# PetropoulakisPanagiotis/ICP-Variants

Hardware: AMD Instinct MI355X
Metric: ICP iterations/s (k-NN + point-to-plane linear, 370k-point ETH-Apartment-like pair) (higher is better)
Workload: dtype f32

## Files before the change

### icp-variants_amd/csrc/dev_fused.hpp

```cpp
struct RowSlotGen {
    const RowTerms& R;
    static constexpr int N = 27;
    template <int A> __device__ __forceinline__ double get() const { return row_slot<A>(R); }
};
struct P2pGen {
    float s[3], d[3]; double wd;
    static constexpr int N = 22;
    template <int A> __device__ __forceinline__ double get() const {
        double v;
        if constexpr (A < 3) v = (double)s[A];
        else if constexpr (A < 6) v = (double)d[A - 3];
        else if constexpr (A == 6) v = wd;
        else if constexpr (A < 10) v = wd * s[A - 7];
        else if constexpr (A < 13) v = wd * d[A - 10];
        else v = (double)d[(A - 13) / 3] * (wd * s[(A - 13) % 3]);
        return v;
    }
};
#ifndef ICP_FUSED_WAVES
#define ICP_FUSED_WAVES 6
#endif
#ifndef ICP_WAVE_STRIDE
#define ICP_WAVE_STRIDE (ICP_BVH_THREADS > 64 ? 128 : 0)
#endif
#ifndef ICP_DEBUG_WALK_ENDS
#define ICP_DEBUG_WALK_ENDS 0
#endif
#ifndef ICP_DEBUG_TIMES
#define ICP_DEBUG_TIMES 0
#endif
#if ICP_DEBUG_TIMES
#define ICP_STAMP(j) do { if (kp.dbg_steps && lane == 0) kp.dbg_steps[8 * (wave_slot) + (j)] = (int)(unsigned int)wall_clock64(); } while (0)
#define ICP_BUDGET_ROW(slot) ((kp.dbg_steps && 16 * kp.dbg_waves + 8 * 4096 <= kp.n) ? kp.dbg_steps + 8 * kp.dbg_waves + 8 * 4096 + 8 * (slot) : nullptr)
#else
#define ICP_STAMP(j)
#define ICP_BUDGET_ROW(slot) nullptr
#endif

template <int DIM> struct QueryIn {
    float r0, r1, r2;
    float c3, c4, c5;
    float rn0, rn1, rn2;
    int q0;
    float4 st;
    float4 ra, rb;
    float tq[DIM]; int j0;
};
template <int DIM>
__device__ __forceinline__ void fused_front_clear(QueryIn<DIM>& in) {
    in.r0 = 0.f; in.r1 = 0.f; in.r2 = 0.f; in.c3 = 0.f; in.c4 = 0.f; in.c5 = 0.f; in.rn0 = 0.f; in.rn1 = 0.f; in.rn2 = 0.f; in.q0 = -1; in.j0 = -1;
    in.st.x = 0.f; in.st.y = 0.f; in.st.z = 0.f; in.st.w = 0.f; in.ra = in.st; in.rb = in.st;
#pragma unroll
    for (int q = 0; q < DIM; q++) in.tq[q] = 0.f;
}
template <int DIM>
__device__ __forceinline__ void fused_front_loads(const KnnParams& kp, const PostParams& pp, const BvhViewT<DIM>& bv, int k, bool seeded, bool inc, QueryIn<DIM>& in) {
    fused_front_clear<DIM>(in);
    if (k >= 0) {
        const int i = kp.sel ? kp.sel[k] : k;
        in.r0 = kp.sx[i]; in.r1 = kp.sy[i]; in.r2 = kp.sz[i];
        if (DIM == 6) { in.c3 = kp.scr[i]; in.c4 = kp.scg[i]; in.c5 = kp.scb[i]; }
        in.rn0 = pp.snx[i]; in.rn1 = pp.sny[i]; in.rn2 = pp.snz[i];
        in.q0 = seeded ? kp.nn_raw[k] : -1;
        if (inc) in.st = kp.qstate[k];
        if (in.q0 >= 0) {
            if (DIM == 3) { in.ra = *(const float4*)(bv.recs + in.q0); in.rb = *((const float4*)(bv.recs + in.q0) + 1); in.tq[0] = in.ra.x; in.tq[1] = in.ra.y; in.tq[2] = in.ra.z; in.j0 = __float_as_int(in.ra.w); }
            else {
                const BvhLeafT<DIM>* lf = bv.leaves + (in.q0 >> 3);
#pragma unroll
                for (int q = 0; q < DIM; q++) in.tq[q] = lf->c[q][in.q0 & 7];
                in.j0 = lf->idx[in.q0 & 7];
            }
        }
    }
}

__host__ __device__ __forceinline__ int fused_wave_slot(int lb, int w, int mgrid) {
    constexpr int NW = BVH_THREADS / WAVE, S = ICP_WAVE_STRIDE;
    if (S == 0 || NW == 1) return lb * NW + w;
    if (S == 1) return w * mgrid + lb;
    const int g = lb / S, j = lb - g * S;
    return (g + 1) * S <= mgrid ? (g * NW + w) * S + j : lb * NW + w;
}

struct PairOut { bool valid; float s0, s1, s2, d0, d1, d2, n0, n1, n2, wt; };

template <int DIM, bool WIDE, bool XW = false>
__device__ __forceinline__ void fused_search_post(const KnnParams& kp, const BvhViewT<DIM>& bv, const PostParams& pp, int k, bool seeded, bool inc, const float* Pm, const float* Nm,
                                                  QueryIn<DIM>& in, uint2* __restrict__ bvh_lbq, int tid, int wave_slot, PairOut& o) {
    const int lane = tid & 63; (void)lane; (void)wave_slot; (void)seeded;
    o.valid = false; o.s0 = 0.f; o.s1 = 0.f; o.s2 = 0.f; o.d0 = 0.f; o.d1 = 0.f; o.d2 = 0.f; o.n0 = 0.f; o.n1 = 0.f; o.n2 = 0.f; o.wt = 0.f;
    float p[DIM];
#pragma unroll
    for (int q = 0; q < DIM; q++) p[q] = 0.f;
    if (DIM == 6) { p[3 % DIM] = in.c3; p[4 % DIM] = in.c4; p[5 % DIM] = in.c5; }
    float rn0 = in.rn0, rn1 = in.rn1, rn2 = in.rn2;
    float best = FLT_MAX, lb_others = 0.f; int bi = -1, bpos = -1, q0 = in.q0;
    float4 ra = in.ra, rb = in.rb;
#if ICP_DEBUG_TIMES
    float dbg_lbo = 0.f, dbg_lb3 = 0.f, dbg_delta = 0.f; int dbg_l2old = -1; const int dbg_q0old = in.q0;
#endif
    bool need_walk = false, verified = false, two_leaf = false;
    float lb3 = 0.f; int l2 = -1;
    if (k >= 0) {
        float2 st2; st2.x = 0.f; st2.y = __int_as_float(-1);
        xform_point(Pm, in.r0, in.r1, in.r2, p[0], p[1], p[2]);
        if (finite3(p[0], p[1], p[2]) && bv.n_valid > 0) {
            need_walk = true;
            if (q0 >= 0) {
                float d = 0.f;
#pragma unroll
                for (int q = 0; q < DIM; q++) { const float e = p[q] - in.tq[q]; d = (q == 0) ? e * e : d + e * e; }
                if (d < best) { best = d; bi = in.j0; bpos = q0; }
                if (inc && bi >= 0) {
                    const float ex = p[0] - in.st.x, ey = p[1] - in.st.y, ez = p[2] - in.st.z;
                    const float delta = sqrt_up((ex * ex + ey * ey) + ez * ez), sbest = sqrt_up(best);
                    const float lbn = (in.st.w - delta) * 0.999999f;
#if ICP_DEBUG_TIMES
                    dbg_lbo = in.st.w; dbg_lb3 = st2.x; dbg_delta = delta;
#endif
                    if (sbest < lbn) { lb_others = lbn; need_walk = false; verified = true; }
                    else {
                        if (kp.qstate2) st2 = kp.qstate2[k];
#if ICP_DEBUG_TIMES
                        dbg_l2old = __float_as_int(st2.y);
#endif
                        const float lb2 = (st2.x - delta) * 0.999999f;
                        l2 = __float_as_int(st2.y);
                        if (sbest < lb2) { two_leaf = true; lb3 = lb2; }
                    }
                }
            }
        }
    }
    ICP_STAMP(1);
#if ICP_DEBUG_TIMES
    if (kp.dbg_steps && k >= 0 && (need_walk || two_leaf) && seeded) {
        int* r = kp.dbg_steps + 8 * kp.dbg_waves + 8 * (k & 4095);
        r[0] = k; r[1] = __float_as_int(best); r[2] = __float_as_int(dbg_lbo); r[3] = __float_as_int(dbg_lb3); r[4] = __float_as_int(dbg_delta); r[5] = two_leaf ? l2 : -2; r[6] = q0; r[7] = (int)(unsigned int)wall_clock64();
    }
    if (kp.dbg_steps) { const int nw_ = __popcll(__ballot(need_walk && !two_leaf)), nl_ = __popcll(__ballot(two_leaf)); if (lane == 0) { kp.dbg_steps[8 * wave_slot + 6] = nw_ | (nl_ << 8);
            kp.dbg_steps[8 * wave_slot + 7] = (int)((__builtin_amdgcn_s_getreg((31 << 11) | 4) & 0xFFFFu) | (__builtin_amdgcn_s_getreg((31 << 11) | 20) << 16)); } }
#endif
    if (two_leaf) {
        f2 p2[DIM];
#pragma unroll
        for (int q = 0; q < DIM; q++) { p2[q].x = p[q]; p2[q].y = p[q]; }
        float b2 = FLT_MAX, b3 = FLT_MAX; int nl2 = -1;
        const int lf = q0 >> 3;
        if constexpr (DIM == 3) {
#pragma unroll 1
            for (int r = 0; r < 2; r++) {
                const int lx = r ? l2 : lf;
                if (r == 0 || (l2 >= 0 && l2 != lf)) leaf_eval<DIM>(bv.leaves + lx, lx, p2, best, bi, bpos, b2, nl2, b3);
            }
        } else {
            leaf_eval<DIM>(bv.leaves + lf, lf, p2, best, bi, bpos, b2, nl2, b3);
            if (l2 >= 0 && l2 != lf) leaf_eval<DIM>(bv.leaves + l2, l2, p2, best, bi, bpos, b2, nl2, b3);
        }
        lb_others = fminf(sqrt_dn(b2), lb3);
        lb3 = fminf(sqrt_dn(b3), lb3);
        l2 = nl2;
        need_walk = false;
    }
#if ICP_DEBUG_STEPS && !ICP_DEBUG_TIMES
    if (k >= 0 && kp.dbg_steps) kp.dbg_steps[k] = need_walk ? -1 : two_leaf ? -2 : 0;
#endif
#if ICP_DEBUG_TIMES
    if (int* row = ICP_BUDGET_ROW(wave_slot)) { if (lane < 8) row[lane] = 0; }
#endif
    bool walked = false;
    if (__any(need_walk)) {
        walked = true;
        float rn[3] = {rn0, rn1, rn2};
        knn_walk_shared<DIM, BVH_THREADS, typename std::conditional<WIDE, unsigned long long, unsigned int>::type, XW ? 1 : 0>(bv, p, rn, need_walk, best, bi, bpos, lb_others, lb3, l2, bvh_lbq, tid, kp.fault, ICP_BUDGET_ROW(wave_slot));
        rn0 = rn[0]; rn1 = rn[1]; rn2 = rn[2];
        q0 = -2;
        fused_front_clear<DIM>(in);
    }
    ICP_STAMP(2);
#if ICP_DEBUG_TIMES && ICP_DEBUG_WALK_ENDS
    if (k >= 0 && need_walk && seeded) {
        DEV_COUNT(8, 1);
        if (dbg_q0old >= 0 && (bpos >> 3) == (dbg_q0old >> 3)) DEV_COUNT(9, 1);
        if (dbg_l2old >= 0 && (bpos >> 3) == dbg_l2old) DEV_COUNT(10, 1);
    }
#endif
    asm volatile("" : "+v"(k));
    if (k >= 0) {
        if (!verified) knn_store_state<DIM>(kp, k, p, best, bpos, lb_others, lb3, l2);
        else if (kp.d2_out) kp.d2_out[k] = best;
        icp_match_t m;
        if (best <= kp.max_dist) { m.idx = bi; m.weight = 1.f; } else { m.idx = -1; m.weight = 0.f; }
        if (m.idx < 0) { if (pp.matches) pp.matches[k] = m; }
        else {
            if (walked || DIM != 3 || bpos != q0) { ra = *(const float4*)(bv.recs + bpos); rb = *((const float4*)(bv.recs + bpos) + 1); }
            o.d0 = ra.x; o.d1 = ra.y; o.d2 = ra.z; o.n0 = rb.x; o.n1 = rb.y; o.n2 = rb.z;
            o.s0 = p[0]; o.s1 = p[1]; o.s2 = p[2];
            o.valid = post_eval<true>(pp, k, m, o.d0, o.d1, o.d2, o.n0, o.n1, o.n2, __float_as_uint(rb.w), o.s0, o.s1, o.s2, o.wt, rn0, rn1, rn2, Nm);
        }
    }
    ICP_STAMP(3);
}

template <class StoreFn>
__device__ __forceinline__ void fused_block_epilogue(const KnnParams& kp, const PostParams& pp, PairOut& o, uint2* __restrict__ bvh_lbq, int tid, int wave_slot, const StoreFn& store) {
    constexpr int NW = BVH_THREADS / WAVE;
    const int lane = tid & 63, w = tid >> 6; (void)wave_slot; (void)kp;
    __syncthreads();
    double* lds = (double*)bvh_lbq;
    double tot;
    if (!o.valid) { o.s0 = 0.f; o.s1 = 0.f; o.s2 = 0.f; o.d0 = 0.f; o.d1 = 0.f; o.d2 = 0.f; o.n0 = 0.f; o.n1 = 0.f; o.n2 = 0.f; o.wt = 0.f; }
    if (pp.metric == ICP_METRIC_POINT_TO_PLANE) {
        RowTerms R;
        build_rows(0, o.s0, o.s1, o.s2, o.d0, o.d1, o.d2, o.n0, o.n1, o.n2, o.wt, R);
        const RowSlotGen g{R};
        tot = wave_transpose_reduce_gen<6, 0>(g, lane);
    } else {
        const P2pGen g{{o.s0, o.s1, o.s2}, {o.d0, o.d1, o.d2}, (double)o.wt};
        tot = wave_transpose_reduce_gen<6, 0>(g, lane);
    }
    ICP_STAMP(4);
    {
        const unsigned long long vm = __ballot(o.valid);
        const int v = wave_value_of_lane(lane);
        if (v < 32) lds[w * 32 + v] = tot;
        if (lane == 0) lds[NW * 32 + w] = (double)__popcll(vm);
    }
    __syncthreads();
    if (tid < NSUM_USED) {
        double out = 0.0;
        if (tid == SUM_N) { for (int ww = 0; ww < NW; ww++) out += lds[NW * 32 + ww]; }
        else {
            const int v = pp.metric == ICP_METRIC_POINT_TO_PLANE ? tid - SUM_M : tid - 1;
            const int nv = pp.metric == ICP_METRIC_POINT_TO_PLANE ? 27 : 22;
            if (v >= 0 && v < nv) { for (int ww = 0; ww < NW; ww++) out += lds[ww * 32 + v]; }
        }
        store(tid, out);
    }
    ICP_STAMP(5);
}

template <int DIM, bool WIDE, bool MERGED>
__device__ __forceinline__ void fused_matcher_body(const KnnParams& kp, const BvhViewT<DIM>& bv, const int* __restrict__ qorder, const PostParams& pp, const RingParams& rp) {
    extern __shared__ uint2 bvh_lbq[];
    constexpr int NW = BVH_THREADS / WAVE;
    if constexpr (MERGED) { if ((int)blockIdx.x < rp.n_red) { if (BVH_THREADS == RING_THREADS || threadIdx.x < RING_THREADS) ring_reduce_solve(rp); return; } }
    const int n_red = MERGED ? rp.n_red : 0;
    const int mblock = (int)blockIdx.x - n_red, mgrid = (int)gridDim.x - n_red;
    typedef const __attribute__((address_space(4))) float* cfloat_p;
    float Pm[16], Nm[9];
    if constexpr (!MERGED) {
        const cfloat_p pc = (cfloat_p)(const void*)kp.ps->pose; const cfloat_p nc = (cfloat_p)(const void*)kp.ps->nmat;
#pragma unroll
        for (int q = 0; q < 16; q++) Pm[q] = pc[q];
#pragma unroll
        for (int q = 0; q < 9; q++) Nm[q] = nc[q];
    }
    const int tid = threadIdx.x, lane = tid & 63, w = tid >> 6;
    const int lb = xcd_contiguous_block(mblock, mgrid);
    const int wave_slot = fused_wave_slot(lb, w, mgrid);
    const int t = wave_slot * BVH_QPW + lane;
    ICP_STAMP(0);
    const int k = ((BVH_QPW == WAVE || lane < BVH_QPW) && t < kp.n) ? (qorder ? qorder[t] : t) : -1;
    const bool seeded = kp.use_prev != 0, inc = kp.incremental && seeded;
    QueryIn<DIM> in;
    fused_front_loads<DIM>(kp, pp, bv, k, seeded, inc, in);
    constexpr bool XW = xw_enabled<DIM, BVH_THREADS>();
    if constexpr (XW) {
        xw_init<BVH_THREADS>(bvh_lbq, tid);
        asm volatile("s_waitcnt lgkmcnt(0)\n\ts_barrier" ::: "memory");
    }
    if constexpr (MERGED) { if (!ring_wait_pose(loop_slot((PoseState*)kp.ps, 0, (int)((blockIdx.x * 2u + (unsigned int)w) % (unsigned int)POSE_REPLICAS)), lane, rp.run_fault, Pm, Nm)) return; }
    PairOut o;
    fused_search_post<DIM, WIDE, XW>(kp, bv, pp, k, seeded, inc, Pm, Nm, in, bvh_lbq, tid, wave_slot, o);
    if constexpr (XW) {
        if (xw_block_is_searching<BVH_THREADS>(bvh_lbq)) {
            constexpr int NT = BVH_THREADS;
            bvh_lbq[3 * NT + tid] = make_uint2(__float_as_uint(o.s0), __float_as_uint(o.s1)); bvh_lbq[4 * NT + tid] = make_uint2(__float_as_uint(o.s2), __float_as_uint(o.d0));
            bvh_lbq[5 * NT + tid] = make_uint2(__float_as_uint(o.d1), __float_as_uint(o.d2)); bvh_lbq[7 * NT + tid] = make_uint2(__float_as_uint(o.n0), __float_as_uint(o.n1));
            bvh_lbq[8 * NT + tid] = make_uint2(__float_as_uint(o.n2), __float_as_uint(o.wt)); bvh_lbq[9 * NT + tid] = make_uint2(o.valid ? 1u : 0u, 0u);
            xw_help<DIM, NT, typename std::conditional<WIDE, unsigned long long, unsigned int>::type>(bv, bvh_lbq, tid, kp.fault, ICP_BUDGET_ROW(wave_slot));
            const uint2 a = bvh_lbq[3 * NT + tid], b = bvh_lbq[4 * NT + tid], c = bvh_lbq[5 * NT + tid], d = bvh_lbq[7 * NT + tid], e = bvh_lbq[8 * NT + tid], f = bvh_lbq[9 * NT + tid];
            o.s0 = __uint_as_float(a.x); o.s1 = __uint_as_float(a.y); o.s2 = __uint_as_float(b.x); o.d0 = __uint_as_float(b.y); o.d1 = __uint_as_float(c.x); o.d2 = __uint_as_float(c.y);
            o.n0 = __uint_as_float(d.x); o.n1 = __uint_as_float(d.y); o.n2 = __uint_as_float(e.x); o.wt = __uint_as_float(e.y); o.valid = f.x != 0u;
        }
    }
    double* partials = pp.partials;
    fused_block_epilogue(kp, pp, o, bvh_lbq, tid, wave_slot, [=](int a, double v) { partials[(size_t)a * mgrid + lb] = v; });
}
template <int DIM, bool WIDE>
__global__ __launch_bounds__(BVH_THREADS, DIM == 3 ? ICP_FUSED_WAVES : 4) void k_knn_bvh_post(const KnnParams kp, const BvhViewT<DIM> bv, const int* __restrict__ qorder, const PostParams pp) {
    const RingParams none{};
    fused_matcher_body<DIM, WIDE, false>(kp, bv, qorder, pp, none);
}
template <int DIM, bool WIDE>
__global__ __launch_bounds__(BVH_THREADS, DIM == 3 ? ICP_FUSED_WAVES : 4) void k_knn_bvh_post_ring(const KnnParams kp, const BvhViewT<DIM> bv, const int* __restrict__ qorder, const PostParams pp, const RingParams rp) {
    static_assert(BVH_THREADS >= RING_THREADS, "the reducer blocks are the first RING_THREADS threads of a matcher-sized block");
    fused_matcher_body<DIM, WIDE, true>(kp, bv, qorder, pp, rp);
}
```

### icp-variants_amd/csrc/dev_solve.hpp

```cpp
template <int n, int COPY>
__device__ inline void jacobi_eig_sym(double* A , double* V, double* ev) {
#pragma unroll
    for (int i = 0; i < n; i++) {
#pragma unroll
        for (int j = 0; j < n; j++) V[i * n + j] = (i == j) ? 1.0 : 0.0;
    }
    for (int sweep = 0; sweep < 50; sweep++) {
        double off = 0.0, dg = 0.0;
#pragma unroll
        for (int i = 0; i < n; i++) {
#pragma unroll
            for (int j = 0; j < n; j++) { if (i != j) off += A[i * n + j] * A[i * n + j]; else dg += A[i * n + j] * A[i * n + j]; }
        }
        if (off <= 1e-300 || off <= 1e-34 * dg) break;
#pragma unroll
        for (int p = 0; p < n - 1; p++) {
#pragma unroll
            for (int q = p + 1; q < n; q++) {
                const double apq = A[p * n + q];
                if (apq != 0.0) {
                    const double theta = (A[q * n + q] - A[p * n + p]) / (2.0 * apq);
                    const double t = (theta >= 0 ? 1.0 : -1.0) / (fabs(theta) + sqrt(theta * theta + 1.0));
                    const double c = 1.0 / sqrt(t * t + 1.0), s = t * c;
#pragma unroll
                    for (int k = 0; k < n; k++) { const double akp = A[k * n + p], akq = A[k * n + q]; A[k * n + p] = c * akp - s * akq; A[k * n + q] = s * akp + c * akq; }
#pragma unroll
                    for (int k = 0; k < n; k++) { const double apk = A[p * n + k], aqk = A[q * n + k]; A[p * n + k] = c * apk - s * aqk; A[q * n + k] = s * apk + c * aqk; }
#pragma unroll
                    for (int k = 0; k < n; k++) { const double vkp = V[k * n + p], vkq = V[k * n + q]; V[k * n + p] = c * vkp - s * vkq; V[k * n + q] = s * vkp + c * vkq; }
                    A[p * n + q] = 0.0; A[q * n + p] = 0.0;
                }
            }
        }
    }
#pragma unroll
    for (int i = 0; i < n; i++) ev[i] = A[i * n + i];
}

constexpr double RANK_CUT6 = 6.0 * 1.1920928955078125e-07;
constexpr double RANK_CUT3 = 3.0 * 1.1920928955078125e-07;
template <int COPY = 0>
__device__ inline void solve_normal_svd(const double* sums , double* x) {
    __shared__ double A[36], V[36], ev[6];
    int q = 0;
    for (int a = 0; a < 6; a++) for (int c = a; c < 6; c++) { A[a * 6 + c] = sums[q]; A[c * 6 + a] = sums[q]; q++; }
    const double* g = sums + 21;
    jacobi_eig_sym<6, COPY>(A, V, ev);
    double emax = 0.0;
    for (int i = 0; i < 6; i++) emax = fmax(emax, ev[i]);
    const double thr = RANK_CUT6;
    for (int i = 0; i < 6; i++) x[i] = 0.0;
    for (int j = 0; j < 6; j++) {
        if (!(ev[j] > thr * thr * emax)) continue;
        double vg = 0.0;
        for (int i = 0; i < 6; i++) vg += V[i * 6 + j] * g[i];
        const double coef = vg / ev[j];
        for (int i = 0; i < 6; i++) x[i] += V[i * 6 + j] * coef;
    }
}

template <int COPY = 0>
__device__ inline void solve_fullpiv_lu6(double* M, double* rhs, double* x, int* colp, double* y) {
    const int n = 6;
    for (int i = 0; i < n; i++) colp[i] = i;
    double maxpiv = 0.0; int rank = n;
    for (int k = 0; k < n; k++) {
        int pr = k, pc = k; double best = -1.0;
        for (int i = k; i < n; i++) for (int j = k; j < n; j++) { const double v = fabs(M[i * n + j]); if (v > best) { best = v; pr = i; pc = j; } }
        if (best > maxpiv) maxpiv = best;
        if (best == 0.0) { rank = k; break; }
        if (pr != k) { for (int j = 0; j < n; j++) { const double t = M[k * n + j]; M[k * n + j] = M[pr * n + j]; M[pr * n + j] = t; } const double t = rhs[k]; rhs[k] = rhs[pr]; rhs[pr] = t; }
        if (pc != k) { for (int i = 0; i < n; i++) { const double t = M[i * n + k]; M[i * n + k] = M[i * n + pc]; M[i * n + pc] = t; } const int t = colp[k]; colp[k] = colp[pc]; colp[pc] = t; }
        for (int i = k + 1; i < n; i++) {
            const double f = M[i * n + k] / M[k * n + k];
            for (int j = k + 1; j < n; j++) M[i * n + j] -= f * M[k * n + j];
            rhs[i] -= f * rhs[k];
        }
    }
    const double thr = 1.1920928955078125e-07 * 6.0;
    int r = 0;
    for (int k = 0; k < rank; k++) { if (fabs(M[k * n + k]) > maxpiv * thr) r++; else break; }
    for (int k = 0; k < n; k++) y[k] = 0.0;
    for (int k = r - 1; k >= 0; k--) { double s = rhs[k]; for (int j = k + 1; j < r; j++) s -= M[k * n + j] * y[j]; y[k] = s / M[k * n + k]; }
    for (int k = 0; k < n; k++) x[colp[k]] = (k < r) ? y[k] : 0.0;
}

template <int COPY = 0>
__device__ inline void procrustes_rotation(const double* A , double noise_floor, double* R) {
    __shared__ double B[9], V[9], ev[3], Vs[9], U[9];
    for (int i = 0; i < 3; i++) for (int j = 0; j < 3; j++) { double s = 0; for (int k = 0; k < 3; k++) s += A[k * 3 + i] * A[k * 3 + j]; B[i * 3 + j] = s; }
    jacobi_eig_sym<3, COPY>(B, V, ev);
    int o[3] = {0, 1, 2};
    for (int a = 0; a < 2; a++) for (int b = a + 1; b < 3; b++) if (ev[o[b]] > ev[o[a]]) { const int t = o[a]; o[a] = o[b]; o[b] = t; }
    for (int c = 0; c < 3; c++) for (int r = 0; r < 3; r++) Vs[r * 3 + c] = V[r * 3 + o[c]];
    double s0 = 0.0;
    for (int c = 0; c < 2; c++) {
        double u[3];
        for (int r = 0; r < 3; r++) { u[r] = 0; for (int k = 0; k < 3; k++) u[r] += A[r * 3 + k] * Vs[k * 3 + c]; }
        if (c == 1) {
            const double dp = u[0] * U[0] + u[1] * U[3] + u[2] * U[6];
            u[0] -= dp * U[0]; u[1] -= dp * U[3]; u[2] -= dp * U[6];
        }
        const double nr = sqrt(u[0] * u[0] + u[1] * u[1] + u[2] * u[2]);
        if (c == 0) {
            s0 = nr;
            if (!(nr > noise_floor)) { for (int i = 0; i < 9; i++) R[i] = (i % 4 == 0) ? 1.0 : 0.0; return; }
        } else if (!(nr > fmax(RANK_CUT3 * s0, noise_floor))) {
            const double v0 = Vs[0], v1 = Vs[3], v2 = Vs[6], u0 = U[0], u1 = U[3], u2 = U[6];
            const double cs = v0 * u0 + v1 * u1 + v2 * u2;
            if (1.0 + cs < 1e-8) {
                const int kmin = fabs(v0) < fabs(v1) ? (fabs(v0) < fabs(v2) ? 0 : 2) : (fabs(v1) < fabs(v2) ? 1 : 2);
                const double dp = (kmin == 0 ? v0 : (kmin == 1 ? v1 : v2));
                double a[3] = {(kmin == 0 ? 1.0 : 0.0) - dp * v0, (kmin == 1 ? 1.0 : 0.0) - dp * v1, (kmin == 2 ? 1.0 : 0.0) - dp * v2};
                const double an = sqrt(a[0] * a[0] + a[1] * a[1] + a[2] * a[2]);
                for (int i = 0; i < 3; i++) a[i] /= an;
                for (int r = 0; r < 3; r++) for (int q = 0; q < 3; q++) R[r * 3 + q] = 2.0 * a[r] * a[q] - (r == q ? 1.0 : 0.0);
            } else {
                const double k0 = v1 * u2 - v2 * u1, k1 = v2 * u0 - v0 * u2, k2 = v0 * u1 - v1 * u0, f = 1.0 / (1.0 + cs);
                const double kk = k0 * k0 + k1 * k1 + k2 * k2;
                R[0] = 1.0 + f * (k0 * k0 - kk); R[1] = -k2 + f * (k0 * k1);      R[2] = k1 + f * (k0 * k2);
                R[3] = k2 + f * (k1 * k0);       R[4] = 1.0 + f * (k1 * k1 - kk); R[5] = -k0 + f * (k1 * k2);
                R[6] = -k1 + f * (k2 * k0);      R[7] = k0 + f * (k2 * k1);       R[8] = 1.0 + f * (k2 * k2 - kk);
            }
            return;
        }
        for (int r = 0; r < 3; r++) U[r * 3 + c] = u[r] / nr;
    }
    U[2] = U[3] * U[7] - U[6] * U[4]; U[5] = U[6] * U[1] - U[0] * U[7]; U[8] = U[0] * U[4] - U[3] * U[1];
    const double detV = Vs[0] * (Vs[4] * Vs[8] - Vs[5] * Vs[7]) - Vs[1] * (Vs[3] * Vs[8] - Vs[5] * Vs[6]) + Vs[2] * (Vs[3] * Vs[7] - Vs[4] * Vs[6]);
    for (int r = 0; r < 3; r++) for (int c = 0; c < 3; c++)
        R[r * 3 + c] = (U[r * 3] * Vs[c * 3] + U[r * 3 + 1] * Vs[c * 3 + 1]) + detV * U[r * 3 + 2] * Vs[c * 3 + 2];
}

__device__ inline void mat4_mul_f32(const float* A, const float* B, float* C) {
    float T[16];
    for (int c = 0; c < 4; c++) for (int r = 0; r < 4; r++) {
        float acc = A[0 * 4 + r] * B[c * 4 + 0];
        acc = acc + A[1 * 4 + r] * B[c * 4 + 1];
        acc = acc + A[2 * 4 + r] * B[c * 4 + 2];
        acc = acc + A[3 * 4 + r] * B[c * 4 + 3];
        T[c * 4 + r] = acc;
    }
    for (int i = 0; i < 16; i++) C[i] = T[i];
}
__device__ inline void mat3_mul_f32(const float* A, const float* B, float* C) {
    float T[9];
    for (int r = 0; r < 3; r++) for (int c = 0; c < 3; c++) T[r * 3 + c] = A[r * 3] * B[c] + (A[r * 3 + 1] * B[3 + c] + A[r * 3 + 2] * B[6 + c]);
    for (int i = 0; i < 9; i++) C[i] = T[i];
}
__device__ inline void set_pose_f32(float* pose, const float* R, const float* t) {
    for (int i = 0; i < 16; i++) pose[i] = (i % 5 == 0) ? 1.f : 0.f;
    for (int r = 0; r < 3; r++) { for (int c = 0; c < 3; c++) pose[c * 4 + r] = R[r * 3 + c]; pose[12 + r] = t[r]; }
}
__device__ __host__ inline void normal_matrix_from_pose(const float* pose, float* N) {
    const double a = pose[0], b = pose[4], c = pose[8];
    const double d = pose[1], e = pose[5], f = pose[9];
    const double g = pose[2], h = pose[6], i = pose[10];
    const double c00 = e * i - f * h, c01 = f * g - d * i, c02 = d * h - e * g;
    const double c10 = c * h - b * i, c11 = a * i - c * g, c12 = b * g - a * h;
    const double c20 = b * f - c * e, c21 = c * d - a * f, c22 = a * e - b * d;
    const double det = (a * c00 + b * c01) + c * c02;
    N[0] = (float)(c00 / det); N[1] = (float)(c01 / det); N[2] = (float)(c02 / det);
    N[3] = (float)(c10 / det); N[4] = (float)(c11 / det); N[5] = (float)(c12 / det);
    N[6] = (float)(c20 / det); N[7] = (float)(c21 / det); N[8] = (float)(c22 / det);
}

__device__ inline float normal_matrix_entry(const float* pose, int e) {
    const double a = pose[0], b = pose[4], c = pose[8];
    const double d = pose[1], e_ = pose[5], f = pose[9];
    const double g = pose[2], h = pose[6], i = pose[10];
    const double c00 = e_ * i - f * h, c01 = f * g - d * i, c02 = d * h - e_ * g;
    const double det = (a * c00 + b * c01) + c * c02;
    double cof;
    switch (e) {
        case 0: cof = c00; break;  case 1: cof = c01; break;  case 2: cof = c02; break;
        case 3: cof = c * h - b * i; break;  case 4: cof = a * i - c * g; break;  case 5: cof = b * g - a * h; break;
        case 6: cof = b * f - c * e_; break;  case 7: cof = c * d - a * f; break;  default: cof = a * e_ - b * d; break;
    }
    return (float)(cof / det);
}

struct SolveParams {
    const double* partials; int nblocks;
    double* totals; unsigned* ticket;
    PoseState* ps;
    int metric; int phase;
    icp_iter_stats* stats;
    int n_src;
    double* sums_out;
    int update_pose;
    const double* rmse_partials; int rmse_blocks;
    int spin;
};

__device__ __forceinline__ void wave_sync() { __builtin_amdgcn_fence(__ATOMIC_ACQ_REL, "wavefront"); __builtin_amdgcn_wave_barrier(); }
constexpr int SDF_COPY = 4;
constexpr int SDF_COLOR_COPY = 5;
template <int COPY = 0>
__device__ __forceinline__ const float* p2plane_lanes_core(const double* m , const float* pose_in, double* x_out = nullptr) {
    __shared__ double A[6][7], Lm[6][6], od[6], zs[6], rd[6], hinv[6];
    __shared__ float npose[16];
    __shared__ int okflag, guardflag;
    const int tid = threadIdx.x;
    if (tid < WAVE) {
        const int i = tid / 7, j = tid % 7;
        if (tid < 42) A[i][j] = (j == 6) ? m[21 + i] : (j >= i ? m[i * 6 - i * (i - 1) / 2 + (j - i)] : 0.0);
        if (tid < 6) od[tid] = m[tid * 6 - tid * (tid - 1) / 2];
        wave_sync();
        bool ok_all = true;
        for (int k = 0; k < 6; k++) {
            const double d = A[k][k];
            const bool ok = (d > 1e-9 * od[k]) && (k > 0 || od[0] > 0);
            if (!ok) { ok_all = false; break; }
            if (tid < 42 && i > k && j >= i) {
                const double lik = A[k][i] / d;
                if (j == i) Lm[i][k] = lik;
                A[i][j] = A[i][j] - lik * A[k][j];
            }
            wave_sync();
        }
        if (tid == 0) okflag = ok_all ? 1 : 0;
    }
    __syncthreads();
    const bool factored = okflag != 0;
    if (factored && tid >= WAVE && tid < 2 * WAVE) {
        const int l = tid - WAVE;
        if (l < 6) rd[l] = 1.0 / A[l][l];
        wave_sync();
        const int kk = l < 6 ? l : 0;
        double z[6], h = 0.0;
#pragma unroll
        for (int r = 0; r < 6; r++) {
            double v = (r == kk) ? 1.0 : 0.0;
#pragma unroll
            for (int c = 0; c < r; c++) v = v - Lm[r][c] * z[c];
            z[r] = v;
            h = h + (v * v) * rd[r];
        }
        if (l < 6) hinv[l] = h;
        wave_sync();
        if (l == 0) {
            const double tr = ((((od[0] + od[1]) + od[2]) + od[3]) + od[4]) + od[5], tri = ((((hinv[0] + hinv[1]) + hinv[2]) + hinv[3]) + hinv[4]) + hinv[5];
            guardflag = (RANK_CUT6 * RANK_CUT6) * tr * tri < 1.0 ? 1 : 0;
        }
    }
    if (tid < WAVE) {
        if (factored) {
            if (tid < 6) zs[tid] = A[tid][6] / A[tid][tid];
            wave_sync();
            double x[6];
#pragma unroll
            for (int r = 5; r >= 0; r--) {
                double v = zs[r];
#pragma unroll
                for (int c = r + 1; c < 6; c++) v = v - Lm[c][r] * x[c];
                x[r] = v;
            }
            if constexpr (COPY == SDF_COPY || COPY == SDF_COLOR_COPY) {
                if (tid < 6) x_out[tid] = tid == 0 ? x[0] : tid == 1 ? x[1] : tid == 2 ? x[2] : tid == 3 ? x[3] : tid == 4 ? x[4] : x[5];
            }
            const float ang = (float)(tid == 0 ? x[0] : tid == 1 ? x[1] : x[2]);
            double sd, cd;
            sincos((double)ang, &sd, &cd);
            const float sf = (float)sd, cf = (float)cd;
            const float ca = __int_as_float(__builtin_amdgcn_readlane(__float_as_int(cf), 0)), sa = __int_as_float(__builtin_amdgcn_readlane(__float_as_int(sf), 0));
            const float cb = __int_as_float(__builtin_amdgcn_readlane(__float_as_int(cf), 1)), sb = __int_as_float(__builtin_amdgcn_readlane(__float_as_int(sf), 1));
            const float cg = __int_as_float(__builtin_amdgcn_readlane(__float_as_int(cf), 2)), sg = __int_as_float(__builtin_amdgcn_readlane(__float_as_int(sf), 2));
            if (tid < 16) {
                const int c = tid >> 2, r = tid & 3;
                const float one = 1.f, zero = 0.f;
                const float rx0 = r == 0 ? one : zero, rx1 = r == 1 ? ca : r == 2 ? sa : zero, rx2 = r == 1 ? -sa : r == 2 ? ca : zero;
                const float ry[9] = {cb, zero, sb, zero, one, zero, -sb, zero, cb}, rz[9] = {cg, -sg, zero, sg, cg, zero, zero, zero, one};
                float q[3], rr[3];
#pragma unroll
                for (int e = 0; e < 3; e++) q[e] = rx0 * ry[e] + (rx1 * ry[3 + e] + rx2 * ry[6 + e]);
#pragma unroll
                for (int e = 0; e < 3; e++) rr[e] = q[0] * rz[e] + (q[1] * rz[3 + e] + q[2] * rz[6 + e]);
                const float tr = (float)(r == 0 ? x[3] : r == 1 ? x[4] : x[5]);
                const float d0 = r < 3 ? rr[0] : zero, d1 = r < 3 ? rr[1] : zero, d2 = r < 3 ? rr[2] : zero, d3 = r < 3 ? tr : one;
                float acc = d0 * pose_in[c * 4 + 0];
                acc = acc + d1 * pose_in[c * 4 + 1];
                acc = acc + d2 * pose_in[c * 4 + 2];
                acc = acc + d3 * pose_in[c * 4 + 3];
                npose[tid] = acc;
            }
        }
    }
    __syncthreads();
    if (!factored || !guardflag) return nullptr;
    return npose;
}
template <int COPY = 0>
__device__ __forceinline__ bool solve_p2plane_lanes(const SolveParams& sp, const double* tot ) {
    if (!(sp.update_pose && sp.metric == ICP_METRIC_POINT_TO_PLANE && sp.phase == 0 && tot[SUM_N] > 0)) return false;
    PoseState* ps = sp.ps;
    const float* npose = p2plane_lanes_core<COPY>(tot + SUM_M, ps->pose);
    if (!npose) return false;
    const int tid = threadIdx.x;
    if (tid == 0 && sp.sums_out) for (int a = 0; a < NSUM; a++) sp.sums_out[a] = tot[a];
    if (tid >= 64 && tid < 70) {
        const int k = tid - 64; const double n = tot[SUM_N];
        if (k < 3) ps->mean_s[k] = (float)(tot[SUM_S + k] / n); else ps->mean_d[k - 3] = (float)(tot[SUM_D + k - 3] / n);
    }
    if (tid < 16) { ps->pose[tid] = npose[tid]; if (sp.stats) sp.stats->pose[tid] = npose[tid]; }
    if (tid >= 32 && tid < 41) ps->nmat[tid - 32] = normal_matrix_entry(npose, tid - 32);
    if (tid == 33 && sp.stats) {
        sp.stats->n_src = sp.n_src; sp.stats->n_valid = (int)tot[SUM_N];
        sp.stats->rmse = -1.f; sp.stats->benchmark_error = -1.f; sp.stats->status = ICP_OK;
    }
    return true;
}

template <bool WITH_SYMMETRIC, int COPY = 0>
__device__ inline void solve_generic(const SolveParams& sp, const double* tot) {
    if (sp.sums_out) for (int a = 0; a < NSUM; a++) sp.sums_out[a] = tot[a];
    PoseState* ps = sp.ps;
    const double n = tot[SUM_N];
    if (sp.phase == 0) {
        float ms[3] = {0, 0, 0}, md[3] = {0, 0, 0};
        if (n > 0) for (int k = 0; k < 3; k++) { ms[k] = (float)(tot[SUM_S + k] / n); md[k] = (float)(tot[SUM_D + k] / n); }
        for (int k = 0; k < 3; k++) { ps->mean_s[k] = ms[k]; ps->mean_d[k] = md[k]; }
    }
    if (!sp.update_pose) return;
    if (sp.metric == ICP_METRIC_SYMMETRIC && sp.phase == 0) return;
    int status = ICP_OK;
    float dT[16];
    for (int i = 0; i < 16; i++) dT[i] = (i % 5 == 0) ? 1.f : 0.f;
    if (!(n > 0)) {
        status = ICP_ERR_NO_CORRESPONDENCES;
    } else if (sp.metric == ICP_METRIC_POINT_TO_PLANE) {
        double x[6];
        solve_normal_svd<COPY>(tot + SUM_M, x);
        const float al = (float)x[0], be = (float)x[1], ga = (float)x[2];
        const float ca = (float)cos((double)al), sa = (float)sin((double)al);
        const float cb = (float)cos((double)be), sb = (float)sin((double)be);
        const float cg = (float)cos((double)ga), sg = (float)sin((double)ga);
        const float Rx[9] = {1, 0, 0, 0, ca, -sa, 0, sa, ca}, Ry[9] = {cb, 0, sb, 0, 1, 0, -sb, 0, cb}, Rz[9] = {cg, -sg, 0, sg, cg, 0, 0, 0, 1};
        float Rxy[9], R[9];
        mat3_mul_f32(Rx, Ry, Rxy); mat3_mul_f32(Rxy, Rz, R);
        const float t[3] = {(float)x[3], (float)x[4], (float)x[5]};
        set_pose_f32(dT, R, t);
    } else if (sp.metric == ICP_METRIC_POINT_TO_POINT) {
        const double* m = tot + SUM_M;
        const float msf[3] = {ps->mean_s[0], ps->mean_s[1], ps->mean_s[2]}, mdf[3] = {ps->mean_d[0], ps->mean_d[1], ps->mean_d[2]};
        __shared__ double A[9], Rd[9];
        for (int j = 0; j < 3; j++) for (int k = 0; k < 3; k++)
            A[j * 3 + k] = m[7 + j * 3 + k] - m[4 + j] * (double)msf[k] - (double)mdf[j] * m[1 + k] + m[0] * (double)mdf[j] * (double)msf[k];
        double mom = 0.0;
        for (int i = 0; i < 9; i++) mom = fmax(mom, fabs(m[7 + i]));
        float R[9];
        procrustes_rotation<COPY>(A, (RANK_CUT3 * RANK_CUT3) * mom, Rd);
        for (int i = 0; i < 9; i++) R[i] = (float)Rd[i];
        const float tr[3] = {mdf[0] - msf[0], mdf[1] - msf[1], mdf[2] - msf[2]};
        float t[3];
        for (int r = 0; r < 3; r++) {
            const float Rt = R[r * 3] * tr[0] + (R[r * 3 + 1] * tr[1] + R[r * 3 + 2] * tr[2]);
            const float Rm = R[r * 3] * mdf[0] + (R[r * 3 + 1] * mdf[1] + R[r * 3 + 2] * mdf[2]);
            t[r] = (Rt - Rm) + mdf[r];
        }
        set_pose_f32(dT, R, t);
    } else if constexpr (WITH_SYMMETRIC) {
        __shared__ double M[36], g[6], x[6], ywork[6];
        __shared__ int colp[6];
        int q = 0;
        for (int a = 0; a < 6; a++) for (int c = a; c < 6; c++) { M[a * 6 + c] = tot[SUM_M + q]; M[c * 6 + a] = tot[SUM_M + q]; q++; }
        for (int a = 0; a < 6; a++) g[a] = tot[SUM_M + 21 + a];
        const float lambda = 0.0001f; const float l2 = lambda * lambda;
        for (int a = 0; a < 6; a++) M[a * 6 + a] += (double)l2;
        solve_fullpiv_lu6<COPY>(M, g, x, colp, ywork);
        const float at[3] = {(float)x[0], (float)x[1], (float)x[2]}, tt[3] = {(float)x[3], (float)x[4], (float)x[5]};
        const float tan_theta = sqrtf(at[0] * at[0] + (at[1] * at[1] + at[2] * at[2]));
        const float ax[3] = {at[0] / tan_theta, at[1] / tan_theta, at[2] / tan_theta};
        const float sin_theta = (float)((double)tan_theta / sqrt(1.0 + (double)(tan_theta * tan_theta)));
        const float cos_theta = sin_theta / tan_theta;
        const float t[3] = {tt[0] * cos_theta, tt[1] * cos_theta, tt[2] * cos_theta};
        const float K[9] = {0, -ax[2], ax[1], ax[2], 0, -ax[0], -ax[1], ax[0], 0};
        float Ks[9], KK[9], Rod[9];
        const float omc = 1 - cos_theta;
        for (int i = 0; i < 9; i++) Ks[i] = omc * K[i];
        mat3_mul_f32(Ks, K, KK);
        for (int i = 0; i < 9; i++) Rod[i] = ((i % 4 == 0) ? 1.f : 0.f) + (sin_theta * K[i] + KK[i]);
        const float I3[9] = {1, 0, 0, 0, 1, 0, 0, 0, 1}, zero[3] = {0, 0, 0};
        const float md[3] = {ps->mean_d[0], ps->mean_d[1], ps->mean_d[2]}, nms[3] = {-ps->mean_s[0], -ps->mean_s[1], -ps->mean_s[2]};
        float Tm[16], Tt[16], Ts[16], Rm[16], t1[16], t2[16];
        set_pose_f32(Tm, I3, md); set_pose_f32(Tt, I3, t); set_pose_f32(Ts, I3, nms); set_pose_f32(Rm, Rod, zero);
        mat4_mul_f32(Tm, Rm, t1); mat4_mul_f32(t1, Tt, t2); mat4_mul_f32(t2, Rm, t1); mat4_mul_f32(t1, Ts, dT);
    }
    if (status == ICP_OK) {
        float np[16];
        mat4_mul_f32(dT, ps->pose, np);
        for (int i = 0; i < 16; i++) ps->pose[i] = np[i];
        normal_matrix_from_pose(ps->pose, ps->nmat);
    }
    if (sp.stats) {
        sp.stats->n_src = sp.n_src;
        sp.stats->n_valid = (int)n;
        for (int i = 0; i < 16; i++) sp.stats->pose[i] = ps->pose[i];
        sp.stats->rmse = -1.f;
        sp.stats->benchmark_error = -1.f;
        sp.stats->status = status;
    }
}

template <bool WITH_SYMMETRIC = true, int COPY = 0>
__device__ __forceinline__ void solve_tail(const SolveParams& sp, const double* tot) {
    if (solve_p2plane_lanes<COPY>(sp, tot)) return;
    if (threadIdx.x == 0) solve_generic<WITH_SYMMETRIC, COPY>(sp, tot);
}

constexpr int SOLVE_THREADS = 256;
constexpr unsigned long long TOTAL_SENTINEL = 0xFFF8D1CEC0DE5EEDull;
constexpr int SPIN_LIMIT = 1 << 22;
constexpr int SOLVE_INFLIGHT = 12;
__global__ __launch_bounds__(SOLVE_THREADS) void k_reduce_solve(const SolveParams sp) {
#include "dev_body_reduce_solve.hpp"
}


#ifndef ICP_POSE_REPLICAS
#define ICP_POSE_REPLICAS 16
#endif
constexpr int POSE_REPLICAS = ICP_POSE_REPLICAS;
constexpr size_t POSE_REPLICA_STRIDE = 4096 + 128;
__device__ __host__ __forceinline__ PoseState* loop_slot(PoseState* base, int g, int replica) {
    return (PoseState*)((char*)base + ((size_t)g * POSE_REPLICAS + (size_t)replica) * POSE_REPLICA_STRIDE);
}
__global__ void k_run_init(const PoseState* __restrict__ src, PoseState* slots, int n_slots, unsigned long long* totals, int n_totals, int* zero_words, int n_zero) {
    const int t = blockIdx.x * blockDim.x + threadIdx.x;
    const int n_slot_granules = n_slots * POSE_REPLICAS * 16;
    if (t < n_slot_granules) {
        const int g = t / (POSE_REPLICAS * 16), r = (t / 16) % POSE_REPLICAS, q = t & 15;
        unsigned long long* dst = (unsigned long long*)loop_slot(slots, g, r) + q;
        *dst = g == 0 ? ((const unsigned long long*)src)[q] : ~0ull;
    } else if (t < n_slot_granules + n_totals) totals[t - n_slot_granules] = ~0ull;
    else if (t < n_slot_granules + n_totals + n_zero) zero_words[t - n_slot_granules - n_totals] = 0;
}
constexpr unsigned long long GRANULE_EMPTY = ~0ull;
#ifndef ICP_RING_SLEEP
#define ICP_RING_SLEEP 4
#endif
struct RingParams {
    const double* red_partials; int red_nblocks;
    unsigned long long* totals_row;
    const PoseState* ps_in;
    PoseState* ps_out;
    icp_iter_stats* stats; int n_src;
    PoseState* final_out;
    int* run_fault;
    int n_red;
    ConvergeParams cv;
};
__device__ __forceinline__ unsigned long long granule_of(unsigned int lo, unsigned int hi) {
    const unsigned long long g = ((unsigned long long)hi << 32) | lo;
    return g == GRANULE_EMPTY ? g ^ 1ull : g;
}
constexpr int RING_THREADS = 128;
#ifndef ICP_DEBUG_TIMES
#define ICP_DEBUG_TIMES 0
#endif
#if ICP_DEBUG_TIMES
__device__ int g_ring_dbg[(NSUM_USED + 1) * 8];
#define RING_STAMP(a, j) do { if (threadIdx.x == 0 && !rp.final_out) g_ring_dbg[8 * (a) + (j)] = (int)(unsigned int)wall_clock64(); } while (0)
#else
#define RING_STAMP(a, j)
#endif
__device__ __forceinline__ void ring_reduce_solve(const RingParams& rp) {
    __shared__ double tot[NSUM];
    __shared__ double wsum[4];
    __shared__ unsigned int slot_words[32];
    __shared__ int give_up;
    const int tid = threadIdx.x, lane = tid & 63, w = tid >> 6, a = blockIdx.x;
    RING_STAMP(a, 0);
    if (a == 0 && rp.ps_in->fault) {
        { const unsigned int* src = (const unsigned int*)rp.ps_in; for (int q = tid; q < 16 * POSE_REPLICAS; q += RING_THREADS) __hip_atomic_store((unsigned long long*)loop_slot(rp.ps_out, 0, q >> 4) + (q & 15), granule_of(src[2 * (q & 15)], src[2 * (q & 15) + 1]), __ATOMIC_RELAXED, __HIP_MEMORY_SCOPE_AGENT);
          if (rp.final_out && tid < 32) ((unsigned int*)rp.final_out)[tid] = src[tid]; }
        return;
    }
    {
        const double* __restrict__ row = rp.red_partials + (size_t)a * rp.red_nblocks;
        double x0 = 0.0, x1 = 0.0;
        for (int b0 = 0; b0 < rp.red_nblocks; b0 += SOLVE_INFLIGHT * SOLVE_THREADS) {
            double v0[SOLVE_INFLIGHT], v1[SOLVE_INFLIGHT];
#pragma unroll
            for (int j = 0; j < SOLVE_INFLIGHT; j++) {
                const int b = b0 + j * SOLVE_THREADS + tid;
                v0[j] = b < rp.red_nblocks ? row[b] : 0.0;
                v1[j] = b + RING_THREADS < rp.red_nblocks ? row[b + RING_THREADS] : 0.0;
            }
#pragma unroll
            for (int j = 0; j < SOLVE_INFLIGHT; j++) {
                const int b = b0 + j * SOLVE_THREADS + tid;
                if (b < rp.red_nblocks) x0 += v0[j];
                if (b + RING_THREADS < rp.red_nblocks) x1 += v1[j];
            }
        }
        for (int off = 32; off > 0; off >>= 1) { x0 += __shfl_down(x0, off, WAVE); x1 += __shfl_down(x1, off, WAVE); }
        if (lane == 0) { wsum[w] = x0; wsum[2 + w] = x1; }
    }
    RING_STAMP(a, 1);
    __syncthreads();
    if (tid == 0) {
        double x = wsum[0];
        for (int k = 1; k < 4; k++) x += wsum[k];
        const unsigned long long bits = (unsigned long long)__double_as_longlong(x);
        __hip_atomic_store(rp.totals_row + a, granule_of((unsigned int)bits, (unsigned int)(bits >> 32)), __ATOMIC_RELAXED, __HIP_MEMORY_SCOPE_AGENT);
    }
    RING_STAMP(a, 2);
    if (a != 0) return;
    if (tid == 0) give_up = 0;
    __syncthreads();
    if (tid < NSUM) {
        double v = 0.0;
        if (tid < NSUM_USED) {
            unsigned long long bits = GRANULE_EMPTY;
            for (int spin = 0; spin < SPIN_LIMIT; spin++) {
                bits = __hip_atomic_load(rp.totals_row + tid, __ATOMIC_RELAXED, __HIP_MEMORY_SCOPE_AGENT);
                if (bits != GRANULE_EMPTY) break;
                __builtin_amdgcn_s_sleep(2);
            }
            if (bits == GRANULE_EMPTY) give_up = 1;
            v = __longlong_as_double((long long)bits);
        }
        tot[tid] = v;
    }
    __syncthreads();
    RING_STAMP(NSUM_USED, 0);
    const PoseState* pin = rp.ps_in;
    const double n = tot[SUM_N];
    int fault = 0, status = ICP_OK;
    const float* npose = nullptr;
    if (give_up) { fault = 1; if (tid == 0) atomicOr(rp.run_fault, 1); }
    else if (n > 0) { npose = p2plane_lanes_core(tot + SUM_M, pin->pose); if (!npose) fault = 2; }
    else status = ICP_ERR_NO_CORRESPONDENCES;
    RING_STAMP(NSUM_USED, 1);
    int code = fault;
    if (rp.cv.on && !fault) {
        if (tid < WAVE && converge_step(rp.cv, npose ? npose : pin->pose, pin->pose, status == ICP_OK, tid)) code = SLOT_STOPPED;
    }
    if (tid < 16) slot_words[tid] = __float_as_uint(npose ? npose[tid] : pin->pose[tid]);
    if (tid >= 32 && tid < 41) slot_words[16 + tid - 32] = __float_as_uint(npose ? normal_matrix_entry(npose, tid - 32) : pin->nmat[tid - 32]);
    if (tid >= 64 && tid < 70) {
        const int k = tid - 64;
        slot_words[25 + k] = __float_as_uint(n > 0 ? (float)(tot[(k < 3 ? SUM_S : SUM_D - 3) + k] / n) : 0.f);
    }
    if (tid == 0) slot_words[31] = (unsigned int)code;
    __syncthreads();
    for (int q = tid; q < 16 * POSE_REPLICAS; q += RING_THREADS)
        __hip_atomic_store((unsigned long long*)loop_slot(rp.ps_out, 0, q >> 4) + (q & 15), granule_of(slot_words[2 * (q & 15)], slot_words[2 * (q & 15) + 1]), __ATOMIC_RELAXED, __HIP_MEMORY_SCOPE_AGENT);
    RING_STAMP(NSUM_USED, 2);
    if (rp.final_out && tid < 32) ((unsigned int*)rp.final_out)[tid] = slot_words[tid];
    if (rp.stats && !fault) {
        if (tid < 16) rp.stats->pose[tid] = __uint_as_float(slot_words[tid]);
        if (tid == 16) { rp.stats->n_src = rp.n_src; rp.stats->n_valid = (int)n; rp.stats->rmse = -1.f; rp.stats->benchmark_error = -1.f; rp.stats->status = status; }
    }
}
__global__ __launch_bounds__(RING_THREADS) void k_ring_reduce_solve(const RingParams rp) { ring_reduce_solve(rp); }

__device__ __forceinline__ bool ring_wait_pose(const PoseState* slot, int lane, int* run_fault, float (&Pm)[16], float (&Nm)[9]) {
    const unsigned long long* g = (const unsigned long long*)slot;
    unsigned long long v = 0ull;
    bool ok = false;
    for (int spin = 0; spin < SPIN_LIMIT; spin++) {
        if (lane < 16) v = __hip_atomic_load(g + lane, __ATOMIC_RELAXED, __HIP_MEMORY_SCOPE_AGENT);
        if (!__any(lane < 16 && v == GRANULE_EMPTY)) { ok = true; break; }
        __builtin_amdgcn_s_sleep(ICP_RING_SLEEP);
    }
    if (!ok) { if (lane == 0) atomicOr(run_fault, 1); return false; }
    const int lo = (int)(unsigned int)v, hi = (int)(unsigned int)(v >> 32);
#pragma unroll
    for (int q = 0; q < 16; q++) Pm[q] = __int_as_float(__builtin_amdgcn_readlane((q & 1) ? hi : lo, q >> 1));
#pragma unroll
    for (int q = 0; q < 9; q++) Nm[q] = __int_as_float(__builtin_amdgcn_readlane(((16 + q) & 1) ? hi : lo, (16 + q) >> 1));
    return __builtin_amdgcn_readlane(hi, 15) == 0;
}
```

### icp-variants_amd/csrc/host_ctx.hpp

```cpp
using namespace icpdev;

#define HIPCK(ctx, expr)                                                                        \
    do {                                                                                        \
        hipError_t e__ = (expr);                                                                \
        if (e__ != hipSuccess) {                                                                \
            char buf__[256];                                                                    \
            snprintf(buf__, sizeof(buf__), "%s failed: %s (%s:%d)", #expr, hipGetErrorString(e__), __FILE__, __LINE__); \
            (ctx)->err = buf__;                                                                 \
            return ICP_ERR_HIP;                                                                 \
        }                                                                                       \
    } while (0)

namespace {
std::atomic<long long> g_live_bytes{0};

struct DevBuf {
    void* p = nullptr; size_t cap = 0;
    bool view = false;
    DevBuf() = default;
    DevBuf(DevBuf&& o) noexcept : p(o.p), cap(o.cap), view(o.view) { o.p = nullptr; o.cap = 0; o.view = false; }
    DevBuf& operator=(DevBuf&& o) noexcept { if (this != &o) { reset(); p = o.p; cap = o.cap; view = o.view; o.p = nullptr; o.cap = 0; o.view = false; } return *this; }
    ~DevBuf() { reset(); }
    void reset() { if (p && !view) { (void)hipFree(p); g_live_bytes -= (long long)cap; } p = nullptr; cap = 0; view = false; }
    template <class T> T* as() const { return (T*)p; }
};
static_assert(!std::is_copy_constructible<DevBuf>::value && !std::is_copy_assignable<DevBuf>::value, "a copied DevBuf would be freed twice");
struct PinBuf {
    void* p = nullptr; size_t cap = 0;
    PinBuf() = default; PinBuf(const PinBuf&) = delete; PinBuf& operator=(const PinBuf&) = delete;
    ~PinBuf() { if (p) (void)hipHostFree(p); }
    template <class T> T* as() const { return (T*)p; }
};
struct Event {
    hipEvent_t e = nullptr;
    Event() = default; Event(Event&& o) noexcept : e(o.e) { o.e = nullptr; } Event& operator=(Event&& o) noexcept { std::swap(e, o.e); return *this; }
    ~Event() { if (e) (void)hipEventDestroy(e); }
    operator hipEvent_t() const { return e; }
};
struct Stream {
    hipStream_t s = nullptr;
    Stream() = default; Stream(const Stream&) = delete; Stream& operator=(const Stream&) = delete;
    ~Stream() { if (s) (void)hipStreamDestroy(s); }
    operator hipStream_t() const { return s; }
};

struct Cloud {
    int n = 0, npad = 0;
    DevBuf x, y, z, nx, ny, nz, cr, cg, cb, rgba;
    bool has_normals = false, has_colors = false;
};

struct Level { DevBuf idx; DevBuf order; DevBuf sorted_idx; DevBuf pack; Cloud sorted; bool sorted_valid = false; int n = 0; };

struct NssLevel { DevBuf cand, seg, longs; int n_base = 0, max_long = 0, max_chunks = 0; };
struct NssHeld { Level lv; uint32_t word = 0; };

struct FpfhCache { DevBuf nb_idx, nb_d2, counts, pairs, feat; bool ready = false; int k = 0, stride = 0, n = 0, nk = 0; };

struct Bvh {
    bool valid = false;
    int n_valid = 0, n_leaves = 0, Lp = 1;
    DevBuf keys, keys2, vals, vals2, temp, leaves, recs, nodes, qnodes, pos_of;
    DevBuf axl[12], side, scanr, axis_of_node;
    int n_ids = 0;
    const Cloud* attrs = nullptr;
    int Lq = 0;
    const int* d_finite = nullptr;
    double build_ms = 0.0;
};
}

struct icp_ctx {
    int device = 0;
    Stream own_stream, depth_stream;
    hipStream_t stream = nullptr;
    int stage_timing = 1;
    unsigned timing_phase = 0;
    PinBuf pinned;
    bool trace = false;
    bool merge_loop = true;
    int merged_runs = 0, merged_fallbacks = 0;
    bool lm_on = false; icp_lm_options lm_opt;
    DevBuf lm_state, lm_partials, lm_sums;
    std::vector<icp_lm_summary> lm_last;
    DevBuf ms_ps, ms_nn, ms_st, ms_st2, ms_rec, ms_d2, ms_partials, ms_totals, ms_stats, ms_score, ms_res;
    icp_gicp_options gicp_opt = {1e-3f, 20};
    DevBuf gicp_n[2][3], gicp_flag;
    bool gicp_ready[2] = {false, false};
    icp_colored_options col_opt = {0.968f, 20};
    DevBuf col_grad[3];
    bool col_ready = false;
    icp_robust_options rob_opt = {ICP_ROBUST_NONE, 0.f, 0.f, 1.f};
    DevBuf rob_keys, rob_state, rob_stats;
    std::vector<icp_robust_stats> rob_last;
    icp_reciprocal_options rcp_opt = {0};
    Bvh src_bvh; DevBuf src_rflag, src_finite;
    DevBuf rcp_stats;
    bool rcp_naive = false; DevBuf rcp_q[3], rcp_nn;
    std::vector<icp_reciprocal_stats> rcp_last;
    icp_convergence_options cvg_opt = {0, 1e-6f, 1e-6f, 1, 1};
    icp_convergence_result cvg_last = {0, 0, 0, -1.f, -1.f};
    std::vector<icp_convergence_step> cvg_trace;
    icp_global_options glob_opt = {20, 1, 1, 4096, 0.9f, 0.005f, 0u, 16};
    FpfhCache fpfh[2];
    DevBuf gm_best[2], gm_fwd, gm_keep, gm_list, gm_idx, gm_pts, gm_hyp;
    std::vector<icp_global_hypothesis> glob_last;
    icp_params prm;
    Cloud tgt, src, qry;
    Cloud nrm_cloud; Bvh nrm_bvh;
    Bvh bvh, bvh6;
    DevBuf src_flag, src_box;
    DevBuf tgt_flag, tgt_finite, nrm_finite, sel_temp, d_count;
    PinBuf pin_up; Event up_ev; bool up_pending = false;
    DevBuf okeys, okeys2, ovals, otemp;
    std::map<int, Level> levels;
    DevBuf sel_lists, sel_counts, sel_blocks;
    icp_nss_options nss_opt = {5, 1};
    DevBuf nss_bkt; int nss_bkt_grid = 0;
    std::map<int, NssLevel> nss_levels;
    std::map<int, NssHeld> nss_held;
    float nss_held_proba = 0.f; uint32_t nss_held_seed = 0u; bool nss_held_stale = false;
    DevBuf nss_table, nss_quota, nss_thr, nss_state, nss_hist, nss_total;
    std::vector<std::pair<const int*, int>> sel_last;
    DevBuf qpack; size_t q_cap = 0;
    DevBuf qstate, qstate2;
    DevBuf dbg_steps;
    DevBuf ps, matches, d2, best64, nn_raw, partials, partials2, ring, totals, sums, stats, staging, rmse_partials, rmse_out, fontana_partials;
    Cloud conv_src, conv_ref; int conv_n = 0;
    PinBuf depth_pin[2]; DevBuf depth_dev[2]; Event depth_up[2]; bool depth_pending[2] = {false, false};
    DevBuf depth_blocks, track_rmse;
    PinBuf pin_track;
    DevBuf tsdf_vox, tsdf_cnt; bool tsdf_on = false; icp_tsdf_options tsdf_opt;
    DevBuf tsdf_col; bool tsdf_col_on = false;
    DevBuf th_keys, th_vals, th_pool, th_pkey, th_ctr;
    bool tsdf_hashed = false; int th_log2cap = 0, th_pool_cap = 0, th_nblk = 0, th_grown = 0, th_unplaced = 0, th_max_log2 = 22; long long th_oor = 0;
    DevBuf tm_bits, tm_mask, tm_base, tm_blk, tm_out;
    DevBuf tm_nbr, tm_ord;
    DevBuf sdf_state, sdf_partials, sdf_rec; Event sdf_ev;
    DevBuf vg_box, vg_count, vg_sums, vg_cells;
    bool vg_ready = false; float vg_voxel = 0.f; icp_voxel_grid_info vg_info = {{0, 0, 0}, {0, 0, 0}, 0, 0};
    DevBuf vm_count, vm_sums, vm_cells, vm_stamp, vm_list, vm_ctr, vm_box;
    bool vm_on = false; icp_voxel_map_options vm_opt = {0.f, {0, 0, 0}, {0, 0, 0}}; int vm_serial = 0;
    DevBuf vh_keys;
    bool vm_hashed = false; int vh_log2cap = 0, vh_grown = 0; long long vh_bound = 0;
    bool vh_vac = false; int vh_compacted = 0; long long vh_vac_bound = 0;
    float cos_reject = 0.5f;
    std::vector<Event> events;
    Event build_ev[2];
    icp_timing timing;
    std::vector<float> it_match_ms, it_post_ms, it_solve_ms;
    std::string err;
};

namespace {
constexpr int POST_BLOCKS = 512;

int ensure(icp_ctx* c, DevBuf& b, size_t bytes) {
    if (bytes <= b.cap && b.p) return ICP_OK;
    if (b.view) { b.p = nullptr; b.cap = 0; b.view = false; }
    if (b.p) { HIPCK(c, hipFree(b.p)); g_live_bytes -= (long long)b.cap; b.p = nullptr; b.cap = 0; }
    size_t want = bytes < 256 ? 256 : bytes;
    HIPCK(c, hipMalloc(&b.p, want));
    b.cap = want; g_live_bytes += (long long)want;
    return ICP_OK;
}
int ensure_pin(icp_ctx* c, PinBuf& b, size_t bytes, size_t min_bytes, size_t slack_div) {
    if (bytes <= b.cap && b.p) return ICP_OK;
    if (b.p) { HIPCK(c, hipHostFree(b.p)); b.p = nullptr; b.cap = 0; }
    const size_t want = bytes < min_bytes ? min_bytes : bytes + (slack_div ? bytes / slack_div : 0);
    HIPCK(c, hipHostMalloc(&b.p, want, hipHostMallocDefault));
    b.cap = want;
    return ICP_OK;
}
int ensure_pinned(icp_ctx* c, size_t bytes) { return ensure_pin(c, c->pinned, bytes, 4096, 0); }
void release(DevBuf& b) { b.reset(); }
void set_view(DevBuf& b, void* p, size_t bytes) { release(b); b.p = p; b.cap = bytes; b.view = true; }
void release(Cloud& c) { release(c.x); release(c.y); release(c.z); release(c.nx); release(c.ny); release(c.nz); release(c.cr); release(c.cg); release(c.cb); release(c.rgba); }
void release(Level& lv) { release(lv.idx); release(lv.order); release(lv.sorted_idx); release(lv.sorted); release(lv.pack); lv.sorted_valid = false; }
void release(NssLevel& nl) { release(nl.cand); release(nl.seg); release(nl.longs); }
void drop_nss(icp_ctx* c, bool held_only);

float compute_cos_reject() {
    const double threshold = 60 * 3.141592653589793238462643383279502884 / 180.0;
    uint32_t lo, hi; float flo = 0.25f, fhi = 0.75f;
    memcpy(&lo, &flo, 4); memcpy(&hi, &fhi, 4);
    while (hi - lo > 1) {
        uint32_t mid = lo + (hi - lo) / 2; float fm; memcpy(&fm, &mid, 4);
        if ((double)acosf(fm) > threshold) lo = mid; else hi = mid;
    }
    float r; memcpy(&r, &lo, 4);
    return r;
}

int set_device(icp_ctx* c) { HIPCK(c, hipSetDevice(c->device)); return ICP_OK; }

struct DrainOnError {
    icp_ctx* c; bool ok = false;
    explicit DrainOnError(icp_ctx* ctx) : c(ctx) {}
    ~DrainOnError() { if (!ok && c && c->stream) (void)hipStreamSynchronize(c->stream); }
    int done(int rc = ICP_OK) { ok = (rc == ICP_OK); return rc; }
};

int ensure_pin_up(icp_ctx* c, size_t bytes) {
    if (c->up_pending) { HIPCK(c, hipEventSynchronize(c->up_ev)); c->up_pending = false; }
    int rc;
    if ((rc = ensure_pin(c, c->pin_up, bytes, 65536, 8))) return rc;
    if (!c->up_ev) HIPCK(c, hipEventCreateWithFlags(&c->up_ev.e, hipEventDisableTiming));
    return ICP_OK;
}
int upload_cloud(icp_ctx* c, Cloud& cl, const float* xyz, const float* nrm, const uint8_t* rgba, int n, bool pad_inf) {
    const int npad = pad_inf ? ((n + 63) / 64) * 64 : n;
    const size_t b_xyz = (size_t)n * 12, b_nrm = nrm ? (size_t)n * 12 : 0, b_col = rgba ? (size_t)n * 4 : 0, total = b_xyz + b_nrm + b_col;
    int rc;
    if ((rc = ensure_pin_up(c, total))) return rc;
    if ((rc = ensure(c, c->staging, total))) return rc;
    char* h = c->pin_up.as<char>();
    memcpy(h, xyz, b_xyz);
    if (nrm) memcpy(h + b_xyz, nrm, b_nrm);
    if (rgba) memcpy(h + b_xyz + b_nrm, rgba, b_col);
    HIPCK(c, hipMemcpyAsync(c->staging.p, h, total, hipMemcpyHostToDevice, c->stream));
    HIPCK(c, hipEventRecord(c->up_ev, c->stream)); c->up_pending = true;
    const char* d = c->staging.as<char>();
    const dim3 g((npad + 255) / 256), b(256);
    for (DevBuf* pl : {&cl.x, &cl.y, &cl.z}) if ((rc = ensure(c, *pl, (size_t)npad * 4))) return rc;
    hipLaunchKernelGGL(k_deinterleave3, g, b, 0, c->stream, (const float*)d, n, npad, INFINITY, cl.x.as<float>(), cl.y.as<float>(), cl.z.as<float>());
    cl.has_normals = nrm != nullptr;
    if (nrm) {
        for (DevBuf* pl : {&cl.nx, &cl.ny, &cl.nz}) if ((rc = ensure(c, *pl, (size_t)n * 4))) return rc;
        hipLaunchKernelGGL(k_deinterleave3, dim3((n + 255) / 256), b, 0, c->stream, (const float*)(d + b_xyz), n, n, 0.f, cl.nx.as<float>(), cl.ny.as<float>(), cl.nz.as<float>());
    }
    cl.has_colors = rgba != nullptr;
    if (rgba) {
        for (DevBuf* pl : {&cl.rgba, &cl.cr, &cl.cg, &cl.cb}) if ((rc = ensure(c, *pl, (size_t)npad * 4))) return rc;
        hipLaunchKernelGGL(k_colors, g, b, 0, c->stream, (const uint8_t*)(d + b_xyz + b_nrm), n, npad, cl.rgba.as<uint32_t>(), cl.cr.as<float>(), cl.cg.as<float>(), cl.cb.as<float>());
    }
    HIPCK(c, hipGetLastError());
    cl.n = n; cl.npad = npad;
    return ICP_OK;
}
int upload3(icp_ctx* c, const float* aos, int n, int npad, float pad_value, DevBuf& x, DevBuf& y, DevBuf& z) {
    int rc;
    if ((rc = ensure_pin_up(c, (size_t)n * 12))) return rc;
    if ((rc = ensure(c, c->staging, (size_t)n * 12))) return rc;
    for (DevBuf* pl : {&x, &y, &z}) if ((rc = ensure(c, *pl, (size_t)npad * 4))) return rc;
    memcpy(c->pin_up.p, aos, (size_t)n * 12);
    HIPCK(c, hipMemcpyAsync(c->staging.p, c->pin_up.p, (size_t)n * 12, hipMemcpyHostToDevice, c->stream));
    HIPCK(c, hipEventRecord(c->up_ev, c->stream)); c->up_pending = true;
    hipLaunchKernelGGL(k_deinterleave3, dim3((npad + 255) / 256), dim3(256), 0, c->stream, c->staging.as<float>(), n, npad, pad_value, x.as<float>(), y.as<float>(), z.as<float>());
    HIPCK(c, hipGetLastError());
    HIPCK(c, hipStreamSynchronize(c->stream));
    return ICP_OK;
}

int count_slot(icp_ctx* c, int** slot) {
    int rc;
    if ((rc = ensure_pinned(c, 4096))) return rc;
    *slot = (int*)(c->pinned.as<char>() + 2048);
    return ICP_OK;
}
int read_count(icp_ctx* c, const void* d_count, int* out, int n_words = 1) {
    int rc; int* h;
    if ((rc = count_slot(c, &h))) return rc;
    HIPCK(c, hipMemcpyAsync(h, d_count, (size_t)n_words * 4, hipMemcpyDeviceToHost, c->stream));
    HIPCK(c, hipStreamSynchronize(c->stream));
    memcpy(out, h, (size_t)n_words * 4);
    return ICP_OK;
}

int compact_flagged(icp_ctx* c, const uint8_t* d_flags, int count, int factor, DevBuf& out, int* n_out) {
    int rc;
    if ((rc = ensure(c, out, (size_t)(count > 0 ? count : 1) * 4))) return rc;
    if ((rc = ensure(c, c->d_count, 16))) return rc;
    *n_out = 0;
    if (count <= 0) return ICP_OK;
    auto in = rocprim::make_transform_iterator(rocprim::counting_iterator<int>(0), MulBy{factor});
    size_t tb = 0;
    HIPCK(c, rocprim::select(nullptr, tb, in, d_flags, out.as<int>(), c->d_count.as<int>(), (size_t)count, c->stream));
    if ((rc = ensure(c, c->sel_temp, tb))) return rc;
    HIPCK(c, rocprim::select(c->sel_temp.p, tb, in, d_flags, out.as<int>(), c->d_count.as<int>(), (size_t)count, c->stream));
    return read_count(c, c->d_count.p, n_out);
}
int finite_list(icp_ctx* c, const Cloud& cl, bool with_normals, DevBuf& flag, DevBuf& list, int* n_out) {
    int rc;
    if ((rc = ensure(c, flag, (size_t)cl.n))) return rc;
    const bool nrm = with_normals && cl.has_normals;
    hipLaunchKernelGGL(k_mark_finite, dim3((cl.n + 255) / 256), dim3(256), 0, c->stream, cl.x.as<float>(), cl.y.as<float>(), cl.z.as<float>(),
                       nrm ? cl.nx.as<float>() : nullptr, nrm ? cl.ny.as<float>() : nullptr, nrm ? cl.nz.as<float>() : nullptr, cl.n, flag.as<uint8_t>());
    HIPCK(c, hipGetLastError());
    return compact_flagged(c, flag.as<uint8_t>(), cl.n, 1, list, n_out);
}

int write_pose_via(icp_ctx* c, PoseState* h, const float pose[16]) {
    int rc;
    memset(h, 0, sizeof(*h));
    memcpy(h->pose, pose, 64);
    normal_matrix_from_pose(h->pose, h->nmat);
    if ((rc = ensure(c, c->ps, sizeof(PoseState)))) return rc;
    HIPCK(c, hipMemcpyAsync(c->ps.p, h, sizeof(*h), hipMemcpyHostToDevice, c->stream));
    return ICP_OK;
}
int write_pose(icp_ctx* c, const float pose[16]) {
    int rc;
    if ((rc = ensure_pinned(c, sizeof(PoseState)))) return rc;
    return write_pose_via(c, c->pinned.as<PoseState>(), pose);
}

int check_ready(icp_ctx* c, bool need_source, bool full_pipeline) {
    const icp_params& p = c->prm;
    if (c->tgt.n <= 0) { c->err = "target index needs to be built before querying (icp_set_target)"; return ICP_ERR_NO_TARGET; }
    if (need_source && c->src.n <= 0) { c->err = "no source cloud (icp_set_source)"; return ICP_ERR_NO_SOURCE; }
    if (p.matching == ICP_MATCH_PROJECTIVE) {
        if (p.height <= 0 || p.width <= 0) { c->err = "set camera params before querying any matches"; return ICP_ERR_NO_CAMERA; }
        if ((long long)p.width * p.height != c->tgt.n) { c->err = "invalid size of target points (must be width*height)"; return ICP_ERR_TARGET_SIZE; }
    } else if (p.color_icp) {
        if (!c->tgt.has_colors || (need_source && !c->src.has_colors)) { c->err = "colour ICP needs colours on target and source"; return ICP_ERR_COLOR_MISMATCH; }
    }
    if (full_pipeline) {
        if (!c->tgt.has_normals || !c->src.has_normals) { c->err = "normals required on source and target"; return ICP_ERR_INVALID_ARG; }
        if (p.weighting == ICP_WEIGHT_COLORS && (!c->tgt.has_colors || !c->src.has_colors)) { c->err = "colour weighting needs colours"; return ICP_ERR_COLOR_MISMATCH; }
    }
    return ICP_OK;
}

int ensure_events(icp_ctx* c, size_t count) {
    while (c->events.size() < count) { Event e; HIPCK(c, hipEventCreate(&e.e)); c->events.push_back(std::move(e)); }
    return ICP_OK;
}
}
```

### icp-variants_amd/csrc/host_debug.hpp

```cpp
extern "C" {
int icp_debug_steps(icp_ctx* c, int32_t* out, int32_t n) {
    if (!c || !out || n <= 0 || !c->dbg_steps.p || (size_t)n * 4 > c->dbg_steps.cap) return ICP_ERR_INVALID_ARG;
    int rc;
    if ((rc = set_device(c))) return rc;
    HIPCK(c, hipMemcpy(out, c->dbg_steps.p, (size_t)n * 4, hipMemcpyDeviceToHost));
    return ICP_OK;
}

int icp_debug_ring_times(icp_ctx* c, int32_t* out, int32_t n) {
#if ICP_DEBUG_TIMES
    if (!c || !out || n < (NSUM_USED + 1) * 8) return ICP_ERR_INVALID_ARG;
    int rc;
    if ((rc = set_device(c))) return rc;
    HIPCK(c, hipMemcpyFromSymbol(out, HIP_SYMBOL(icpdev::g_ring_dbg), (size_t)(NSUM_USED + 1) * 8 * 4));
    return ICP_OK;
#else
    (void)c; (void)out; (void)n;
    return ICP_ERR_INVALID_ARG;
#endif
}
int icp_debug_dev_counters(icp_ctx* c, uint32_t* out16, int32_t reset) {
#if ICP_DEBUG_TIMES
    if (!c || !out16) return ICP_ERR_INVALID_ARG;
    int rc;
    if ((rc = set_device(c))) return rc;
    HIPCK(c, hipStreamSynchronize(c->stream));
    HIPCK(c, hipMemcpyFromSymbol(out16, HIP_SYMBOL(icpdev::g_dev_counts), 64));
    if (reset == 2) HIPCK(c, hipMemcpyFromSymbol(out16, HIP_SYMBOL(icpdev::g_walk_trace), 256));
    if (reset) { uint32_t z[16] = {0}; HIPCK(c, hipMemcpyToSymbol(HIP_SYMBOL(icpdev::g_dev_counts), z, 64)); }
    return ICP_OK;
#else
    (void)c; (void)out16; (void)reset;
    return ICP_ERR_INVALID_ARG;
#endif
}
int icp_debug_wave_slot(int32_t lb, int32_t w, int32_t mgrid, int32_t* waves_per_block) {
    if (waves_per_block) *waves_per_block = BVH_THREADS / WAVE;
    if (lb < 0 || lb >= mgrid || w < 0 || w >= BVH_THREADS / WAVE) return -1;
    return icpdev::fused_wave_slot(lb, w, mgrid);
}
__global__ void k_debug_pos_of(const icpdev::TgtRec* recs, const int* pos_of, int n_slots, int* bad) {
    const int i = blockIdx.x * blockDim.x + threadIdx.x;
    if (i < n_slots && recs[i].idx >= 0 && pos_of[recs[i].idx] != i) atomicAdd(bad, 1);
}
int icp_debug_pos_of_mismatches(icp_ctx* c, int32_t* n_bad, int32_t* n_checked) {
    if (!c || !n_bad || !c->bvh.valid) return ICP_ERR_INVALID_ARG;
    int rc;
    if ((rc = set_device(c))) return rc;
    const int n_slots = (c->bvh.n_leaves > 0 ? c->bvh.n_leaves : 1) * BVH_LEAF;
    if ((rc = ensure(c, c->d_count, 4))) return rc;
    HIPCK(c, hipMemsetAsync(c->d_count.p, 0, 4, c->stream));
    hipLaunchKernelGGL(k_debug_pos_of, dim3((n_slots + 255) / 256), dim3(256), 0, c->stream, c->bvh.recs.as<icpdev::TgtRec>(), c->bvh.pos_of.as<int>(), n_slots, c->d_count.as<int>());
    HIPCK(c, hipMemcpyAsync(n_bad, c->d_count.p, 4, hipMemcpyDeviceToHost, c->stream));
    HIPCK(c, hipStreamSynchronize(c->stream));
    if (n_checked) *n_checked = c->bvh.n_valid;
    return ICP_OK;
}
int icp_debug_live_bytes(int64_t* out) {
    if (!out) return ICP_ERR_INVALID_ARG;
    *out = (int64_t)g_live_bytes.load();
    return ICP_OK;
}
int icp_debug_reciprocal_naive(icp_ctx* c, int32_t on) {
    if (!c) return ICP_ERR_INVALID_ARG;
    c->rcp_naive = on != 0;
    return ICP_OK;
}
int icp_debug_counters(icp_ctx* c, int32_t* merged_runs, int32_t* merged_fallbacks) {
    if (!c) return ICP_ERR_INVALID_ARG;
    if (merged_runs) *merged_runs = c->merged_runs;
    if (merged_fallbacks) *merged_fallbacks = c->merged_fallbacks;
    return ICP_OK;
}
int icp_debug_poison_handover(icp_ctx* c, int32_t slot, double value) {
    if (!c || slot < 0 || slot >= NSUM) return ICP_ERR_INVALID_ARG;
    int rc;
    if ((rc = set_device(c))) return rc;
    if (!c->totals.p && (rc = rearm_handover(c))) return rc;
    HIPCK(c, hipMemcpyAsync(c->totals.as<double>() + slot, &value, 8, hipMemcpyHostToDevice, c->stream));
    HIPCK(c, hipStreamSynchronize(c->stream));
    return ICP_OK;
}

int icp_debug_loop_sums(icp_ctx* c, const float pose[16], int32_t form, int32_t iteration, double* sums_out, int32_t* n_valid_out, float* pose_out, int32_t* route_out) {
    if (!c || !pose || !sums_out || !n_valid_out || !pose_out || !route_out || (form != 0 && form != 1)) { if (c) c->err = "icp_debug_loop_sums: bad argument"; return ICP_ERR_INVALID_ARG; }
    const icp_params& p = c->prm;
    int rc;
    DrainOnError guard(c);
    if ((rc = set_device(c))) return rc;
    if ((rc = check_ready(c, true, true))) return rc;
    if ((rc = gicp_prepare(c))) return rc;
    if ((rc = colored_prepare(c))) return rc;
    if (c->lm_on || robust_on(c) || reciprocal_on(c)) { c->err = "icp_debug_loop_sums: the non-linear optimiser, robust mode and reciprocal rejection run other chains"; return ICP_ERR_INVALID_ARG; }
    RunPlan pl;
    if ((rc = make_plan(c, false, pl))) return rc;
    const int iters = pl.iters(), it = iteration;
    if (it < 0 || it >= iters || pl.ns[it] <= 0) { c->err = "icp_debug_loop_sums: no such iteration in the plan, or it has no queries"; return ICP_ERR_INVALID_ARG; }
    const bool colors = p.color_icp != 0 && p.matching == ICP_MATCH_KNN;
    const bool lbvh = p.matching == ICP_MATCH_KNN && p.knn_backend == ICP_KNN_LBVH;
    double hs[NSUM]; icp_iter_stats st; memset(&st, 0, sizeof(st)); PoseState hp; int family = 0;
    if (form == 0) {
        if ((rc = ensure(c, c->stats, 512)) || (rc = ensure(c, c->sums, NSUM * 8))) return rc;
        if ((rc = rearm_handover(c))) return rc;
        if ((rc = write_pose(c, pose))) return rc;
        QuerySet q{pl.clouds[it], pl.sels[it], pl.ns[it], 0, colors, false, pl.orders[it], false};
        int fused = 0;
        if ((rc = launch_match(c, q, &fused))) return rc;
        if ((rc = launch_post_and_solve(c, *pl.clouds[it], pl.sels[it], pl.ns[it], c->stats.as<icp_iter_stats>(), c->sums.as<double>(), 1, nullptr, fused, nullptr))) return rc;
        family = fused ? 1 : 0;
        HIPCK(c, hipMemcpyAsync(hs, c->sums.p, NSUM * 8, hipMemcpyDeviceToHost, c->stream));
        HIPCK(c, hipMemcpyAsync(&st, c->stats.p, sizeof(st), hipMemcpyDeviceToHost, c->stream));
        HIPCK(c, hipMemcpyAsync(&hp, c->ps.p, sizeof(hp), hipMemcpyDeviceToHost, c->stream));
        HIPCK(c, hipStreamSynchronize(c->stream));
        if (hp.fault) { c->err = "reduction hand-over timed out on the device (k_reduce_solve)"; return ICP_ERR_HIP; }
    } else {
        const bool rec = (p.record_rmse & 3) && c->conv_n > 0;
        bool merged = iters >= 2 && pl.sorted_levels && p.metric == ICP_METRIC_POINT_TO_PLANE && !rec;
        for (int i = 0; merged && i < iters; i++) if (pl.ns[i] <= 0) merged = false;
        if (!merged) { c->err = "icp_debug_loop_sums: the loop of this configuration does not take the merged form"; return ICP_ERR_INVALID_ARG; }
        const int two[2] = {it, it + 1 < iters ? it + 1 : it};
        LoopRun r{};
        r.pl.sorted_levels = pl.sorted_levels; r.pl.fixed_sets = pl.fixed_sets;
        for (int k : two) { r.pl.factors.push_back(pl.factors[k]); r.pl.ns.push_back(pl.ns[k]); r.pl.clouds.push_back(pl.clouds[k]); r.pl.sels.push_back(pl.sels[k]); r.pl.orders.push_back(pl.orders[k]); }
        r.lay_out(2, false, false);
        if ((rc = ensure_pinned(c, r.pin_bytes))) return rc;
        if ((rc = write_pose(c, pose))) return rc;
        if ((rc = ensure(c, c->stats, r.stats_bytes))) return rc;
        if ((rc = ensure_events(c, 2 * 4 + 2))) return rc;
        r.sampled.assign(2, 0); r.eligible.assign(2, 0); r.ev.assign(2, IterEvents());
        if ((rc = enqueue_merged(c, r))) return rc;
        unsigned long long row[NSUM];
        HIPCK(c, hipMemcpyAsync(row, c->ring.as<char>() + (size_t)3 * POSE_REPLICAS * POSE_REPLICA_STRIDE, NSUM * 8, hipMemcpyDeviceToHost, c->stream));
        HIPCK(c, hipMemcpyAsync(&hp, loop_slot(c->ring.as<PoseState>(), 1, 0), sizeof(hp), hipMemcpyDeviceToHost, c->stream));
        HIPCK(c, hipStreamSynchronize(c->stream));
        if (r.host_tail(c)->merged_fault || hp.fault == 1) { c->err = "icp_debug_loop_sums: a bounded wait of the merged launches ran out"; return ICP_ERR_HIP; }
        for (int a = 0; a < NSUM; a++) {
            if (a < NSUM_USED && row[a] == GRANULE_EMPTY) { c->err = "icp_debug_loop_sums: a total of the ring was never written"; return ICP_ERR_HIP; }
            if (a < NSUM_USED) memcpy(&hs[a], &row[a], 8); else hs[a] = 0.0;
        }
        if (hp.fault) { memcpy(st.pose, pose, 64); st.n_valid = (int)hs[SUM_N]; }
        else memcpy(&st, r.host_records(c), sizeof(st));
        family = 2;
    }
    const Bvh& b = colors ? c->bvh6 : c->bvh;
    route_out[0] = family; route_out[1] = colors ? 6 : 3; route_out[2] = lbvh ? (b.Lq > 8 ? 1 : 0) : -1; route_out[3] = hp.fault;
    memset(sums_out, 0, 64 * 8); memcpy(sums_out, hs, NSUM * 8);
    *n_valid_out = st.n_valid;
    memcpy(pose_out, st.pose, 64);
    return guard.done();
}

__global__ void k_debug_walk_steps(int n_leaves, const icpdev::BvhLeafT<3>* leaves, const float* lq, const int* leaf_no, const float* sf, const int* si, float* of, int* oi,
                                   int n_nodes, const icpdev::BvhQuadT<3>* nodes, const float* nq, float* bounds) {
    const int i = blockIdx.x * blockDim.x + threadIdx.x;
    if (i < n_leaves) {
        icpdev::f2 p2[3];
        for (int k = 0; k < 3; k++) { p2[k].x = lq[3 * i + k]; p2[k].y = p2[k].x; }
        float best = sf[3 * i], b2 = sf[3 * i + 1], b3 = sf[3 * i + 2]; int bi = si[3 * i], bpos = si[3 * i + 1], l2 = si[3 * i + 2];
        const int flags = icpdev::leaf_eval<3>(leaves + i, leaf_no[i], p2, best, bi, bpos, b2, l2, b3);
        of[3 * i] = best; of[3 * i + 1] = b2; of[3 * i + 2] = b3; oi[4 * i] = bi; oi[4 * i + 1] = bpos; oi[4 * i + 2] = l2; oi[4 * i + 3] = flags;
    }
    if (i < n_nodes) {
        icpdev::f2 p2[3], l01, l23;
        for (int k = 0; k < 3; k++) { p2[k].x = nq[3 * i + k]; p2[k].y = p2[k].x; }
        icpdev::quad_lb<3>(nodes + i, p2, l01, l23);
        bounds[4 * i] = l01.x; bounds[4 * i + 1] = l01.y; bounds[4 * i + 2] = l23.x; bounds[4 * i + 3] = l23.y;
    }
}
int icp_debug_walk_steps(icp_ctx* c, int32_t n_leaves, const void* leaves, const float* lq, const int32_t* leaf_no, const float* sf, const int32_t* si, float* of, int32_t* oi,
                         int32_t n_nodes, const void* nodes, const float* nq, float* bounds, float* empty_box) {
    if (!c || n_leaves < 0 || n_nodes < 0 || n_leaves > (1 << 20) || n_nodes > (1 << 20)) return ICP_ERR_INVALID_ARG;
    if (n_leaves > 0 && (!leaves || !lq || !leaf_no || !sf || !si || !of || !oi)) return ICP_ERR_INVALID_ARG;
    if (n_nodes > 0 && (!nodes || !nq || !bounds)) return ICP_ERR_INVALID_ARG;
    if (empty_box) { empty_box[0] = icpdev::BVH_QUAD_EMPTY_LO; empty_box[1] = icpdev::BVH_QUAD_EMPTY_HI; }
    const int n = n_leaves > n_nodes ? n_leaves : n_nodes;
    if (n == 0) return ICP_OK;
    int rc;
    if ((rc = set_device(c))) return rc;
    DrainOnError guard(c);
    const size_t L = (size_t)n_leaves, N = (size_t)n_nodes;
    auto up = [](size_t x) { return (x + 127) & ~(size_t)127; };
    const size_t o_lq = 128 * L, o_no = up(o_lq + 12 * L), o_sf = up(o_no + 4 * L), o_si = up(o_sf + 12 * L), o_nd = up(o_si + 12 * L), o_nq = o_nd + 128 * N, o_of = up(o_nq + 12 * N),
                 o_oi = up(o_of + 12 * L), o_bd = up(o_oi + 16 * L), total = o_bd + 16 * N;
    if ((rc = ensure(c, c->staging, total))) return rc;
    char* d = c->staging.as<char>();
    if (L) {
        HIPCK(c, hipMemcpyAsync(d, leaves, 128 * L, hipMemcpyHostToDevice, c->stream));
        HIPCK(c, hipMemcpyAsync(d + o_lq, lq, 12 * L, hipMemcpyHostToDevice, c->stream));
        HIPCK(c, hipMemcpyAsync(d + o_no, leaf_no, 4 * L, hipMemcpyHostToDevice, c->stream));
        HIPCK(c, hipMemcpyAsync(d + o_sf, sf, 12 * L, hipMemcpyHostToDevice, c->stream));
        HIPCK(c, hipMemcpyAsync(d + o_si, si, 12 * L, hipMemcpyHostToDevice, c->stream));
    }
    if (N) {
        HIPCK(c, hipMemcpyAsync(d + o_nd, nodes, 128 * N, hipMemcpyHostToDevice, c->stream));
        HIPCK(c, hipMemcpyAsync(d + o_nq, nq, 12 * N, hipMemcpyHostToDevice, c->stream));
    }
    hipLaunchKernelGGL(k_debug_walk_steps, dim3((unsigned)((n + 255) / 256)), dim3(256), 0, c->stream, n_leaves, (const icpdev::BvhLeafT<3>*)d, (const float*)(d + o_lq), (const int*)(d + o_no),
                       (const float*)(d + o_sf), (const int*)(d + o_si), (float*)(d + o_of), (int*)(d + o_oi), n_nodes, (const icpdev::BvhQuadT<3>*)(d + o_nd), (const float*)(d + o_nq), (float*)(d + o_bd));
    HIPCK(c, hipGetLastError());
    if (L) {
        HIPCK(c, hipMemcpyAsync(of, d + o_of, 12 * L, hipMemcpyDeviceToHost, c->stream));
        HIPCK(c, hipMemcpyAsync(oi, d + o_oi, 16 * L, hipMemcpyDeviceToHost, c->stream));
    }
    if (N) HIPCK(c, hipMemcpyAsync(bounds, d + o_bd, 16 * N, hipMemcpyDeviceToHost, c->stream));
    HIPCK(c, hipStreamSynchronize(c->stream));
    return guard.done();
}

int icp_selftest_wave_reduce(icp_ctx* c, const double* in, double* out, int32_t* lane_of) {
    if (!c || !in || !out || !lane_of) return ICP_ERR_INVALID_ARG;
    int rc;
    if ((rc = set_device(c))) return rc;
    DrainOnError guard(c);
    if ((rc = ensure(c, c->staging, 64 * 27 * 8 + 27 * 8 + 27 * 4 + 64))) return rc;
    double* d_in = c->staging.as<double>(); double* d_out = d_in + 64 * 27; int* d_lane = (int*)(d_out + 27);
    HIPCK(c, hipMemcpyAsync(d_in, in, 64 * 27 * 8, hipMemcpyHostToDevice, c->stream));
    hipLaunchKernelGGL(k_selftest_wave_reduce, dim3(1), dim3(64), 0, c->stream, d_in, d_out, d_lane);
    HIPCK(c, hipGetLastError());
    HIPCK(c, hipMemcpyAsync(out, d_out, 27 * 8, hipMemcpyDeviceToHost, c->stream));
    HIPCK(c, hipMemcpyAsync(lane_of, d_lane, 27 * 4, hipMemcpyDeviceToHost, c->stream));
    HIPCK(c, hipStreamSynchronize(c->stream));
    return guard.done();
}
}
```

### icp-variants_amd/csrc/host_launch.hpp

```cpp
namespace {
struct MergeLaunch { RingParams rp; const PoseState* slot; double* partials; hipEvent_t ev_start = nullptr, ev_stop = nullptr; };

constexpr size_t WALK_LDS_BYTES = (size_t)ICP_SHARE_ROWS * BVH_THREADS * 8;
template <int DIM> size_t fused_lds_bytes() {
    const size_t red_bytes = (size_t)(BVH_THREADS / WAVE) * 33 * 8;
    return (WALK_LDS_BYTES > red_bytes ? WALK_LDS_BYTES : red_bytes) + xw_lds_bytes<DIM, BVH_THREADS>();
}
int post_nblocks(int n) { const int nb = (n + POST_THREADS - 1) / POST_THREADS; return nb > POST_BLOCKS ? POST_BLOCKS : nb < 1 ? 1 : nb; }
template <class K> K pick_wide(int Lq, K narrow, K wide) { return Lq <= 8 ? narrow : wide; }

struct QuerySet { const Cloud* cl; const int* sel; int n; int pretransformed; bool use_colors; bool seed_prev; const int* order; bool keep_records = false; };

int ensure_qpack(icp_ctx* c, int n) {
    if ((size_t)n <= c->q_cap && c->qpack.p) return ICP_OK;
    int rc;
    c->q_cap = ((size_t)n + 63) / 64 * 64;
    if ((rc = ensure(c, c->qpack, c->q_cap * 28))) return rc;
    set_view(c->nn_raw, c->qpack.p, c->q_cap * 4); set_view(c->qstate, c->qpack.as<char>() + c->q_cap * 4, c->q_cap * 16);
    set_view(c->qstate2, c->qpack.as<char>() + c->q_cap * 20, c->q_cap * 8);
    return ICP_OK;
}

KnnParams knn_params(const icp_ctx* c, const Cloud& q, const int* sel, int n) {
    KnnParams kp; memset(&kp, 0, sizeof(kp));
    kp.sx = q.x.as<float>(); kp.sy = q.y.as<float>(); kp.sz = q.z.as<float>(); kp.scr = q.cr.as<float>(); kp.scg = q.cg.as<float>(); kp.scb = q.cb.as<float>();
    kp.sel = sel; kp.n = n;
    kp.tx = c->tgt.x.as<float>(); kp.ty = c->tgt.y.as<float>(); kp.tz = c->tgt.z.as<float>();
    kp.tcr = c->tgt.cr.as<float>(); kp.tcg = c->tgt.cg.as<float>(); kp.tcb = c->tgt.cb.as<float>();
    kp.mpad = c->tgt.npad; kp.max_dist = c->prm.max_distance; kp.nseg = 1;
    return kp;
}

PostParams make_post_params(icp_ctx* c, const Cloud& src, const int* sel, int n) {
    const icp_params& p = c->prm;
    PostParams pp;
    pp.sx = src.x.as<float>(); pp.sy = src.y.as<float>(); pp.sz = src.z.as<float>();
    pp.snx = src.nx.as<float>(); pp.sny = src.ny.as<float>(); pp.snz = src.nz.as<float>();
    pp.srgba = src.rgba.as<uint32_t>(); pp.sel = sel; pp.n = n;
    pp.tx = c->tgt.x.as<float>(); pp.ty = c->tgt.y.as<float>(); pp.tz = c->tgt.z.as<float>();
    pp.tnx = c->tgt.nx.as<float>(); pp.tny = c->tgt.ny.as<float>(); pp.tnz = c->tgt.nz.as<float>(); pp.trgba = c->tgt.rgba.as<uint32_t>();
    pp.ps = c->ps.as<PoseState>(); pp.matches = c->matches.as<icp_match_t>();
    pp.metric = p.metric; pp.weighting = p.weighting; pp.rejection = p.rejection;
    pp.max_dist = p.max_distance; pp.cos_reject = c->cos_reject; pp.partials = c->partials.as<double>();
    return pp;
}

template <int DIM>
int launch_bvh_query(icp_ctx* c, Bvh& b, const CoordPtrs<DIM>& cp, const KnnParams& kp, const int* order, int n, const Cloud* fuse, bool keep_records, int* fused_blocks, const MergeLaunch* ml = nullptr) {
    int rc;
    if (!b.valid && (rc = build_bvh<DIM>(c, b, cp))) return rc;
    const BvhViewT<DIM> bv = make_view<DIM>(b, cp);
    const int nb = fuse ? fused_nblocks(n) : (n + BVH_THREADS - 1) / BVH_THREADS;
    if (fuse) {
        if ((rc = ensure(c, c->partials, (size_t)(nb > POST_BLOCKS ? nb : POST_BLOCKS) * NSUM * 8))) return rc;
        PostParams pp = make_post_params(c, *fuse, kp.sel, n);
        KnnParams kf = kp; kf.out = nullptr;
        if (!keep_records) { pp.matches = nullptr; kf.d2_out = nullptr; }
        const size_t lds = fused_lds_bytes<DIM>();
        if (ml) {
            kf.ps = ml->slot; pp.ps = ml->slot; pp.partials = ml->partials; kf.fault = ml->rp.run_fault;
            const auto ring = pick_wide(b.Lq, k_knn_bvh_post_ring<DIM, false>, k_knn_bvh_post_ring<DIM, true>);
            if (ml->ev_start) hipExtLaunchKernelGGL(ring, dim3(nb + ml->rp.n_red), dim3(BVH_THREADS), (uint32_t)lds, c->stream, ml->ev_start, ml->ev_stop, 0, kf, bv, order, pp, ml->rp);
            else hipLaunchKernelGGL(ring, dim3(nb + ml->rp.n_red), dim3(BVH_THREADS), lds, c->stream, kf, bv, order, pp, ml->rp);
        }
        else hipLaunchKernelGGL(pick_wide(b.Lq, k_knn_bvh_post<DIM, false>, k_knn_bvh_post<DIM, true>), dim3(nb), dim3(BVH_THREADS), lds, c->stream, kf, bv, order, pp);
        *fused_blocks = nb;
    } else hipLaunchKernelGGL(k_knn_bvh<DIM>, dim3(nb), dim3(BVH_THREADS), WALK_LDS_BYTES, c->stream, kp, bv, order);
    HIPCK(c, hipGetLastError());
    return ICP_OK;
}

int launch_match(icp_ctx* c, const QuerySet& q, int* fused_blocks = nullptr, const MergeLaunch* ml = nullptr) {
    const icp_params& p = c->prm;
    int rc;
    if (fused_blocks) *fused_blocks = 0;
    if ((rc = ensure(c, c->matches, (size_t)q.n * sizeof(icp_match_t))) || (rc = ensure(c, c->d2, (size_t)q.n * 4))) return rc;
    if (p.matching == ICP_MATCH_PROJECTIVE) {
        ProjParams pp;
        pp.sx = q.cl->x.as<float>(); pp.sy = q.cl->y.as<float>(); pp.sz = q.cl->z.as<float>(); pp.sel = q.sel; pp.n = q.n;
        pp.tx = c->tgt.x.as<float>(); pp.ty = c->tgt.y.as<float>(); pp.tz = c->tgt.z.as<float>();
        pp.width = p.width; pp.height = p.height; pp.fx = p.fx; pp.fy = p.fy; pp.mx = p.cx; pp.my = p.cy; pp.window = 12;
        pp.ps = c->ps.as<PoseState>(); pp.pretransformed = q.pretransformed; pp.max_dist = p.max_distance;
        pp.out = c->matches.as<icp_match_t>(); pp.d2_out = c->d2.as<float>();
        hipLaunchKernelGGL(k_projective, dim3((q.n + 255) / 256), dim3(256), 0, c->stream, pp);
        HIPCK(c, hipGetLastError());
        return ICP_OK;
    }
    KnnParams kp = knn_params(c, *q.cl, q.sel, q.n);
    kp.ps = c->ps.as<PoseState>(); kp.pretransformed = q.pretransformed; kp.fault = &c->ps.as<PoseState>()->fault;
    kp.out = c->matches.as<icp_match_t>(); kp.d2_out = c->d2.as<float>();
    if (p.knn_backend == ICP_KNN_LBVH) {
        if ((rc = ensure_qpack(c, q.n))) return rc;
        kp.nn_raw = c->nn_raw.as<int>(); kp.use_prev = q.seed_prev ? 1 : 0;
#if ICP_DEBUG_STEPS
        if ((rc = ensure(c, c->dbg_steps, (size_t)q.n * 4))) return rc;
        kp.dbg_steps = c->dbg_steps.as<int>(); kp.dbg_waves = fused_nblocks(q.n) * (BVH_THREADS / WAVE);
#endif
        if (p.knn_incremental && !q.pretransformed) {
            kp.qstate = c->qstate.as<float4>(); kp.qstate2 = c->qstate2.as<float2>(); kp.incremental = 1;
        }
        const Cloud* fuse = (fused_blocks != nullptr && p.metric != ICP_METRIC_SYMMETRIC && p.metric != ICP_METRIC_GICP && p.metric != ICP_METRIC_COLORED && !q.pretransformed) ? q.cl : nullptr;
        if (q.use_colors) return launch_bvh_query<6>(c, c->bvh6, target_coords6(c), kp, q.order, q.n, fuse, q.keep_records, fused_blocks, fuse ? ml : nullptr);
        return launch_bvh_query<3>(c, c->bvh, target_coords3(c), kp, q.order, q.n, fuse, q.keep_records, fused_blocks, fuse ? ml : nullptr);
    }
    const int bx = (q.n + WAVE - 1) / WAVE;
    const int nch = kp.mpad / KNN_CH;
    int nseg = 1;
    if (bx < 1024) { nseg = (2048 + bx - 1) / bx; if (nseg > nch / 4) nseg = nch / 4; if (nseg < 1) nseg = 1; }
    kp.nseg = nseg;
    if (nseg > 1) {
        if ((rc = ensure(c, c->best64, (size_t)q.n * 8))) return rc;
        kp.best64 = c->best64.as<unsigned long long>();
        const unsigned long long init = ((unsigned long long)0x7F7FFFFFu << 32) | 0xFFFFFFFFull;
        hipLaunchKernelGGL(k_fill_u64, dim3((q.n + 255) / 256), dim3(256), 0, c->stream, kp.best64, q.n, init);
    }
    if (q.use_colors) hipLaunchKernelGGL(k_knn_brute<6>, dim3(bx, nseg), dim3(256), 0, c->stream, kp);
    else              hipLaunchKernelGGL(k_knn_brute<3>, dim3(bx, nseg), dim3(256), 0, c->stream, kp);
    if (nseg > 1)
        hipLaunchKernelGGL(k_knn_finalize, dim3((q.n + 255) / 256), dim3(256), 0, c->stream, kp.best64, q.n, p.max_distance,
                           c->matches.as<icp_match_t>(), c->d2.as<float>());
    HIPCK(c, hipGetLastError());
    return ICP_OK;
}

int rearm_handover(icp_ctx* c) {
    int rc;
    if ((rc = ensure(c, c->totals, NSUM * 8 + 8))) return rc;
    HIPCK(c, hipMemsetAsync(c->totals.p, 0, NSUM * 8 + 8, c->stream));
    hipLaunchKernelGGL(k_fill_u64, dim3(1), dim3(64), 0, c->stream, c->totals.as<unsigned long long>(), NSUM, TOTAL_SENTINEL);
    HIPCK(c, hipGetLastError());
    return ICP_OK;
}

const int* level_src_orig(icp_ctx* c, const Cloud& src) {
    if (&src == &c->src) return nullptr;
    for (auto& kv : c->levels) if (&kv.second.sorted == &src) return kv.second.sorted_idx.as<int>();
    for (auto& kv : c->nss_held) if (&kv.second.lv.sorted == &src) return kv.second.lv.sorted_idx.as<int>();
    return nullptr;
}

GicpPost gicp_post_params(icp_ctx* c, const Cloud& src) {
    GicpPost g; memset(&g, 0, sizeof(g));
    const bool own_t = c->gicp_opt.covariance_k == 0, own_s = own_t;
    g.tnx = own_t ? c->tgt.nx.as<float>() : c->gicp_n[0][0].as<float>(); g.tny = own_t ? c->tgt.ny.as<float>() : c->gicp_n[0][1].as<float>(); g.tnz = own_t ? c->tgt.nz.as<float>() : c->gicp_n[0][2].as<float>();
    g.snx = own_s ? c->src.nx.as<float>() : c->gicp_n[1][0].as<float>(); g.sny = own_s ? c->src.ny.as<float>() : c->gicp_n[1][1].as<float>(); g.snz = own_s ? c->src.nz.as<float>() : c->gicp_n[1][2].as<float>();
    g.src_orig = level_src_orig(c, src);
    g.one_minus_eps = 1.0 - (double)c->gicp_opt.epsilon;
    return g;
}

ColoredPost colored_post_params(icp_ctx* c) {
    ColoredPost g;
    g.gx = c->col_grad[0].as<float>(); g.gy = c->col_grad[1].as<float>(); g.gz = c->col_grad[2].as<float>();
    g.lambda = (double)c->col_opt.lambda_geometric;
    return g;
}

bool robust_on(const icp_ctx* c) { return c->rob_opt.kernel != ICP_ROBUST_NONE || c->rob_opt.overlap < 1.f; }

int robust_prepare(icp_ctx* c, int slots) {
    int rc;
    if ((rc = ensure(c, c->rob_state, sizeof(RobustState)))) return rc;
    if ((rc = ensure(c, c->rob_stats, (size_t)(slots > 0 ? slots : 1) * sizeof(icp_robust_stats)))) return rc;
    if ((rc = ensure(c, c->rob_keys, (size_t)(c->src.n > 0 ? c->src.n : 1) * 4))) return rc;
    HIPCK(c, hipMemsetAsync(c->rob_state.p, 0, sizeof(RobustState), c->stream));
    return ICP_OK;
}

int launch_robust(icp_ctx* c, const PostParams& pp, int n, icp_robust_stats* d_rstats) {
    int rc;
    if ((rc = ensure(c, c->rob_keys, (size_t)(n > 0 ? n : 1) * 4))) return rc;
    static const float standard[4] = {0.f, 1.345f, 2.3849f, 4.6851f};
    const icp_robust_options& o = c->rob_opt;
    RobustParams rp;
    rp.st = c->rob_state.as<RobustState>(); rp.keys = c->rob_keys.as<unsigned int>(); rp.stats = d_rstats;
    rp.kernel = o.kernel; rp.linear_weight = c->prm.metric == ICP_METRIC_POINT_TO_POINT ? 1 : 0;
    rp.tuning = o.tuning > 0.f ? o.tuning : standard[o.kernel]; rp.sigma = o.sigma; rp.overlap = o.overlap; rp.n = n;
    int nb = (n + ROBUST_THREADS - 1) / ROBUST_THREADS; if (nb > ROBUST_BLOCKS) nb = ROBUST_BLOCKS; if (nb < 1) nb = 1;
    hipLaunchKernelGGL(k_robust_eval, dim3(nb), dim3(ROBUST_THREADS), 0, c->stream, pp, rp);
    hipLaunchKernelGGL(k_robust_select<1>, dim3(nb), dim3(ROBUST_THREADS), 0, c->stream, rp);
    hipLaunchKernelGGL(k_robust_select<2>, dim3(nb), dim3(ROBUST_THREADS), 0, c->stream, rp);
    hipLaunchKernelGGL(k_robust_finish, dim3(1), dim3(ROBUST_THREADS), 0, c->stream, rp);
    hipLaunchKernelGGL(k_robust_apply, dim3(nb), dim3(ROBUST_THREADS), 0, c->stream, pp, rp);
    HIPCK(c, hipGetLastError());
    return ICP_OK;
}

bool reciprocal_on(const icp_ctx* c) { return c->rcp_opt.enabled != 0; }

int reciprocal_check(icp_ctx* c) {
    if (c->prm.color_icp) { c->err = "reciprocal rejection (icp_set_reciprocal_options) does not support color_icp = 1: a 6-D forward search against a 3-D reverse one is not a mutual test"; return ICP_ERR_INVALID_ARG; }
    if (c->lm_on) { c->err = "the non-linear optimiser does not support reciprocal rejection (icp_set_reciprocal_options)"; return ICP_ERR_INVALID_ARG; }
    return ICP_OK;
}

int reciprocal_prepare(icp_ctx* c, int slots) {
    int rc;
    Bvh& b = c->src_bvh;
    if (!b.valid) {
        if ((rc = finite_list(c, c->src, false, c->src_rflag, c->src_finite, &b.n_valid))) return rc;
        b.d_finite = c->src_finite.as<int>(); b.n_ids = c->src.n; b.attrs = nullptr;
        CoordPtrs<3> cp; cp.c[0] = c->src.x.as<float>(); cp.c[1] = c->src.y.as<float>(); cp.c[2] = c->src.z.as<float>();
        if ((rc = build_bvh<3>(c, b, cp))) return rc;
    }
    const size_t bytes = (size_t)(slots > 0 ? slots : 1) * sizeof(icp_reciprocal_stats);
    if ((rc = ensure(c, c->rcp_stats, bytes))) return rc;
    HIPCK(c, hipMemsetAsync(c->rcp_stats.p, 0, bytes, c->stream));
    return ICP_OK;
}

int launch_reciprocal(icp_ctx* c, const QuerySet& q, icp_reciprocal_stats* d_stats) {
    const Bvh& b = c->src_bvh;
    CoordPtrs<3> cp; cp.c[0] = c->src.x.as<float>(); cp.c[1] = c->src.y.as<float>(); cp.c[2] = c->src.z.as<float>();
    RecipParams rp; memset(&rp, 0, sizeof(rp));
    rp.matches = c->matches.as<icp_match_t>(); rp.n = q.n; rp.order = q.order; rp.sel = q.sel; rp.src_orig = level_src_orig(c, *q.cl);
    rp.tx = c->tgt.x.as<float>(); rp.ty = c->tgt.y.as<float>(); rp.tz = c->tgt.z.as<float>();
    rp.ps = c->ps.as<PoseState>(); rp.stats = d_stats;
    rp.tree_depth = 0; while ((1 << rp.tree_depth) < b.Lp) rp.tree_depth++;
    if (c->rcp_naive) {
        int rc;
        for (DevBuf& d : c->rcp_q) if ((rc = ensure(c, d, (size_t)q.n * 4))) return rc;
        if ((rc = ensure(c, c->rcp_nn, (size_t)q.n * sizeof(icp_match_t)))) return rc;
        float* qx = c->rcp_q[0].as<float>(); float* qy = c->rcp_q[1].as<float>(); float* qz = c->rcp_q[2].as<float>();
        hipLaunchKernelGGL(k_reciprocal_queries, dim3((q.n + 255) / 256), dim3(256), 0, c->stream, rp, qx, qy, qz);
        KnnParams kp; memset(&kp, 0, sizeof(kp));
        kp.sx = qx; kp.sy = qy; kp.sz = qz; kp.n = q.n; kp.tx = cp.c[0]; kp.ty = cp.c[1]; kp.tz = cp.c[2]; kp.mpad = c->src.npad;
        kp.ps = rp.ps; kp.pretransformed = 1; kp.max_dist = FLT_MAX; kp.out = c->rcp_nn.as<icp_match_t>(); kp.nseg = 1;
        kp.fault = &c->ps.as<PoseState>()->fault;
        hipLaunchKernelGGL(k_knn_bvh<3>, dim3((q.n + BVH_THREADS - 1) / BVH_THREADS), dim3(BVH_THREADS), WALK_LDS_BYTES, c->stream, kp, make_view<3>(b, cp), q.order);
        hipLaunchKernelGGL(k_reciprocal_compare, dim3((q.n + BVH_THREADS - 1) / BVH_THREADS), dim3(BVH_THREADS), 0, c->stream, rp, c->rcp_nn.as<icp_match_t>());
        HIPCK(c, hipGetLastError());
        return ICP_OK;
    }
    const size_t lds = (size_t)(rp.tree_depth + 1) * BVH_THREADS * 2;
    hipLaunchKernelGGL(k_reciprocal, dim3((q.n + BVH_THREADS - 1) / BVH_THREADS), dim3(BVH_THREADS), lds, c->stream, rp, make_view<3>(b, cp));
    HIPCK(c, hipGetLastError());
    return ICP_OK;
}

int launch_post_and_solve(icp_ctx* c, const Cloud& src, const int* sel, int n, icp_iter_stats* d_stats, double* d_sums_out, int update_pose,
                          hipEvent_t ev_after_post, int fused_blocks = 0, icp_robust_stats* d_rstats = nullptr) {
    const icp_params& p = c->prm;
    int rc;
    if (!fused_blocks && (rc = ensure(c, c->partials, (size_t)POST_BLOCKS * NSUM * 8))) return rc;
    if (!c->totals.p && (rc = rearm_handover(c))) return rc;
    PostParams pp = make_post_params(c, src, sel, n);
    int nb = post_nblocks(n);
    if (d_rstats && !fused_blocks) {
        if ((rc = launch_robust(c, pp, n, d_rstats))) return rc;
        pp.weighting = ICP_WEIGHT_CONSTANT; pp.rejection = 0;
    }
    if (fused_blocks) nb = fused_blocks;
    else if (p.metric == ICP_METRIC_GICP) hipLaunchKernelGGL(k_post_gicp, dim3(nb), dim3(POST_THREADS), 0, c->stream, pp, gicp_post_params(c, src));
    else if (p.metric == ICP_METRIC_COLORED) hipLaunchKernelGGL(k_post_colored, dim3(nb), dim3(POST_THREADS), 0, c->stream, pp, colored_post_params(c));
    else hipLaunchKernelGGL(k_post, dim3(nb), dim3(POST_THREADS), 0, c->stream, pp);
    SolveParams sp; memset(&sp, 0, sizeof(sp));
    sp.partials = c->partials.as<double>(); sp.nblocks = nb; sp.ps = c->ps.as<PoseState>();
    sp.metric = (p.metric == ICP_METRIC_GICP || p.metric == ICP_METRIC_COLORED) ? ICP_METRIC_POINT_TO_PLANE : p.metric;
    sp.totals = c->totals.as<double>(); sp.ticket = (unsigned*)(c->totals.as<double>() + NSUM);
    sp.n_src = n; sp.update_pose = update_pose; sp.spin = 1;
    auto reduce_solve = [&]() { hipLaunchKernelGGL(k_reduce_solve, dim3(NSUM_USED), dim3(SOLVE_THREADS), 0, c->stream, sp); };
    const bool sym = p.metric == ICP_METRIC_SYMMETRIC;
    if (sym) {
        reduce_solve();
        hipLaunchKernelGGL(k_sym_accumulate, dim3(nb), dim3(POST_THREADS), 0, c->stream, pp);
    }
    if (ev_after_post) HIPCK(c, hipEventRecord(ev_after_post, c->stream));
    sp.phase = sym ? 1 : 0; sp.stats = d_stats; sp.sums_out = d_sums_out;
    reduce_solve();
    HIPCK(c, hipGetLastError());
    return ICP_OK;
}

int launch_post_and_lm(icp_ctx* c, const Cloud& src, const int* sel, int n, icp_iter_stats* d_stats, icp_lm_summary* d_summary,
                       hipEvent_t ev_after_post, int fused_blocks) {
    int rc;
    if (!fused_blocks) {
        if ((rc = ensure(c, c->partials, (size_t)POST_BLOCKS * NSUM * 8))) return rc;
        hipLaunchKernelGGL(k_post, dim3(post_nblocks(n)), dim3(POST_THREADS), 0, c->stream, make_post_params(c, src, sel, n));
    }
    if (ev_after_post) HIPCK(c, hipEventRecord(ev_after_post, c->stream));
    const bool fresh = c->lm_state.p == nullptr;
    if ((rc = ensure(c, c->lm_state, sizeof(LmState) + 2 * sizeof(LmRot)))) return rc;
    LmRot* rots = (LmRot*)(c->lm_state.as<char>() + sizeof(LmState));
    if (fresh) hipLaunchKernelGGL(k_lm_init, dim3(1), dim3(WAVE), 0, c->stream, rots);
    if ((rc = ensure(c, c->lm_partials, (size_t)LM_NSUM * LM_BLOCKS * 8))) return rc;
    int nb = (n + LM_THREADS - 1) / LM_THREADS; if (nb > LM_BLOCKS) nb = LM_BLOCKS; if (nb < 1) nb = 1;
    LmEvalParams ep; memset(&ep, 0, sizeof(ep));
    ep.pp = make_post_params(c, src, sel, n); ep.st = c->lm_state.as<LmState>(); ep.partials = c->lm_partials.as<double>();
    static_assert(sizeof(LmState) % 8 == 0, "the evaluation points follow the state");
    LmStepParams sp; memset(&sp, 0, sizeof(sp));
    sp.partials = c->lm_partials.as<double>(); sp.nblocks = nb; sp.st = c->lm_state.as<LmState>(); sp.rot = rots + 1; sp.opt = c->lm_opt;
    sp.ps = c->ps.as<PoseState>(); sp.stats = d_stats; sp.summary = d_summary; sp.n_src = n;
    for (int k = 0; k <= c->lm_opt.max_num_iterations; k++) {
        ep.first = sp.first = k == 0 ? 1 : 0; ep.rot = rots + (k == 0 ? 0 : 1);
        hipLaunchKernelGGL(k_lm_eval, dim3(nb), dim3(LM_THREADS), 0, c->stream, ep);
        hipLaunchKernelGGL(k_lm_step, dim3(1), dim3(WAVE), 0, c->stream, sp);
    }
    HIPCK(c, hipGetLastError());
    return ICP_OK;
}

int enqueue_rmse(icp_ctx* c, float* d_out) {
    int rc;
    if ((rc = ensure(c, c->rmse_partials, 256 * 2 * 8))) return rc;
    hipLaunchKernelGGL(k_rmse_partial, dim3(256), dim3(256), 0, c->stream, c->conv_src.x.as<float>(), c->conv_src.y.as<float>(), c->conv_src.z.as<float>(),
                       c->conv_ref.x.as<float>(), c->conv_ref.y.as<float>(), c->conv_ref.z.as<float>(), c->conv_n, c->ps.as<PoseState>(), c->rmse_partials.as<double>());
    hipLaunchKernelGGL(k_rmse_finish, dim3(1), dim3(64), 0, c->stream, c->rmse_partials.as<double>(), 256, d_out);
    HIPCK(c, hipGetLastError());
    return ICP_OK;
}

static int enqueue_fontana(icp_ctx* c, float* d_out) {
    int rc;
    if ((rc = ensure(c, c->fontana_partials, (size_t)256 * 5 * 8))) return rc;
    double* cpart = c->fontana_partials.as<double>(); double* epart = cpart + 256 * 4;
    hipLaunchKernelGGL(k_fontana_centroid, dim3(256), dim3(256), 0, c->stream, c->conv_src.x.as<float>(), c->conv_src.y.as<float>(), c->conv_src.z.as<float>(),
                       c->conv_n, c->ps.as<PoseState>(), cpart);
    hipLaunchKernelGGL(k_fontana_error, dim3(256), dim3(256), 0, c->stream, c->conv_src.x.as<float>(), c->conv_src.y.as<float>(), c->conv_src.z.as<float>(),
                       c->conv_ref.x.as<float>(), c->conv_ref.y.as<float>(), c->conv_ref.z.as<float>(), c->conv_n, c->ps.as<PoseState>(), cpart, 256, epart);
    hipLaunchKernelGGL(k_fontana_finish, dim3(1), dim3(64), 0, c->stream, epart, 256, c->conv_n, d_out);
    HIPCK(c, hipGetLastError());
    return ICP_OK;
}
}
```

### icp-variants_amd/csrc/host_loop.hpp

```cpp
namespace {
struct RunPlan {
    std::vector<int> factors, ns; std::vector<const Cloud*> clouds; std::vector<const int*> sels, orders;
    bool sorted_levels = false;
    bool fixed_sets = true;
    int iters() const { return (int)factors.size(); }
    bool seeded(int i) const { return i > 0 && factors[i] == factors[i - 1] && ns[i - 1] > 0 && fixed_sets; }
};

int nss_buckets(icp_ctx* c) {
    const int grid = c->nss_opt.grid, n = c->src.n;
    if (c->nss_bkt_grid == grid) return ICP_OK;
    int rc;
    for (auto& kv : c->nss_levels) release(kv.second);
    c->nss_levels.clear();
    const Cloud& s = c->src;
    if ((rc = ensure(c, c->nss_bkt, (size_t)n * 2))) return rc;
    hipLaunchKernelGGL(k_nss_bucket, dim3((n + 255) / 256), dim3(256), 0, c->stream, s.x.as<float>(), s.y.as<float>(), s.z.as<float>(),
                       s.nx.as<float>(), s.ny.as<float>(), s.nz.as<float>(), n, grid, c->nss_bkt.as<unsigned short>());
    HIPCK(c, hipGetLastError());
    c->nss_bkt_grid = grid;
    return ICP_OK;
}
int nss_level(icp_ctx* c, int factor, const int* base, int n_base, const NssLevel** out) {
    auto it = c->nss_levels.find(factor);
    if (it == c->nss_levels.end()) {
        NssLevel nl; int rc;
        const int nb = 6 * c->nss_opt.grid * c->nss_opt.grid, nblocks = (n_base + NSS_LEVEL_THREADS - 1) / NSS_LEVEL_THREADS;
        nl.n_base = n_base; nl.max_long = n_base / NSS_LONG; nl.max_chunks = n_base / NSS_CHUNK + nl.max_long;
        const int n_table = (nb + 1) * nblocks;
        if ((rc = ensure(c, nl.cand, (size_t)n_base * 4)) || (rc = ensure(c, nl.seg, (NSS_MAX_BUCKETS + 2) * 4)) || (rc = ensure(c, nl.longs, sizeof(NssLongs)))) { release(nl); return rc; }
        if ((rc = ensure(c, c->nss_table, (size_t)n_table * 4)) || (rc = ensure(c, c->nss_total, 4))) { release(nl); return rc; }
        const unsigned short* bkt = c->nss_bkt.as<unsigned short>();
        hipLaunchKernelGGL(k_nss_level_hist, dim3(nblocks), dim3(NSS_LEVEL_THREADS), 0, c->stream, base, n_base, bkt, nb, c->nss_table.as<int>(), nblocks);
        hipLaunchKernelGGL(k_select_scan, dim3(1), dim3(1024), 0, c->stream, c->nss_table.as<int>(), n_table, c->nss_total.as<int>());
        hipLaunchKernelGGL(k_nss_level_scatter, dim3(nblocks), dim3(NSS_LEVEL_THREADS), 0, c->stream, base, n_base, bkt, nb, c->nss_table.as<int>(), nblocks, nl.cand.as<int>());
        hipLaunchKernelGGL(k_nss_level_segs, dim3(1), dim3(NSS_QUOTA_THREADS), 0, c->stream, c->nss_table.as<int>(), nblocks, nb, nl.seg.as<int>(), nl.longs.as<NssLongs>());
        if (hipGetLastError() != hipSuccess) { release(nl); c->err = "normal-space sampling: a level launch failed"; return ICP_ERR_HIP; }
        it = c->nss_levels.emplace(factor, std::move(nl)).first;
    }
    *out = &it->second;
    return ICP_OK;
}
int nss_draw(icp_ctx* c, const NssLevel& nl, const int* base, uint32_t word0, int n_draws, int max_long_all, size_t cap) {
    const icp_params& p = c->prm;
    const int nb = 6 * c->nss_opt.grid * c->nss_opt.grid, n = nl.n_base, nblk = (n + 255) / 256, stride = nblk + 1;
    unsigned int* quota = c->nss_quota.as<unsigned int>() + (size_t)word0 * NSS_ROW; unsigned int* thr = c->nss_thr.as<unsigned int>() + (size_t)word0 * NSS_ROW;
    NssLongState* state = c->nss_state.as<NssLongState>() + (size_t)word0 * max_long_all;
    unsigned int* hist = c->nss_hist.as<unsigned int>() + (size_t)word0 * max_long_all * NSS_BINS;
    int* counts = c->sel_counts.as<int>() + word0; int* blocks = c->sel_blocks.as<int>();
    const int* cand = nl.cand.as<int>(); const int* seg = nl.seg.as<int>(); const NssLongs* longs = nl.longs.as<NssLongs>();
    const unsigned short* bkt = c->nss_bkt.as<unsigned short>();
    const uint32_t seed = p.selection_seed;
    const dim3 B(NSS_THREADS);
    hipLaunchKernelGGL(k_nss_quota, dim3(n_draws), dim3(NSS_QUOTA_THREADS), 0, c->stream, seg, nb, p.selection_proba, seed, word0, quota, thr);
    hipLaunchKernelGGL(k_nss_select_small, dim3(nb, n_draws), B, 0, c->stream, cand, seg, seed, word0, quota, thr);
    if (nl.max_long > 0) {
        const dim3 gh(nl.max_chunks, n_draws), gp(nl.max_long, n_draws);
        hipLaunchKernelGGL(k_nss_long_hist<1>, gh, B, 0, c->stream, cand, seg, longs, max_long_all, seed, word0, quota, state, hist);
        hipLaunchKernelGGL(k_nss_long_pick<1>, gp, B, 0, c->stream, seg, longs, max_long_all, quota, state, hist, thr);
        hipLaunchKernelGGL(k_nss_long_hist<2>, gh, B, 0, c->stream, cand, seg, longs, max_long_all, seed, word0, quota, state, hist);
        hipLaunchKernelGGL(k_nss_long_pick<2>, gp, B, 0, c->stream, seg, longs, max_long_all, quota, state, hist, thr);
        hipLaunchKernelGGL(k_nss_long_hist<3>, gh, B, 0, c->stream, cand, seg, longs, max_long_all, seed, word0, quota, state, hist);
        hipLaunchKernelGGL(k_nss_long_pick<3>, gp, B, 0, c->stream, seg, longs, max_long_all, quota, state, hist, thr);
    }
    hipLaunchKernelGGL(k_nss_count, dim3(nblk, n_draws), dim3(256), 0, c->stream, base, n, bkt, seed, word0, quota, thr, blocks, stride);
    hipLaunchKernelGGL(k_nss_scan, dim3(n_draws), dim3(1024), 0, c->stream, blocks, nblk, stride, counts);
    hipLaunchKernelGGL(k_nss_scatter, dim3(nblk, n_draws), dim3(256), 0, c->stream, base, n, bkt, seed, word0, quota, thr, blocks, stride, c->sel_lists.as<int>() + (size_t)word0 * cap, cap);
    HIPCK(c, hipGetLastError());
    return ICP_OK;
}
int nss_plan(icp_ctx* c, RunPlan& pl) {
    const icp_params& p = c->prm;
    const int iters = pl.iters(); int rc;
    const bool held = c->nss_opt.resample == 0;
    if (!c->src.has_normals) { c->err = "normal-space sampling (selection = 2) needs normals on the source"; return ICP_ERR_INVALID_ARG; }
    if (c->nss_held_stale || c->nss_held_proba != p.selection_proba || c->nss_held_seed != p.selection_seed) drop_nss(c, true);
    c->nss_held_proba = p.selection_proba; c->nss_held_seed = p.selection_seed;
    if ((rc = nss_buckets(c))) return rc;
    const size_t cap = (size_t)c->src.n; const int max_long_all = c->src.n / NSS_LONG;
    const size_t hist_bytes = (size_t)iters * max_long_all * NSS_BINS * 4;
    if ((rc = ensure(c, c->sel_lists, (size_t)iters * cap * 4)) || (rc = ensure(c, c->sel_counts, (size_t)iters * 4))) return rc;
    if ((rc = ensure(c, c->sel_blocks, (size_t)iters * ((cap + 255) / 256 + 1) * 4))) return rc;
    if ((rc = ensure(c, c->nss_quota, (size_t)iters * NSS_ROW * 4)) || (rc = ensure(c, c->nss_thr, (size_t)iters * NSS_ROW * 4))) return rc;
    if ((rc = ensure(c, c->nss_state, (size_t)iters * (max_long_all + 1) * sizeof(NssLongState)))) return rc;
    if (hist_bytes > c->nss_hist.cap || !c->nss_hist.p) {
        if ((rc = ensure(c, c->nss_hist, hist_bytes))) return rc;
        HIPCK(c, hipMemsetAsync(c->nss_hist.p, 0, c->nss_hist.cap, c->stream));
    }
    HIPCK(c, hipMemsetAsync(c->sel_counts.p, 0, (size_t)iters * 4, c->stream));
    std::vector<int> first((size_t)iters);
    std::vector<char> drawn((size_t)iters, 0);
    for (int i = 0; i < iters; i++) {
        first[i] = i;
        if (held) for (int j = 0; j < i; j++) if (pl.factors[j] == pl.factors[i]) { first[i] = j; break; }
    }
    for (int i = 0; i < iters;) {
        int run = 1;
        if (held) {
            auto it = c->nss_held.find(pl.factors[i]);
            if (first[i] != i || (it != c->nss_held.end() && it->second.word == (uint32_t)i)) { i++; continue; }
            if (it != c->nss_held.end()) { release(it->second.lv); c->nss_held.erase(it); }
        } else while (i + run < iters && pl.factors[i + run] == pl.factors[i]) run++;
        if (pl.ns[i] > 0) {
            const NssLevel* nl = nullptr;
            if ((rc = nss_level(c, pl.factors[i], pl.sels[i], pl.ns[i], &nl))) return rc;
            if ((rc = nss_draw(c, *nl, pl.sels[i], (uint32_t)i, run, max_long_all, cap))) return rc;
        }
        for (int k = 0; k < run; k++) drawn[i + k] = 1;
        i += run;
    }
    std::vector<int> counts((size_t)iters);
    HIPCK(c, hipMemcpyAsync(counts.data(), c->sel_counts.p, (size_t)iters * 4, hipMemcpyDeviceToHost, c->stream));
    HIPCK(c, hipStreamSynchronize(c->stream));
    for (int i = 0; i < iters; i++) {
        if (!held) { pl.sels[i] = c->sel_lists.as<int>() + (size_t)i * cap; pl.ns[i] = counts[i]; pl.orders[i] = nullptr; continue; }
        if (drawn[i]) {
            NssHeld& h = c->nss_held[pl.factors[i]];
            h.word = (uint32_t)i; h.lv.n = counts[i];
            if ((rc = ensure(c, h.lv.idx, (size_t)(counts[i] > 0 ? counts[i] : 1) * 4))) return rc;
            if (counts[i] > 0) HIPCK(c, hipMemcpyAsync(h.lv.idx.p, c->sel_lists.as<int>() + (size_t)i * cap, (size_t)counts[i] * 4, hipMemcpyDeviceToDevice, c->stream));
        }
        Level& lv = c->nss_held[pl.factors[i]].lv;
        pl.ns[i] = lv.n; pl.orders[i] = nullptr;
        if (pl.sorted_levels) { pl.sels[i] = nullptr; if ((rc = get_sorted_held(c, lv, &pl.clouds[i]))) return rc; }
        else pl.sels[i] = lv.idx.as<int>();
    }
    return ICP_OK;
}

int make_plan(icp_ctx* c, bool single, RunPlan& pl) {
    const icp_params& p = c->prm;
    int rc;
    c->sel_last.clear();
    if (single) pl.factors.assign(1, 0);
    else {
        int32_t cnt = 0;
        if ((rc = icp_schedule(&p, c->src.n, nullptr, 0, &cnt))) { c->err = "multires with n_iterations < 1 never terminates in the reference"; return rc; }
        pl.factors.resize((size_t)cnt);
        if (cnt > 0) icp_schedule(&p, c->src.n, pl.factors.data(), cnt, &cnt);
    }
    const std::vector<int>& factors = pl.factors; std::vector<int>& ns = pl.ns; std::vector<const int*>& sels = pl.sels; std::vector<const int*>& orders = pl.orders;
    const int iters = pl.iters();
    const bool nss = !single && p.selection == ICP_SELECT_NORMAL_SPACE;
    const bool resample = !single && p.selection == ICP_SELECT_RANDOM;
    pl.fixed_sets = !resample && !(nss && c->nss_opt.resample != 0);
    sels.assign((size_t)iters, nullptr); ns.assign((size_t)iters, c->src.n); orders.assign((size_t)iters, nullptr); pl.clouds.assign((size_t)iters, &c->src);
    pl.sorted_levels = p.matching == ICP_MATCH_KNN && p.knn_backend == ICP_KNN_LBVH && pl.fixed_sets;
    if (iters == 0) return ICP_OK;
    for (int i = 0; i < iters; i++) {
        if (pl.sorted_levels && !nss) { if ((rc = get_sorted_level(c, factors[i], &pl.clouds[i], &ns[i]))) return rc; }
        else if (factors[i] > 0) { if ((rc = get_level(c, factors[i], &sels[i], &ns[i], nullptr))) return rc; }
    }
    if (nss && (rc = nss_plan(c, pl))) return rc;
    if (resample) {
        double th = (double)p.selection_proba * 4294967296.0;
        const int take_all = th >= 4294967296.0 ? 1 : 0;
        const uint32_t threshold = th <= 0.0 ? 0u : (take_all ? 0xFFFFFFFFu : (uint32_t)th);
        const size_t cap = (size_t)c->src.n;
        if ((rc = ensure(c, c->sel_lists, (size_t)iters * cap * 4))) return rc;
        if ((rc = ensure(c, c->sel_counts, (size_t)iters * 4))) return rc;
        if ((rc = ensure(c, c->sel_blocks, (size_t)((cap + 255) / 256 + 1) * 4))) return rc;
        for (int i = 0; i < iters; i++) {
            const int nb = (ns[i] + 255) / 256;
            int* out = c->sel_lists.as<int>() + (size_t)i * cap;
            if (ns[i] > 0) {
                hipLaunchKernelGGL(k_select_count, dim3(nb), dim3(256), 0, c->stream, sels[i], ns[i], p.selection_seed, (uint32_t)i, threshold, take_all, c->sel_blocks.as<int>());
                hipLaunchKernelGGL(k_select_scan, dim3(1), dim3(1024), 0, c->stream, c->sel_blocks.as<int>(), nb, c->sel_counts.as<int>() + i);
                hipLaunchKernelGGL(k_select_scatter, dim3(nb), dim3(256), 0, c->stream, sels[i], ns[i], p.selection_seed, (uint32_t)i, threshold, take_all, c->sel_blocks.as<int>(), out);
            } else HIPCK(c, hipMemsetAsync(c->sel_counts.as<int>() + i, 0, 4, c->stream));
            sels[i] = out; orders[i] = nullptr;
        }
        HIPCK(c, hipGetLastError());
        std::vector<int> counts((size_t)iters);
        HIPCK(c, hipMemcpyAsync(counts.data(), c->sel_counts.p, (size_t)iters * 4, hipMemcpyDeviceToHost, c->stream));
        HIPCK(c, hipStreamSynchronize(c->stream));
        for (int i = 0; i < iters; i++) ns[i] = counts[i];
    }
    if (resample || nss) {
        c->sel_last.resize((size_t)iters);
        for (int i = 0; i < iters; i++) {
            const int* list = sels[i];
            if (nss && pl.fixed_sets) list = c->nss_held[factors[i]].lv.idx.as<int>();
            c->sel_last[(size_t)i] = std::make_pair(ns[i] > 0 ? list : nullptr, ns[i]);
        }
    }
    return ICP_OK;
}

int finish_records(const RunPlan& pl, int n_run, icp_iter_stats* hs, const float* pose_in, bool rmse, bool fontana, icp_iter_stats* out, int max_out) {
    int status = ICP_OK;
    for (int i = 0; i < n_run; i++) {
        const bool empty = pl.ns[i] <= 0;
        if (empty) { hs[i].n_src = 0; hs[i].n_valid = 0; hs[i].status = ICP_ERR_NO_CORRESPONDENCES; memcpy(hs[i].pose, i ? hs[i - 1].pose : pose_in, 64); }
        if (empty || !rmse) hs[i].rmse = -1.f;
        if (empty || !fontana) hs[i].benchmark_error = -1.f;
        if (hs[i].status != ICP_OK && status == ICP_OK) status = hs[i].status;
        if (out && i < max_out) out[i] = hs[i];
    }
    return status;
}

struct Ring { PoseState* slots; unsigned long long* trows; int* run_fault; size_t slot_bytes; };
int make_ring(icp_ctx* c, int n_slots, int n_rows, int nbmax, int* fault, Ring& r) {
    static_assert(sizeof(PoseState) == 128, "a pose slot is 16 granules");
    int rc;
    r.slot_bytes = (size_t)n_slots * POSE_REPLICAS * POSE_REPLICA_STRIDE; const size_t tot_bytes = (size_t)n_rows * NSUM * 8;
    if ((rc = ensure(c, c->ring, r.slot_bytes + tot_bytes + (fault ? 0 : 64)))) return rc;
    if ((rc = ensure(c, c->partials, (size_t)nbmax * NSUM * 8))) return rc;
    if ((rc = ensure(c, c->partials2, (size_t)nbmax * NSUM * 8))) return rc;
    r.slots = c->ring.as<PoseState>(); r.trows = (unsigned long long*)(c->ring.as<char>() + r.slot_bytes);
    r.run_fault = fault ? fault : (int*)(c->ring.as<char>() + r.slot_bytes + tot_bytes);
    return ICP_OK;
}
double* ring_partials(const icp_ctx* c, int j) { return (j & 1) ? c->partials2.as<double>() : c->partials.as<double>(); }
RingParams ring_params(const icp_ctx* c, const Ring& r, int j, int n_prev, PoseState* ps_out) {
    RingParams rp; memset(&rp, 0, sizeof(rp));
    rp.run_fault = r.run_fault;
    if (j > 0) {
        rp.n_red = NSUM_USED;
        rp.red_partials = ring_partials(c, j - 1); rp.red_nblocks = fused_nblocks(n_prev);
        rp.totals_row = r.trows + (size_t)(j - 1) * NSUM; rp.ps_in = loop_slot(r.slots, j - 1, 0); rp.ps_out = ps_out; rp.n_src = n_prev;
    }
    return rp;
}

struct RunTail {
    PoseState final_pose;
    int merged_fault, spare[3];
    int merged_cvg[12];
    char unused[64];
    int cvg_state[CONV_STATE_BYTES / 4];
    icp_convergence_step* trace() { return (icp_convergence_step*)(this + 1); }
    static constexpr size_t used_bytes(bool cvg, int n_trace) { return cvg ? sizeof(RunTail) + (size_t)n_trace * sizeof(icp_convergence_step) : offsetof(RunTail, unused); }
};
static_assert(offsetof(RunTail, merged_fault) == 128 && offsetof(RunTail, merged_cvg) == 144 && offsetof(RunTail, unused) == 192 && offsetof(RunTail, cvg_state) == 256 && sizeof(RunTail) == 512, "the layout the device was handed");

struct IterEvents { hipEvent_t start = nullptr, matched = nullptr, posted = nullptr, end = nullptr; };
struct LoopRun {
    RunPlan pl; bool lm, robust, recip, rmse, fontana, cvg; std::vector<char> sampled, eligible; std::vector<IterEvents> ev; int n_enqueued = 0;
    size_t pin_stats = 256, pin_tail, pin_lm, pin_bytes, stats_bytes;
    void lay_out(int iters, bool with_lm, bool with_cvg) {
        auto pad = [](size_t b) { return (b + 255) & ~(size_t)255; };
        const size_t trace_pad = with_cvg ? pad((size_t)iters * sizeof(icp_convergence_step)) : 0;
        pin_tail = pin_stats + pad((size_t)iters * sizeof(icp_iter_stats)); pin_lm = pin_tail + sizeof(RunTail) + trace_pad;
        pin_bytes = pin_lm + (with_lm ? (size_t)iters * sizeof(icp_lm_summary) : 0);
        stats_bytes = records_bytes() + (with_cvg ? sizeof(RunTail) + trace_pad : RunTail::used_bytes(false, 0));
    }
    size_t records_bytes() const { return pin_tail - pin_stats; }
    RunTail* dev_tail(const icp_ctx* c) const { return (RunTail*)(c->stats.as<char>() + records_bytes()); }
    icp_iter_stats* host_records(const icp_ctx* c) const { return (icp_iter_stats*)(c->pinned.as<char>() + pin_stats); }
    RunTail* host_tail(const icp_ctx* c) const { return (RunTail*)(c->pinned.as<char>() + pin_tail); }
    icp_lm_summary* host_lm(const icp_ctx* c) const { return (icp_lm_summary*)(c->pinned.as<char>() + pin_lm); }
};
#ifndef ICP_CONVERGE_CHUNK
#define ICP_CONVERGE_CHUNK 2
#endif
constexpr int CONVERGE_CHUNK = ICP_CONVERGE_CHUNK;
ConvergeParams converge_params(const icp_ctx* c, const LoopRun& r, int i, int* words) {
    ConvergeParams cp; memset(&cp, 0, sizeof(cp));
    if (!r.cvg) return cp;
    const icp_convergence_options& o = c->cvg_opt;
    cp.on = 1; cp.eligible = r.eligible[(size_t)i]; cp.index = i; cp.min_iterations = o.min_iterations; cp.patience = o.patience;
    cp.rotation_eps = o.rotation_eps; cp.translation_eps = o.translation_eps;
    cp.trace = r.dev_tail(c)->trace(); cp.words = words;
    return cp;
}
hipEvent_t loop_event(const icp_ctx* c, int i, int k) { return c->events[(size_t)2 + 4 * i + k]; }

int enqueue_merged(icp_ctx* c, LoopRun& r) {
    const icp_params& p = c->prm; const RunPlan& pl = r.pl;
    const int iters = pl.iters(); RunTail* tail = r.dev_tail(c);
    int rc, nbmax = POST_BLOCKS;
    for (int i = 0; i < iters; i++) { const int nb = fused_nblocks(pl.ns[i]); if (nb > nbmax) nbmax = nb; }
    Ring ring;
    if ((rc = make_ring(c, iters + 1, iters, nbmax, &tail->merged_fault, ring))) return rc;
    const int n_init = (iters + 1) * POSE_REPLICAS * 16 + iters * NSUM + 16;
    hipLaunchKernelGGL(k_run_init, dim3((n_init + 255) / 256), dim3(256), 0, c->stream, c->ps.as<PoseState>(), ring.slots, iters + 1, ring.trows, iters * NSUM, ring.run_fault, 16);
    auto reducer = [&](int i) {
        RingParams rp = ring_params(c, ring, i, i > 0 ? pl.ns[i - 1] : 0, loop_slot(ring.slots, i, 0));
        if (i > 0) { rp.stats = c->stats.as<icp_iter_stats>() + (i - 1); rp.cv = converge_params(c, r, i - 1, tail->merged_cvg); }
        if (i == iters) rp.final_out = &tail->final_pose;
        return rp;
    };
    HIPCK(c, hipEventRecord(c->events[0], c->stream));
    for (int i = 0; i < iters; i++) {
        QuerySet q{pl.clouds[i], pl.sels[i], pl.ns[i], 0, p.color_icp != 0 && p.matching == ICP_MATCH_KNN, pl.seeded(i), pl.orders[i]};
        MergeLaunch ml; ml.rp = reducer(i); ml.slot = loop_slot(ring.slots, i, 0); ml.partials = ring_partials(c, i);
        if (r.sampled[i]) { r.ev[i].start = ml.ev_start = loop_event(c, i, 0); r.ev[i].matched = ml.ev_stop = loop_event(c, i, 1); }
        int fused = 0;
        if ((rc = launch_match(c, q, &fused, &ml))) return rc;
        if (!fused) { c->err = "merged loop: the matcher did not take the fused path"; return ICP_ERR_HIP; }
    }
    hipLaunchKernelGGL(k_ring_reduce_solve, dim3(NSUM_USED), dim3(RING_THREADS), 0, c->stream, reducer(iters));
    HIPCK(c, hipGetLastError());
    if (r.sampled[iters - 1]) { r.ev[iters - 1].end = loop_event(c, iters - 1, 3); HIPCK(c, hipEventRecord(r.ev[iters - 1].end, c->stream)); }
    HIPCK(c, hipEventRecord(c->events[1], c->stream));
    r.n_enqueued = iters;
    HIPCK(c, hipMemcpyAsync(r.host_records(c), c->stats.p, r.records_bytes() + RunTail::used_bytes(r.cvg, iters), hipMemcpyDeviceToHost, c->stream));
    return ICP_OK;
}

int enqueue_separate(icp_ctx* c, LoopRun& r) {
    const icp_params& p = c->prm; const RunPlan& pl = r.pl;
    const int iters = pl.iters(); int rc;
    if ((rc = rearm_handover(c))) return rc;
    RunTail* tail = r.dev_tail(c); RunTail* htail = r.host_tail(c);
    if (r.cvg) {
        hipLaunchKernelGGL(k_converge_init, dim3(1), dim3(64), 0, c->stream, c->ps.as<PoseState>(), tail->cvg_state);
        HIPCK(c, hipGetLastError());
    }
    HIPCK(c, hipEventRecord(c->events[0], c->stream));
    int n_enq = 0;
    for (int i = 0; i < iters; i++) {
        if (r.cvg && i > 0 && i % CONVERGE_CHUNK == 0) {
            const int* stop = &htail->cvg_state[CONV_STOPPED];
            HIPCK(c, hipMemcpyAsync((void*)stop, &tail->cvg_state[CONV_STOPPED], 4, hipMemcpyDeviceToHost, c->stream));
            HIPCK(c, hipStreamSynchronize(c->stream));
            if (*stop) break;
        }
        n_enq = i + 1;
        icp_iter_stats* d_st = c->stats.as<icp_iter_stats>() + i;
        const bool ev = r.sampled[i] != 0;
        if (ev) {
            r.ev[i].start = (i > 0 && r.sampled[i - 1]) ? loop_event(c, i - 1, 3) : loop_event(c, i, 0);
            r.ev[i].matched = loop_event(c, i, 1); r.ev[i].end = loop_event(c, i, 3);
            HIPCK(c, hipEventRecord(loop_event(c, i, 0), c->stream));
        }
        if (pl.ns[i] > 0) {
            QuerySet q{pl.clouds[i], pl.sels[i], pl.ns[i], 0, p.color_icp != 0 && p.matching == ICP_MATCH_KNN, pl.seeded(i), pl.orders[i], r.lm};
            int fused = 0;
            if ((rc = launch_match(c, q, !r.robust && !r.recip ? &fused : nullptr))) return rc;
            if (r.recip && (rc = launch_reciprocal(c, q, c->rcp_stats.as<icp_reciprocal_stats>() + i))) return rc;
            if (ev) HIPCK(c, hipEventRecord(r.ev[i].matched, c->stream));
            if (ev && !fused) r.ev[i].posted = loop_event(c, i, 2);
            if (r.lm) rc = launch_post_and_lm(c, *pl.clouds[i], pl.sels[i], pl.ns[i], d_st, c->lm_sums.as<icp_lm_summary>() + i, r.ev[i].posted, fused);
            else rc = launch_post_and_solve(c, *pl.clouds[i], pl.sels[i], pl.ns[i], d_st, nullptr, 1, r.ev[i].posted, fused, r.robust ? c->rob_stats.as<icp_robust_stats>() + i : nullptr);
            if (rc) return rc;
        } else if (ev) HIPCK(c, hipEventRecord(r.ev[i].matched, c->stream));
        if (r.rmse && (rc = enqueue_rmse(c, &d_st->rmse))) return rc;
        if (r.fontana && (rc = enqueue_fontana(c, &d_st->benchmark_error))) return rc;
        if (r.cvg) {
            hipLaunchKernelGGL(k_converge_step, dim3(1), dim3(64), 0, c->stream, converge_params(c, r, i, tail->cvg_state), c->ps.as<PoseState>(), pl.ns[i] > 0 ? d_st : nullptr);
            HIPCK(c, hipGetLastError());
        }
        if (ev) HIPCK(c, hipEventRecord(r.ev[i].end, c->stream));
    }
    r.n_enqueued = n_enq;
    HIPCK(c, hipEventRecord(c->events[1], c->stream));
    HIPCK(c, hipMemcpyAsync(r.host_records(c), c->stats.p, (size_t)n_enq * sizeof(icp_iter_stats), hipMemcpyDeviceToHost, c->stream));
    HIPCK(c, hipMemcpyAsync(&htail->final_pose, c->ps.p, sizeof(PoseState), hipMemcpyDeviceToHost, c->stream));
    if (r.cvg) HIPCK(c, hipMemcpyAsync(htail->cvg_state, tail->cvg_state, RunTail::used_bytes(true, n_enq) - offsetof(RunTail, cvg_state), hipMemcpyDeviceToHost, c->stream));
    if (r.lm) HIPCK(c, hipMemcpyAsync(r.host_lm(c), c->lm_sums.p, (size_t)n_enq * sizeof(icp_lm_summary), hipMemcpyDeviceToHost, c->stream));
    return ICP_OK;
}

int run_loop(icp_ctx* c, float pose_inout[16], icp_iter_stats* stats, int32_t max_stats, int32_t* n_run, bool single, bool try_merged) {
    const icp_params& p = c->prm;
    int rc;
    DrainOnError guard(c);
    if ((rc = set_device(c))) return rc;
    if ((rc = check_ready(c, true, true))) return rc;
    if ((rc = gicp_prepare(c))) return rc;
    if ((rc = colored_prepare(c))) return rc;
    LoopRun r{};
    const RunPlan& pl = r.pl;
    if ((rc = make_plan(c, single, r.pl))) return rc;
    const int iters = pl.iters();
    if (n_run) *n_run = 0;
    const bool lm = r.lm = c->lm_on;
    const bool robust = r.robust = robust_on(c);
    const bool recip = r.recip = reciprocal_on(c);
    c->lm_last.clear(); c->rob_last.clear(); c->rcp_last.clear();
    const bool cvg = r.cvg = !single && c->cvg_opt.enabled != 0;
    if (!single) { c->cvg_trace.clear(); c->cvg_last = icp_convergence_result{0, 0, iters, -1.f, -1.f}; }
    if (robust && lm) { c->err = "the non-linear optimiser does not support robust mode (icp_set_robust_options)"; return ICP_ERR_INVALID_ARG; }
    if (recip && (rc = reciprocal_check(c))) return rc;
    if (iters == 0) return guard.done();
    if (robust && (rc = robust_prepare(c, iters))) return rc;
    if (recip && (rc = reciprocal_prepare(c, iters))) return rc;
    r.lay_out(iters, lm, cvg);
    if ((rc = ensure_pinned(c, r.pin_bytes))) return rc;
    if (lm && (rc = ensure(c, c->lm_sums, (size_t)iters * sizeof(icp_lm_summary)))) return rc;
    float pose_in[16]; memcpy(pose_in, pose_inout, 64);
    if ((rc = write_pose(c, pose_inout))) return rc;
    if ((rc = ensure(c, c->stats, r.stats_bytes))) return rc;
    r.eligible.assign((size_t)iters, 0);
    for (int i = 0; i < iters; i++) r.eligible[(size_t)i] = pl.factors[i] == pl.factors[iters - 1] && (i == 0 || pl.factors[i] == pl.factors[i - 1]);
    if ((rc = ensure_events(c, (size_t)iters * 4 + 2))) return rc;
    const bool rmse = r.rmse = (p.record_rmse & 1) && c->conv_n > 0;
    const bool fontana = r.fontana = (p.record_rmse & 2) && c->conv_n > 0;
    bool merged = try_merged && !lm && !robust && !recip && !single && iters >= 2 && pl.sorted_levels && p.metric == ICP_METRIC_POINT_TO_PLANE && !rmse && !fontana;
    for (int i = 0; merged && i < iters; i++) if (pl.ns[i] <= 0) merged = false;
    const int tmode = c->stage_timing;
    r.sampled.assign((size_t)iters, 0); r.ev.assign((size_t)iters, IterEvents());
    for (int i = 0; i < iters; i++) r.sampled[i] = tmode == 1 || (tmode > 1 && (i + (int)(c->timing_phase % (unsigned)tmode)) % tmode == 0);
    c->timing_phase++;
    if ((rc = merged ? enqueue_merged(c, r) : enqueue_separate(c, r))) return rc;
    std::vector<icp_robust_stats> rob((size_t)(robust ? iters : 0));
    if (robust) HIPCK(c, hipMemcpyAsync(rob.data(), c->rob_stats.p, (size_t)iters * sizeof(icp_robust_stats), hipMemcpyDeviceToHost, c->stream));
    std::vector<icp_reciprocal_stats> rcp((size_t)(recip ? iters : 0));
    if (recip) HIPCK(c, hipMemcpyAsync(rcp.data(), c->rcp_stats.p, (size_t)iters * sizeof(icp_reciprocal_stats), hipMemcpyDeviceToHost, c->stream));
    HIPCK(c, hipStreamSynchronize(c->stream));
    c->rcp_last.swap(rcp);
    for (int i = 0; robust && i < iters; i++) if (pl.ns[i] <= 0) rob[(size_t)i] = icp_robust_stats{0, 0, -1.f, -1.f};
    c->rob_last.swap(rob);
    RunTail* htail = r.host_tail(c);
    const PoseState* hp = &htail->final_pose;
    if (merged) {
        c->merged_runs++;
        const int rf = htail->merged_fault;
        if ((hp->fault && hp->fault != SLOT_STOPPED) || rf) {
            c->merged_fallbacks++;
            if (c->trace) fprintf(stderr, "[icp_hip] merged loop gave up: slot fault %d, abort word %d -> the run again with separate launches\n", hp->fault, rf);
            guard.ok = true;
            memcpy(pose_inout, pose_in, 64);
            return run_loop(c, pose_inout, stats, max_stats, n_run, single, false);
        }
    }
    int n_done = iters; bool stopped = false;
    if (cvg) {
        const int* cw = merged ? htail->merged_cvg : htail->cvg_state;
        if (cw[CONV_STOPPED]) {
            stopped = true; n_done = cw[CONV_RUN];
            if (n_done < 1 || n_done > r.n_enqueued) { c->err = "the device reports a stop outside the iterations that were enqueued"; return ICP_ERR_HIP; }
            if (!merged) hp = (const PoseState*)(cw + CONV_FINAL);
        }
    }
    memcpy(pose_inout, hp->pose, 64);
    if (!merged && hp->fault) { c->err = "reduction hand-over timed out on the device (k_reduce_solve)"; return ICP_ERR_HIP; }
    if (lm) {
        c->lm_last.resize((size_t)n_done);
        memcpy(c->lm_last.data(), r.host_lm(c), (size_t)n_done * sizeof(icp_lm_summary));
        for (int i = 0; i < n_done; i++)
            if (pl.ns[i] <= 0) { memset(&c->lm_last[(size_t)i], 0, sizeof(icp_lm_summary)); c->lm_last[(size_t)i].termination = ICP_LM_NO_RESIDUALS; }
    }
    if (robust) c->rob_last.resize((size_t)n_done);
    if (recip) c->rcp_last.resize((size_t)n_done);
    const int status = finish_records(pl, n_done, r.host_records(c), pose_in, rmse, fontana, stats, max_stats);
    if (n_run) *n_run = n_done;
    if (!single) { c->cvg_last.converged = stopped; c->cvg_last.iterations_run = n_done; }
    if (cvg) {
        const icp_convergence_step* tr = htail->trace();
        c->cvg_trace.assign(tr, tr + n_done);
        c->cvg_last.rotation = tr[n_done - 1].rotation; c->cvg_last.translation = tr[n_done - 1].translation;
    }
    icp_timing& t = c->timing; memset(&t, 0, sizeof(t)); t.iterations = n_done;
    c->it_match_ms.assign((size_t)n_done, -1.f); c->it_post_ms.assign((size_t)n_done, -1.f); c->it_solve_ms.assign((size_t)n_done, -1.f);
    double ev_match = 0, ev_post = 0, ev_solve = 0; int n_ev = 0;
    for (int i = 0; i < n_done; i++) {
        if (!r.sampled[i]) continue;
        n_ev++;
        const IterEvents& e = r.ev[i];
        float a = 0, b = 0, d = 0;
        HIPCK(c, hipEventElapsedTime(&a, e.start, e.matched));
        if (e.posted) HIPCK(c, hipEventElapsedTime(&b, e.matched, e.posted));
        if (e.end) HIPCK(c, hipEventElapsedTime(&d, e.posted ? e.posted : e.matched, e.end));
        ev_match += a; ev_post += b; ev_solve += d;
        c->it_match_ms[(size_t)i] = a; c->it_post_ms[(size_t)i] = b; c->it_solve_ms[(size_t)i] = d;
        if (c->trace) fprintf(stderr, "[icp_hip] it %2d  n %d  match %.4f  post %.4f  solve %.4f ms\n", i, pl.ns[i], a, b, d);
    }
    if (n_ev > 0) {
        const double f = (double)n_done / n_ev;
        t.match_ms += ev_match * f; t.weight_reject_build_ms += ev_post * f; t.solve_ms += ev_solve * f;
    }
    t.sampled_iterations = n_ev;
    float tot = 0; HIPCK(c, hipEventElapsedTime(&tot, c->events[0], c->events[1])); t.total_ms = tot;
    if (status != ICP_OK) c->err = "no valid correspondences in at least one iteration (reference would hang in ASSERT)";
    guard.ok = true;
    return status;
}
}

int icp_schedule(const icp_params* p, int32_t n_src, int32_t* factors_out, int32_t max_out, int32_t* count_out) {
    if (!p || !count_out || n_src < 0) return ICP_ERR_INVALID_ARG;
    int cnt = 0;
    if (!p->multires) {
        for (int i = 0; i < p->n_iterations; i++) { if (factors_out && cnt < max_out) factors_out[cnt] = 0; cnt++; }
    } else {
        if (p->n_iterations < 1) return ICP_ERR_INVALID_ARG;
        float res = 1.0f; int osz = n_src;
        while (1) { osz = (int)(osz / 2.0); if (osz < 100) break; res *= 2.0f; }
        for (int i = 0;; ++i) {
            if (factors_out && cnt < max_out) factors_out[cnt] = (int)res;
            cnt++;
            if (res == 1.0f && i >= p->n_iterations - 1) break;
            if (res == 1.0f) continue;
            res /= 2.0f; if (res < 1.0f) res = 1.0f;
        }
    }
    *count_out = cnt;
    return ICP_OK;
}

int icp_iterate(icp_ctx* c, float pose_inout[16], icp_iter_stats* stats) {
    if (!c || !pose_inout) { if (c) c->err = "icp_iterate: bad argument"; return ICP_ERR_INVALID_ARG; }
    return run_loop(c, pose_inout, stats, stats ? 1 : 0, nullptr, true, c->merge_loop);
}

int icp_run(icp_ctx* c, float pose_inout[16], icp_iter_stats* stats, int32_t max_stats, int32_t* n_iterations_run) {
    if (!c || !pose_inout) { if (c) c->err = "icp_run: bad argument"; return ICP_ERR_INVALID_ARG; }
    return run_loop(c, pose_inout, stats, stats ? max_stats : 0, n_iterations_run, false, c->merge_loop);
}

int icp_query_matches(icp_ctx* c, const float* transformed_xyz, const uint8_t* rgba, int32_t n, icp_match_t* out) {
    if (!c || !transformed_xyz || !out || n <= 0) { if (c) c->err = "icp_query_matches: bad argument"; return ICP_ERR_INVALID_ARG; }
    int rc;
    DrainOnError guard(c);
    if ((rc = set_device(c))) return rc;
    if ((rc = check_ready(c, false, false))) return rc;
    const bool colors = rgba != nullptr;
    if (c->prm.matching == ICP_MATCH_KNN && colors && !c->tgt.has_colors) {
        c->err = "index built without colours: call queryMatches without colours";
        return ICP_ERR_COLOR_MISMATCH;
    }
    if ((rc = upload_cloud(c, c->qry, transformed_xyz, nullptr, rgba, n, false))) return rc;
    QuerySet q{&c->qry, nullptr, n, 1, colors && c->prm.matching == ICP_MATCH_KNN, false, nullptr};
    if ((rc = launch_match(c, q))) return rc;
    HIPCK(c, hipMemcpyAsync(out, c->matches.p, (size_t)n * sizeof(icp_match_t), hipMemcpyDeviceToHost, c->stream));
    HIPCK(c, hipStreamSynchronize(c->stream));
    return guard.done();
}

int icp_match(icp_ctx* c, const float pose[16], icp_match_t* out, float* d2_out) {
    if (!c || !pose || !out) { if (c) c->err = "icp_match_t: bad argument"; return ICP_ERR_INVALID_ARG; }
    int rc;
    DrainOnError guard(c);
    if ((rc = set_device(c))) return rc;
    if ((rc = check_ready(c, true, false))) return rc;
    if ((rc = write_pose(c, pose))) return rc;
    const int* full_order = nullptr;
    if ((rc = get_full_order(c, &full_order))) return rc;
    QuerySet q{&c->src, nullptr, c->src.n, 0, c->prm.color_icp != 0 && c->prm.matching == ICP_MATCH_KNN, false, full_order};
    if ((rc = launch_match(c, q))) return rc;
    HIPCK(c, hipMemcpyAsync(out, c->matches.p, (size_t)q.n * sizeof(icp_match_t), hipMemcpyDeviceToHost, c->stream));
    if (d2_out) HIPCK(c, hipMemcpyAsync(d2_out, c->d2.p, (size_t)q.n * 4, hipMemcpyDeviceToHost, c->stream));
    HIPCK(c, hipStreamSynchronize(c->stream));
    return guard.done();
}

int icp_correspond(icp_ctx* c, const float pose[16], icp_match_t* out, double* sums_out, int32_t* n_valid_out) {
    if (!c || !pose) { if (c) c->err = "icp_correspond: bad argument"; return ICP_ERR_INVALID_ARG; }
    int rc;
    DrainOnError guard(c);
    if ((rc = set_device(c))) return rc;
    if ((rc = check_ready(c, true, true))) return rc;
    if ((rc = gicp_prepare(c))) return rc;
    if ((rc = colored_prepare(c))) return rc;
    const bool robust = robust_on(c);
    const bool recip = reciprocal_on(c);
    c->rob_last.clear(); c->rcp_last.clear();
    if (recip && (rc = reciprocal_check(c))) return rc;
    if (robust && (rc = robust_prepare(c, 1))) return rc;
    if (recip && (rc = reciprocal_prepare(c, 1))) return rc;
    if ((rc = write_pose(c, pose))) return rc;
    const int* full_order = nullptr;
    if ((rc = get_full_order(c, &full_order))) return rc;
    QuerySet q{&c->src, nullptr, c->src.n, 0, c->prm.color_icp != 0 && c->prm.matching == ICP_MATCH_KNN, false, full_order};
    if ((rc = launch_match(c, q))) return rc;
    if (recip && (rc = launch_reciprocal(c, q, c->rcp_stats.as<icp_reciprocal_stats>()))) return rc;
    if ((rc = ensure(c, c->sums, NSUM * 8))) return rc;
    if ((rc = rearm_handover(c))) return rc;
    if ((rc = launch_post_and_solve(c, c->src, nullptr, q.n, nullptr, c->sums.as<double>(), 0, nullptr, 0, robust ? c->rob_stats.as<icp_robust_stats>() : nullptr))) return rc;
    double hs[NSUM]; int fault = 0;
    icp_robust_stats rs; icp_reciprocal_stats rcs;
    if (out) HIPCK(c, hipMemcpyAsync(out, c->matches.p, (size_t)q.n * sizeof(icp_match_t), hipMemcpyDeviceToHost, c->stream));
    HIPCK(c, hipMemcpyAsync(hs, c->sums.p, NSUM * 8, hipMemcpyDeviceToHost, c->stream));
    HIPCK(c, hipMemcpyAsync(&fault, &c->ps.as<PoseState>()->fault, 4, hipMemcpyDeviceToHost, c->stream));
    if (robust) HIPCK(c, hipMemcpyAsync(&rs, c->rob_stats.p, sizeof(rs), hipMemcpyDeviceToHost, c->stream));
    if (recip) HIPCK(c, hipMemcpyAsync(&rcs, c->rcp_stats.p, sizeof(rcs), hipMemcpyDeviceToHost, c->stream));
    HIPCK(c, hipStreamSynchronize(c->stream));
    if (robust) c->rob_last.assign(1, rs);
    if (recip) c->rcp_last.assign(1, rcs);
    if (fault) { c->err = "reduction hand-over timed out on the device (k_reduce_solve)"; return ICP_ERR_HIP; }
    if (sums_out) { memset(sums_out, 0, 64 * 8); memcpy(sums_out, hs, NSUM * 8); }
    if (n_valid_out) *n_valid_out = (int32_t)hs[SUM_N];
    return guard.done();
}

int icp_match_seeded(icp_ctx* c, const float* poses, int32_t n_poses, icp_match_t* out, float* d2_out) {
    if (!c || !poses || n_poses <= 0) { if (c) c->err = "icp_match_seeded: bad argument"; return ICP_ERR_INVALID_ARG; }
    const icp_params& p = c->prm;
    if (p.metric == ICP_METRIC_GICP) { c->err = "icp_match_seeded: GICP has no fused matcher"; return ICP_ERR_INVALID_ARG; }
    if (p.metric == ICP_METRIC_COLORED) { c->err = "icp_match_seeded: colored ICP has no fused matcher"; return ICP_ERR_INVALID_ARG; }
    if (robust_on(c)) { c->err = "icp_match_seeded: robust mode (icp_set_robust_options) has no fused matcher"; return ICP_ERR_INVALID_ARG; }
    if (reciprocal_on(c)) { c->err = "icp_match_seeded: reciprocal rejection (icp_set_reciprocal_options) has no fused matcher"; return ICP_ERR_INVALID_ARG; }
    if (p.matching != ICP_MATCH_KNN || p.knn_backend != ICP_KNN_LBVH || p.metric == ICP_METRIC_SYMMETRIC) {
        c->err = "icp_match_seeded: needs k-NN matching on the LBVH backend with the fused point-to-point / point-to-plane matcher"; return ICP_ERR_INVALID_ARG;
    }
    int rc;
    DrainOnError guard(c);
    if ((rc = set_device(c))) return rc;
    if ((rc = check_ready(c, true, true))) return rc;
    const Cloud* cloud = nullptr; int n = 0;
    if ((rc = get_sorted_level(c, 0, &cloud, &n))) return rc;
    const bool ring = c->merge_loop && !c->lm_on && p.metric == ICP_METRIC_POINT_TO_PLANE;
    std::vector<unsigned long long> slot_image;
    Ring rg{nullptr, nullptr, nullptr, 0};
    if (ring) {
        const int nb = fused_nblocks(n), n_rows = n_poses > 1 ? n_poses - 1 : 1;
        if ((rc = make_ring(c, n_poses + 1, n_rows, nb > POST_BLOCKS ? nb : POST_BLOCKS, nullptr, rg))) return rc;
        slot_image.assign(rg.slot_bytes / 8, GRANULE_EMPTY);
        for (int j = 0; j < n_poses; j++) {
            PoseState ps; memset(&ps, 0, sizeof(ps)); memcpy(ps.pose, poses + (size_t)16 * j, 64); normal_matrix_from_pose(ps.pose, ps.nmat);
            const unsigned long long* g = (const unsigned long long*)&ps;
            for (int r = 0; r < POSE_REPLICAS; r++)
                for (int q = 0; q < 16; q++)
                    slot_image[((size_t)j * POSE_REPLICAS + r) * (POSE_REPLICA_STRIDE / 8) + q] = g[q] == GRANULE_EMPTY ? g[q] ^ 1ull : g[q];
        }
        HIPCK(c, hipMemcpyAsync(rg.slots, slot_image.data(), rg.slot_bytes, hipMemcpyHostToDevice, c->stream));
        const int n_init = n_rows * NSUM + 16;
        hipLaunchKernelGGL(k_run_init, dim3((n_init + 255) / 256), dim3(256), 0, c->stream, nullptr, rg.slots, 0, rg.trows, n_rows * NSUM, rg.run_fault, 16);
        HIPCK(c, hipGetLastError());
    }
    for (int j = 0; j < n_poses; j++) {
        if (!ring && (rc = write_pose(c, poses + (size_t)16 * j))) return rc;
        QuerySet q{cloud, nullptr, n, 0, p.color_icp != 0, j > 0, nullptr, j == n_poses - 1};
        MergeLaunch ml; memset(&ml.rp, 0, sizeof(ml.rp)); ml.slot = nullptr; ml.partials = nullptr;
        if (ring) {
            ml.rp = ring_params(c, rg, j, n, loop_slot(rg.slots, n_poses, 0));
            ml.slot = loop_slot(rg.slots, j, 0); ml.partials = ring_partials(c, j);
        }
        int fused = 0;
        if ((rc = launch_match(c, q, &fused, ring ? &ml : nullptr))) return rc;
        if (!fused) { c->err = "icp_match_seeded: the matcher did not take the fused path"; return ICP_ERR_INVALID_ARG; }
        if (!ring) {
            int hf = 0;
            HIPCK(c, hipMemcpyAsync(&hf, &c->ps.as<PoseState>()->fault, 4, hipMemcpyDeviceToHost, c->stream));
            HIPCK(c, hipStreamSynchronize(c->stream));
            if (hf) { c->err = "icp_match_seeded: a bounded wait of the matcher ran out (k_knn_bvh_post)"; return ICP_ERR_HIP; }
        }
    }
    if (ring) {
        int hf = 0;
        HIPCK(c, hipMemcpyAsync(&hf, rg.run_fault, 4, hipMemcpyDeviceToHost, c->stream));
        HIPCK(c, hipStreamSynchronize(c->stream));
        if (hf) { c->err = "icp_match_seeded: a bounded wait of the merged launches ran out (k_knn_bvh_post_ring)"; return ICP_ERR_HIP; }
    }
    std::vector<int> pos((size_t)n); std::vector<icp_match_t> m((size_t)n); std::vector<float> d((size_t)n);
    HIPCK(c, hipMemcpyAsync(pos.data(), c->levels[0].sorted_idx.p, (size_t)n * 4, hipMemcpyDeviceToHost, c->stream));
    HIPCK(c, hipMemcpyAsync(m.data(), c->matches.p, (size_t)n * sizeof(icp_match_t), hipMemcpyDeviceToHost, c->stream));
    HIPCK(c, hipMemcpyAsync(d.data(), c->d2.p, (size_t)n * 4, hipMemcpyDeviceToHost, c->stream));
    HIPCK(c, hipStreamSynchronize(c->stream));
    for (int t = 0; t < n; t++) {
        if (out) out[pos[(size_t)t]] = m[(size_t)t];
        if (d2_out) d2_out[pos[(size_t)t]] = d[(size_t)t];
    }
    return guard.done();
}
```

Before: 34970.

## Replace per-iteration HIP events in merged loop with device wall-clock stamps

In the merged ring loop, per-iteration timing now comes from wall_clock64 stamps written by the kernels instead of hipEvents and hipExtLaunchKernelGGL event launches. The initial pose is passed by value into k_run_init rather than copied from host with a separate memcpy, and the stats/fault words are written directly to mapped pinned memory. This is meant to remove event-record and memcpy submissions from the enqueue path, at the cost of extra global stores per block and a max-reduction in one reducer block.

```diff
diff --git a/icp-variants_amd/csrc/dev_fused.hpp b/icp-variants_amd/csrc/dev_fused.hpp
--- a/icp-variants_amd/csrc/dev_fused.hpp
+++ b/icp-variants_amd/csrc/dev_fused.hpp
@@ -258,6 +258,7 @@
         for (int q = 0; q < 9; q++) Nm[q] = nc[q];
     }
     const int tid = threadIdx.x, lane = tid & 63, w = tid >> 6;
+    if constexpr (MERGED) { if (rp.st.t0 && blockIdx.x == 0 && tid == 0) *rp.st.t0 = wall_clock64(); }
     const int lb = xcd_contiguous_block(mblock, mgrid);
     const int wave_slot = fused_wave_slot(lb, w, mgrid);
     const int t = wave_slot * BVH_QPW + lane;
@@ -288,6 +289,7 @@
     }
     double* partials = pp.partials;
     fused_block_epilogue(kp, pp, o, bvh_lbq, tid, wave_slot, [=](int a, double v) { partials[(size_t)a * mgrid + lb] = v; });
+    if constexpr (MERGED) { if (rp.st.block_t1 && tid == 0) rp.st.block_t1[lb] = wall_clock64(); }
 }
 template <int DIM, bool WIDE>
 __global__ __launch_bounds__(BVH_THREADS, DIM == 3 ? ICP_FUSED_WAVES : 4) void k_knn_bvh_post(const KnnParams kp, const BvhViewT<DIM> bv, const int* __restrict__ qorder, const PostParams pp) {
diff --git a/icp-variants_amd/csrc/dev_solve.hpp b/icp-variants_amd/csrc/dev_solve.hpp
--- a/icp-variants_amd/csrc/dev_solve.hpp
+++ b/icp-variants_amd/csrc/dev_solve.hpp
@@ -425,20 +425,28 @@
 __device__ __host__ __forceinline__ PoseState* loop_slot(PoseState* base, int g, int replica) {
     return (PoseState*)((char*)base + ((size_t)g * POSE_REPLICAS + (size_t)replica) * POSE_REPLICA_STRIDE);
 }
-__global__ void k_run_init(const PoseState* __restrict__ src, PoseState* slots, int n_slots, unsigned long long* totals, int n_totals, int* zero_words, int n_zero) {
+__global__ void k_run_init(const PoseState src, PoseState* ps_copy, PoseState* slots, int n_slots, unsigned long long* totals, int n_totals, int* zero_words, int n_zero,
+                           unsigned long long* stamps, int n_stamps) {
     const int t = blockIdx.x * blockDim.x + threadIdx.x;
     const int n_slot_granules = n_slots * POSE_REPLICAS * 16;
     if (t < n_slot_granules) {
         const int g = t / (POSE_REPLICAS * 16), r = (t / 16) % POSE_REPLICAS, q = t & 15;
         unsigned long long* dst = (unsigned long long*)loop_slot(slots, g, r) + q;
-        *dst = g == 0 ? ((const unsigned long long*)src)[q] : ~0ull;
+        *dst = g == 0 ? ((const unsigned long long*)&src)[q] : ~0ull;
+        if (g == 0 && r == 0 && ps_copy) ((unsigned long long*)ps_copy)[q] = ((const unsigned long long*)&src)[q];
     } else if (t < n_slot_granules + n_totals) totals[t - n_slot_granules] = ~0ull;
     else if (t < n_slot_granules + n_totals + n_zero) zero_words[t - n_slot_granules - n_totals] = 0;
+    else if (t < n_slot_granules + n_totals + n_zero + n_stamps) stamps[t - n_slot_granules - n_totals - n_zero] = 0ull;
 }
 constexpr unsigned long long GRANULE_EMPTY = ~0ull;
 #ifndef ICP_RING_SLEEP
 #define ICP_RING_SLEEP 4
 #endif
+struct RingStamps {
+    unsigned long long* t0; unsigned long long* block_t1;
+    const unsigned long long* prev_block_t1; unsigned long long* prev_t1;
+    unsigned long long* end;
+};
 struct RingParams {
     const double* red_partials; int red_nblocks;
     unsigned long long* totals_row;
@@ -446,9 +454,11 @@
     PoseState* ps_out;
     icp_iter_stats* stats; int n_src;
     PoseState* final_out;
+    int* words_out;
     int* run_fault;
     int n_red;
     ConvergeParams cv;
+    RingStamps st;
 };
 __device__ __forceinline__ unsigned long long granule_of(unsigned int lo, unsigned int hi) {
     const unsigned long long g = ((unsigned long long)hi << 32) | lo;
@@ -464,6 +474,17 @@
 #else
 #define RING_STAMP(a, j)
 #endif
+__device__ __forceinline__ void ring_close(const RingParams& rp) {
+    if (threadIdx.x != 0) return;
+    if (rp.words_out) {
+        int wds[16];
+#pragma unroll
+        for (int k = 0; k < 16; k++) wds[k] = __hip_atomic_load(rp.run_fault + k, __ATOMIC_RELAXED, __HIP_MEMORY_SCOPE_AGENT);
+#pragma unroll
+        for (int k = 0; k < 16; k++) rp.words_out[k] = wds[k];
+    }
+    if (rp.st.end) *rp.st.end = wall_clock64();
+}
 __device__ __forceinline__ void ring_reduce_solve(const RingParams& rp) {
     __shared__ double tot[NSUM];
     __shared__ double wsum[4];
@@ -471,9 +492,11 @@
     __shared__ int give_up;
     const int tid = threadIdx.x, lane = tid & 63, w = tid >> 6, a = blockIdx.x;
     RING_STAMP(a, 0);
+    if (a == 0 && tid == 0 && rp.st.t0) *rp.st.t0 = wall_clock64();
     if (a == 0 && rp.ps_in->fault) {
         { const unsigned int* src = (const unsigned int*)rp.ps_in; for (int q = tid; q < 16 * POSE_REPLICAS; q += RING_THREADS) __hip_atomic_store((unsigned long long*)loop_slot(rp.ps_out, 0, q >> 4) + (q & 15), granule_of(src[2 * (q & 15)], src[2 * (q & 15) + 1]), __ATOMIC_RELAXED, __HIP_MEMORY_SCOPE_AGENT);
           if (rp.final_out && tid < 32) ((unsigned int*)rp.final_out)[tid] = src[tid]; }
+        ring_close(rp);
         return;
     }
     {
@@ -506,6 +529,16 @@
         __hip_atomic_store(rp.totals_row + a, granule_of((unsigned int)bits, (unsigned int)(bits >> 32)), __ATOMIC_RELAXED, __HIP_MEMORY_SCOPE_AGENT);
     }
     RING_STAMP(a, 2);
+    if (a == 1 && rp.st.prev_t1) {
+        static_assert(RING_THREADS == 2 * WAVE, "two wave maxima meet below");
+        __shared__ unsigned long long tmax[RING_THREADS / WAVE];
+        unsigned long long m = 0ull;
+        for (int b = tid; b < rp.red_nblocks; b += RING_THREADS) { const unsigned long long v = rp.st.prev_block_t1[b]; m = v > m ? v : m; }
+        for (int off = 32; off > 0; off >>= 1) { const unsigned long long v = __shfl_down(m, off, WAVE); m = v > m ? v : m; }
+        if (lane == 0) tmax[w] = m;
+        __syncthreads();
+        if (tid == 0) *rp.st.prev_t1 = tmax[0] > tmax[1] ? tmax[0] : tmax[1];
+    }
     if (a != 0) return;
     if (tid == 0) give_up = 0;
     __syncthreads();
@@ -553,6 +586,7 @@
         if (tid < 16) rp.stats->pose[tid] = __uint_as_float(slot_words[tid]);
         if (tid == 16) { rp.stats->n_src = rp.n_src; rp.stats->n_valid = (int)n; rp.stats->rmse = -1.f; rp.stats->benchmark_error = -1.f; rp.stats->status = status; }
     }
+    ring_close(rp);
 }
 __global__ __launch_bounds__(RING_THREADS) void k_ring_reduce_solve(const RingParams rp) { ring_reduce_solve(rp); }
 
diff --git a/icp-variants_amd/csrc/host_ctx.hpp b/icp-variants_amd/csrc/host_ctx.hpp
--- a/icp-variants_amd/csrc/host_ctx.hpp
+++ b/icp-variants_amd/csrc/host_ctx.hpp
@@ -26,7 +26,7 @@
 };
 static_assert(!std::is_copy_constructible<DevBuf>::value && !std::is_copy_assignable<DevBuf>::value, "a copied DevBuf would be freed twice");
 struct PinBuf {
-    void* p = nullptr; size_t cap = 0;
+    void* p = nullptr; size_t cap = 0; void* dev = nullptr;
     PinBuf() = default; PinBuf(const PinBuf&) = delete; PinBuf& operator=(const PinBuf&) = delete;
     ~PinBuf() { if (p) (void)hipHostFree(p); }
     template <class T> T* as() const { return (T*)p; }
@@ -76,6 +76,7 @@
     hipStream_t stream = nullptr;
     int stage_timing = 1;
     unsigned timing_phase = 0;
+    double wall_ticks_per_ms = 0;
     PinBuf pinned;
     bool trace = false;
     bool merge_loop = true;
@@ -126,6 +127,7 @@
     DevBuf qstate, qstate2;
     DevBuf dbg_steps;
     DevBuf ps, matches, d2, best64, nn_raw, partials, partials2, ring, totals, sums, stats, staging, rmse_partials, rmse_out, fontana_partials;
+    DevBuf block_t1;
     Cloud conv_src, conv_ref; int conv_n = 0;
     PinBuf depth_pin[2]; DevBuf depth_dev[2]; Event depth_up[2]; bool depth_pending[2] = {false, false};
     DevBuf depth_blocks, track_rmse;
@@ -166,10 +168,11 @@
 }
 int ensure_pin(icp_ctx* c, PinBuf& b, size_t bytes, size_t min_bytes, size_t slack_div) {
     if (bytes <= b.cap && b.p) return ICP_OK;
-    if (b.p) { HIPCK(c, hipHostFree(b.p)); b.p = nullptr; b.cap = 0; }
+    if (b.p) { HIPCK(c, hipHostFree(b.p)); b.p = nullptr; b.cap = 0; b.dev = nullptr; }
     const size_t want = bytes < min_bytes ? min_bytes : bytes + (slack_div ? bytes / slack_div : 0);
     HIPCK(c, hipHostMalloc(&b.p, want, hipHostMallocDefault));
     b.cap = want;
+    HIPCK(c, hipHostGetDevicePointer(&b.dev, b.p, 0));
     return ICP_OK;
 }
 int ensure_pinned(icp_ctx* c, size_t bytes) { return ensure_pin(c, c->pinned, bytes, 4096, 0); }
@@ -290,11 +293,14 @@
     return compact_flagged(c, flag.as<uint8_t>(), cl.n, 1, list, n_out);
 }
 
-int write_pose_via(icp_ctx* c, PoseState* h, const float pose[16]) {
-    int rc;
+void make_pose_state(const float pose[16], PoseState* h) {
     memset(h, 0, sizeof(*h));
     memcpy(h->pose, pose, 64);
     normal_matrix_from_pose(h->pose, h->nmat);
+}
+int write_pose_via(icp_ctx* c, PoseState* h, const float pose[16]) {
+    int rc;
+    make_pose_state(pose, h);
     if ((rc = ensure(c, c->ps, sizeof(PoseState)))) return rc;
     HIPCK(c, hipMemcpyAsync(c->ps.p, h, sizeof(*h), hipMemcpyHostToDevice, c->stream));
     return ICP_OK;
diff --git a/icp-variants_amd/csrc/host_debug.hpp b/icp-variants_amd/csrc/host_debug.hpp
--- a/icp-variants_amd/csrc/host_debug.hpp
+++ b/icp-variants_amd/csrc/host_debug.hpp
@@ -38,6 +38,21 @@
     if (waves_per_block) *waves_per_block = BVH_THREADS / WAVE;
     if (lb < 0 || lb >= mgrid || w < 0 || w >= BVH_THREADS / WAVE) return -1;
     return icpdev::fused_wave_slot(lb, w, mgrid);
+}
+int icp_debug_stamp_times(const uint64_t* t0, const uint64_t* t1, int32_t iters, int32_t n_done, int32_t mode, uint32_t phase, double ticks_per_ms,
+                          icp_timing* timing, float* match_ms, float* post_ms, float* solve_ms) {
+    if (!t0 || !t1 || !timing || iters < 1 || n_done < 1 || n_done > iters || mode < 0 || !(ticks_per_ms > 0)) return ICP_ERR_INVALID_ARG;
+    std::vector<char> sampled;
+    sample_iterations(mode, phase, iters, sampled);
+    stamps_to_timing((const unsigned long long*)t0, (const unsigned long long*)t1, iters, n_done, sampled.data(), ticks_per_ms, timing, match_ms, post_ms, solve_ms);
+    return ICP_OK;
+}
+int icp_debug_wall_clock_khz(icp_ctx* c, int32_t* khz) {
+    if (!c || !khz) return ICP_ERR_INVALID_ARG;
+    int v = 0;
+    HIPCK(c, hipDeviceGetAttribute(&v, hipDeviceAttributeWallClockRate, c->device));
+    *khz = v;
+    return ICP_OK;
 }
 __global__ void k_debug_pos_of(const icpdev::TgtRec* recs, const int* pos_of, int n_slots, int* bad) {
     const int i = blockIdx.x * blockDim.x + threadIdx.x;
@@ -124,10 +139,9 @@
         for (int k : two) { r.pl.factors.push_back(pl.factors[k]); r.pl.ns.push_back(pl.ns[k]); r.pl.clouds.push_back(pl.clouds[k]); r.pl.sels.push_back(pl.sels[k]); r.pl.orders.push_back(pl.orders[k]); }
         r.lay_out(2, false, false);
         if ((rc = ensure_pinned(c, r.pin_bytes))) return rc;
-        if ((rc = write_pose(c, pose))) return rc;
+        make_pose_state(pose, &r.ps_in);
         if ((rc = ensure(c, c->stats, r.stats_bytes))) return rc;
-        if ((rc = ensure_events(c, 2 * 4 + 2))) return rc;
-        r.sampled.assign(2, 0); r.eligible.assign(2, 0); r.ev.assign(2, IterEvents());
+        r.sampled.assign(2, 0); r.eligible.assign(2, 0);
         if ((rc = enqueue_merged(c, r))) return rc;
         unsigned long long row[NSUM];
         HIPCK(c, hipMemcpyAsync(row, c->ring.as<char>() + (size_t)3 * POSE_REPLICAS * POSE_REPLICA_STRIDE, NSUM * 8, hipMemcpyDeviceToHost, c->stream));
diff --git a/icp-variants_amd/csrc/host_launch.hpp b/icp-variants_amd/csrc/host_launch.hpp
--- a/icp-variants_amd/csrc/host_launch.hpp
+++ b/icp-variants_amd/csrc/host_launch.hpp
@@ -1,5 +1,5 @@
 namespace {
-struct MergeLaunch { RingParams rp; const PoseState* slot; double* partials; hipEvent_t ev_start = nullptr, ev_stop = nullptr; };
+struct MergeLaunch { RingParams rp; const PoseState* slot; double* partials; };
 
 constexpr size_t WALK_LDS_BYTES = (size_t)ICP_SHARE_ROWS * BVH_THREADS * 8;
 template <int DIM> size_t fused_lds_bytes() {
@@ -60,8 +60,7 @@
         if (ml) {
             kf.ps = ml->slot; pp.ps = ml->slot; pp.partials = ml->partials; kf.fault = ml->rp.run_fault;
             const auto ring = pick_wide(b.Lq, k_knn_bvh_post_ring<DIM, false>, k_knn_bvh_post_ring<DIM, true>);
-            if (ml->ev_start) hipExtLaunchKernelGGL(ring, dim3(nb + ml->rp.n_red), dim3(BVH_THREADS), (uint32_t)lds, c->stream, ml->ev_start, ml->ev_stop, 0, kf, bv, order, pp, ml->rp);
-            else hipLaunchKernelGGL(ring, dim3(nb + ml->rp.n_red), dim3(BVH_THREADS), lds, c->stream, kf, bv, order, pp, ml->rp);
+            hipLaunchKernelGGL(ring, dim3(nb + ml->rp.n_red), dim3(BVH_THREADS), lds, c->stream, kf, bv, order, pp, ml->rp);
         }
         else hipLaunchKernelGGL(pick_wide(b.Lq, k_knn_bvh_post<DIM, false>, k_knn_bvh_post<DIM, true>), dim3(nb), dim3(BVH_THREADS), lds, c->stream, kf, bv, order, pp);
         *fused_blocks = nb;
diff --git a/icp-variants_amd/csrc/host_loop.hpp b/icp-variants_amd/csrc/host_loop.hpp
--- a/icp-variants_amd/csrc/host_loop.hpp
+++ b/icp-variants_amd/csrc/host_loop.hpp
@@ -231,38 +231,72 @@
     char unused[64];
     int cvg_state[CONV_STATE_BYTES / 4];
     icp_convergence_step* trace() { return (icp_convergence_step*)(this + 1); }
-    static constexpr size_t used_bytes(bool cvg, int n_trace) { return cvg ? sizeof(RunTail) + (size_t)n_trace * sizeof(icp_convergence_step) : offsetof(RunTail, unused); }
+    static constexpr size_t used_bytes(int n_trace) { return sizeof(RunTail) + (size_t)n_trace * sizeof(icp_convergence_step); }
 };
 static_assert(offsetof(RunTail, merged_fault) == 128 && offsetof(RunTail, merged_cvg) == 144 && offsetof(RunTail, unused) == 192 && offsetof(RunTail, cvg_state) == 256 && sizeof(RunTail) == 512, "the layout the device was handed");
+
+struct RunStamps {
+    static size_t bytes(int iters) { return (size_t)2 * (iters + 1) * 8; }
+    static unsigned long long* t0(void* base) { return (unsigned long long*)base; }
+    static unsigned long long* t1(void* base, int iters) { return (unsigned long long*)base + (iters + 1); }
+};
+void sample_iterations(int mode, unsigned phase, int iters, std::vector<char>& sampled) {
+    sampled.assign((size_t)iters, 0);
+    for (int i = 0; i < iters; i++) sampled[(size_t)i] = mode == 1 || (mode > 1 && (i + (int)(phase % (unsigned)mode)) % mode == 0);
+}
+void stamps_to_timing(const unsigned long long* t0, const unsigned long long* t1, int iters, int n_done, const char* sampled, double ticks_per_ms,
+                      icp_timing* t, float* match_ms, float* post_ms, float* solve_ms) {
+    auto ms = [&](unsigned long long from, unsigned long long to) { return (double)(long long)(to - from) / ticks_per_ms; };
+    memset(t, 0, sizeof(*t)); t->iterations = n_done;
+    double sum_match = 0, sum_solve = 0; int n_ev = 0;
+    for (int i = 0; i < n_done; i++) {
+        float a = -1.f, b = -1.f, d = -1.f;
+        if (sampled[i]) {
+            n_ev++;
+            a = (float)ms(t0[i], t1[i]); b = 0.f; d = i == iters - 1 ? (float)ms(t0[iters], t1[iters]) : 0.f;
+            sum_match += a; sum_solve += d;
+        }
+        if (match_ms) match_ms[i] = a;
+        if (post_ms) post_ms[i] = b;
+        if (solve_ms) solve_ms[i] = d;
+    }
+    if (n_ev > 0) { const double f = (double)n_done / n_ev; t->match_ms = sum_match * f; t->solve_ms = sum_solve * f; }
+    t->sampled_iterations = n_ev;
+    t->total_ms = ms(t0[0], t1[iters]);
+}
 
 struct IterEvents { hipEvent_t start = nullptr, matched = nullptr, posted = nullptr, end = nullptr; };
 struct LoopRun {
     RunPlan pl; bool lm, robust, recip, rmse, fontana, cvg; std::vector<char> sampled, eligible; std::vector<IterEvents> ev; int n_enqueued = 0;
-    size_t pin_stats = 256, pin_tail, pin_lm, pin_bytes, stats_bytes;
+    bool stamp_blocks = false;
+    PoseState ps_in;
+    size_t pin_stats = 256, pin_tail, pin_stamps, pin_lm, pin_bytes, stats_bytes;
     void lay_out(int iters, bool with_lm, bool with_cvg) {
         auto pad = [](size_t b) { return (b + 255) & ~(size_t)255; };
         const size_t trace_pad = with_cvg ? pad((size_t)iters * sizeof(icp_convergence_step)) : 0;
-        pin_tail = pin_stats + pad((size_t)iters * sizeof(icp_iter_stats)); pin_lm = pin_tail + sizeof(RunTail) + trace_pad;
+        pin_tail = pin_stats + pad((size_t)iters * sizeof(icp_iter_stats)); pin_stamps = pin_tail + sizeof(RunTail) + trace_pad;
+        pin_lm = pin_stamps + pad(RunStamps::bytes(iters));
         pin_bytes = pin_lm + (with_lm ? (size_t)iters * sizeof(icp_lm_summary) : 0);
-        stats_bytes = records_bytes() + (with_cvg ? sizeof(RunTail) + trace_pad : RunTail::used_bytes(false, 0));
+        stats_bytes = pin_stamps - pin_stats;
     }
     size_t records_bytes() const { return pin_tail - pin_stats; }
     RunTail* dev_tail(const icp_ctx* c) const { return (RunTail*)(c->stats.as<char>() + records_bytes()); }
     icp_iter_stats* host_records(const icp_ctx* c) const { return (icp_iter_stats*)(c->pinned.as<char>() + pin_stats); }
     RunTail* host_tail(const icp_ctx* c) const { return (RunTail*)(c->pinned.as<char>() + pin_tail); }
+    unsigned long long* host_stamps(const icp_ctx* c) const { return (unsigned long long*)(c->pinned.as<char>() + pin_stamps); }
     icp_lm_summary* host_lm(const icp_ctx* c) const { return (icp_lm_summary*)(c->pinned.as<char>() + pin_lm); }
 };
 #ifndef ICP_CONVERGE_CHUNK
 #define ICP_CONVERGE_CHUNK 2
 #endif
 constexpr int CONVERGE_CHUNK = ICP_CONVERGE_CHUNK;
-ConvergeParams converge_params(const icp_ctx* c, const LoopRun& r, int i, int* words) {
+ConvergeParams converge_params(const icp_ctx* c, const LoopRun& r, int i, int* words, icp_convergence_step* trace) {
     ConvergeParams cp; memset(&cp, 0, sizeof(cp));
     if (!r.cvg) return cp;
     const icp_convergence_options& o = c->cvg_opt;
     cp.on = 1; cp.eligible = r.eligible[(size_t)i]; cp.index = i; cp.min_iterations = o.min_iterations; cp.patience = o.patience;
     cp.rotation_eps = o.rotation_eps; cp.translation_eps = o.translation_eps;
-    cp.trace = r.dev_tail(c)->trace(); cp.words = words;
+    cp.trace = trace; cp.words = words;
     return cp;
 }
 hipEvent_t loop_event(const icp_ctx* c, int i, int k) { return c->events[(size_t)2 + 4 * i + k]; }
@@ -274,29 +308,34 @@
     for (int i = 0; i < iters; i++) { const int nb = fused_nblocks(pl.ns[i]); if (nb > nbmax) nbmax = nb; }
     Ring ring;
     if ((rc = make_ring(c, iters + 1, iters, nbmax, &tail->merged_fault, ring))) return rc;
-    const int n_init = (iters + 1) * POSE_REPLICAS * 16 + iters * NSUM + 16;
-    hipLaunchKernelGGL(k_run_init, dim3((n_init + 255) / 256), dim3(256), 0, c->stream, c->ps.as<PoseState>(), ring.slots, iters + 1, ring.trows, iters * NSUM, ring.run_fault, 16);
+    if (r.stamp_blocks && (rc = ensure(c, c->block_t1, (size_t)2 * nbmax * 8))) return rc;
+    if ((rc = ensure(c, c->ps, sizeof(PoseState)))) return rc;
+    char* out = (char*)c->pinned.dev;
+    icp_iter_stats* out_records = (icp_iter_stats*)(out + r.pin_stats); RunTail* out_tail = (RunTail*)(out + r.pin_tail);
+    unsigned long long* stamps = (unsigned long long*)(out + r.pin_stamps);
+    unsigned long long* t0 = RunStamps::t0(stamps); unsigned long long* t1 = RunStamps::t1(stamps, iters);
+    auto block_t1 = [&](int j) { return r.stamp_blocks ? c->block_t1.as<unsigned long long>() + (size_t)(j & 1) * nbmax : nullptr; };
+    const int n_stamps = 2 * (iters + 1), n_init = (iters + 1) * POSE_REPLICAS * 16 + iters * NSUM + 16 + n_stamps;
+    hipLaunchKernelGGL(k_run_init, dim3((n_init + 255) / 256), dim3(256), 0, c->stream, r.ps_in, c->ps.as<PoseState>(), ring.slots, iters + 1, ring.trows, iters * NSUM, ring.run_fault, 16, stamps, n_stamps);
     auto reducer = [&](int i) {
         RingParams rp = ring_params(c, ring, i, i > 0 ? pl.ns[i - 1] : 0, loop_slot(ring.slots, i, 0));
-        if (i > 0) { rp.stats = c->stats.as<icp_iter_stats>() + (i - 1); rp.cv = converge_params(c, r, i - 1, tail->merged_cvg); }
-        if (i == iters) rp.final_out = &tail->final_pose;
+        if (i > 0) { rp.stats = out_records + (i - 1); rp.cv = converge_params(c, r, i - 1, tail->merged_cvg, out_tail->trace()); }
+        rp.st.t0 = t0 + i;
+        if (i < iters) rp.st.block_t1 = block_t1(i);
+        if (i > 0 && r.stamp_blocks) { rp.st.prev_block_t1 = block_t1(i - 1); rp.st.prev_t1 = t1 + (i - 1); }
+        if (i == iters) { rp.final_out = &out_tail->final_pose; rp.words_out = &out_tail->merged_fault; rp.st.end = t1 + iters; }
         return rp;
     };
-    HIPCK(c, hipEventRecord(c->events[0], c->stream));
     for (int i = 0; i < iters; i++) {
         QuerySet q{pl.clouds[i], pl.sels[i], pl.ns[i], 0, p.color_icp != 0 && p.matching == ICP_MATCH_KNN, pl.seeded(i), pl.orders[i]};
         MergeLaunch ml; ml.rp = reducer(i); ml.slot = loop_slot(ring.slots, i, 0); ml.partials = ring_partials(c, i);
-        if (r.sampled[i]) { r.ev[i].start = ml.ev_start = loop_event(c, i, 0); r.ev[i].matched = ml.ev_stop = loop_event(c, i, 1); }
         int fused = 0;
         if ((rc = launch_match(c, q, &fused, &ml))) return rc;
         if (!fused) { c->err = "merged loop: the matcher did not take the fused path"; return ICP_ERR_HIP; }
     }
     hipLaunchKernelGGL(k_ring_reduce_solve, dim3(NSUM_USED), dim3(RING_THREADS), 0, c->stream, reducer(iters));
     HIPCK(c, hipGetLastError());
-    if (r.sampled[iters - 1]) { r.ev[iters - 1].end = loop_event(c, iters - 1, 3); HIPCK(c, hipEventRecord(r.ev[iters - 1].end, c->stream)); }
-    HIPCK(c, hipEventRecord(c->events[1], c->stream));
     r.n_enqueued = iters;
-    HIPCK(c, hipMemcpyAsync(r.host_records(c), c->stats.p, r.records_bytes() + RunTail::used_bytes(r.cvg, iters), hipMemcpyDeviceToHost, c->stream));
     return ICP_OK;
 }
 
@@ -340,7 +379,7 @@
         if (r.rmse && (rc = enqueue_rmse(c, &d_st->rmse))) return rc;
         if (r.fontana && (rc = enqueue_fontana(c, &d_st->benchmark_error))) return rc;
         if (r.cvg) {
-            hipLaunchKernelGGL(k_converge_step, dim3(1), dim3(64), 0, c->stream, converge_params(c, r, i, tail->cvg_state), c->ps.as<PoseState>(), pl.ns[i] > 0 ? d_st : nullptr);
+            hipLaunchKernelGGL(k_converge_step, dim3(1), dim3(64), 0, c->stream, converge_params(c, r, i, tail->cvg_state, tail->trace()), c->ps.as<PoseState>(), pl.ns[i] > 0 ? d_st : nullptr);
             HIPCK(c, hipGetLastError());
         }
         if (ev) HIPCK(c, hipEventRecord(r.ev[i].end, c->stream));
@@ -349,7 +388,7 @@
     HIPCK(c, hipEventRecord(c->events[1], c->stream));
     HIPCK(c, hipMemcpyAsync(r.host_records(c), c->stats.p, (size_t)n_enq * sizeof(icp_iter_stats), hipMemcpyDeviceToHost, c->stream));
     HIPCK(c, hipMemcpyAsync(&htail->final_pose, c->ps.p, sizeof(PoseState), hipMemcpyDeviceToHost, c->stream));
-    if (r.cvg) HIPCK(c, hipMemcpyAsync(htail->cvg_state, tail->cvg_state, RunTail::used_bytes(true, n_enq) - offsetof(RunTail, cvg_state), hipMemcpyDeviceToHost, c->stream));
+    if (r.cvg) HIPCK(c, hipMemcpyAsync(htail->cvg_state, tail->cvg_state, RunTail::used_bytes(n_enq) - offsetof(RunTail, cvg_state), hipMemcpyDeviceToHost, c->stream));
     if (r.lm) HIPCK(c, hipMemcpyAsync(r.host_lm(c), c->lm_sums.p, (size_t)n_enq * sizeof(icp_lm_summary), hipMemcpyDeviceToHost, c->stream));
     return ICP_OK;
 }
@@ -382,19 +421,21 @@
     if ((rc = ensure_pinned(c, r.pin_bytes))) return rc;
     if (lm && (rc = ensure(c, c->lm_sums, (size_t)iters * sizeof(icp_lm_summary)))) return rc;
     float pose_in[16]; memcpy(pose_in, pose_inout, 64);
-    if ((rc = write_pose(c, pose_inout))) return rc;
     if ((rc = ensure(c, c->stats, r.stats_bytes))) return rc;
     r.eligible.assign((size_t)iters, 0);
     for (int i = 0; i < iters; i++) r.eligible[(size_t)i] = pl.factors[i] == pl.factors[iters - 1] && (i == 0 || pl.factors[i] == pl.factors[i - 1]);
-    if ((rc = ensure_events(c, (size_t)iters * 4 + 2))) return rc;
     const bool rmse = r.rmse = (p.record_rmse & 1) && c->conv_n > 0;
     const bool fontana = r.fontana = (p.record_rmse & 2) && c->conv_n > 0;
     bool merged = try_merged && !lm && !robust && !recip && !single && iters >= 2 && pl.sorted_levels && p.metric == ICP_METRIC_POINT_TO_PLANE && !rmse && !fontana;
     for (int i = 0; merged && i < iters; i++) if (pl.ns[i] <= 0) merged = false;
-    const int tmode = c->stage_timing;
-    r.sampled.assign((size_t)iters, 0); r.ev.assign((size_t)iters, IterEvents());
-    for (int i = 0; i < iters; i++) r.sampled[i] = tmode == 1 || (tmode > 1 && (i + (int)(c->timing_phase % (unsigned)tmode)) % tmode == 0);
-    c->timing_phase++;
+    sample_iterations(c->stage_timing, c->timing_phase++, iters, r.sampled);
+    r.stamp_blocks = c->stage_timing != 0;
+    if (merged) make_pose_state(pose_inout, &r.ps_in);
+    else if ((rc = write_pose(c, pose_inout))) return rc;
+    if (merged) {
+        if (c->wall_ticks_per_ms <= 0) { int khz = 0; HIPCK(c, hipDeviceGetAttribute(&khz, hipDeviceAttributeWallClockRate, c->device)); c->wall_ticks_per_ms = khz; }
+        if (c->wall_ticks_per_ms <= 0) { c->err = "the runtime reports no wall clock rate for the device"; return ICP_ERR_HIP; }
+    } else { r.ev.assign((size_t)iters, IterEvents()); if ((rc = ensure_events(c, (size_t)iters * 4 + 2))) return rc; }
     if ((rc = merged ? enqueue_merged(c, r) : enqueue_separate(c, r))) return rc;
     std::vector<icp_robust_stats> rob((size_t)(robust ? iters : 0));
     if (robust) HIPCK(c, hipMemcpyAsync(rob.data(), c->rob_stats.p, (size_t)iters * sizeof(icp_robust_stats), hipMemcpyDeviceToHost, c->stream));
@@ -446,25 +487,32 @@
     }
     icp_timing& t = c->timing; memset(&t, 0, sizeof(t)); t.iterations = n_done;
     c->it_match_ms.assign((size_t)n_done, -1.f); c->it_post_ms.assign((size_t)n_done, -1.f); c->it_solve_ms.assign((size_t)n_done, -1.f);
-    double ev_match = 0, ev_post = 0, ev_solve = 0; int n_ev = 0;
-    for (int i = 0; i < n_done; i++) {
-        if (!r.sampled[i]) continue;
-        n_ev++;
-        const IterEvents& e = r.ev[i];
-        float a = 0, b = 0, d = 0;
-        HIPCK(c, hipEventElapsedTime(&a, e.start, e.matched));
-        if (e.posted) HIPCK(c, hipEventElapsedTime(&b, e.matched, e.posted));
-        if (e.end) HIPCK(c, hipEventElapsedTime(&d, e.posted ? e.posted : e.matched, e.end));
-        ev_match += a; ev_post += b; ev_solve += d;
-        c->it_match_ms[(size_t)i] = a; c->it_post_ms[(size_t)i] = b; c->it_solve_ms[(size_t)i] = d;
-        if (c->trace) fprintf(stderr, "[icp_hip] it %2d  n %d  match %.4f  post %.4f  solve %.4f ms\n", i, pl.ns[i], a, b, d);
-    }
-    if (n_ev > 0) {
-        const double f = (double)n_done / n_ev;
-        t.match_ms += ev_match * f; t.weight_reject_build_ms += ev_post * f; t.solve_ms += ev_solve * f;
-    }
-    t.sampled_iterations = n_ev;
-    float tot = 0; HIPCK(c, hipEventElapsedTime(&tot, c->events[0], c->events[1])); t.total_ms = tot;
+    if (merged) {
+        unsigned long long* hst = r.host_stamps(c);
+        stamps_to_timing(RunStamps::t0(hst), RunStamps::t1(hst, iters), iters, n_done, r.sampled.data(), c->wall_ticks_per_ms, &t, c->it_match_ms.data(), c->it_post_ms.data(), c->it_solve_ms.data());
+        for (int i = 0; c->trace && i < n_done; i++)
+            if (r.sampled[i]) fprintf(stderr, "[icp_hip] it %2d  n %d  match %.4f  post %.4f  solve %.4f ms\n", i, pl.ns[i], c->it_match_ms[(size_t)i], c->it_post_ms[(size_t)i], c->it_solve_ms[(size_t)i]);
+    } else {
+        double ev_match = 0, ev_post = 0, ev_solve = 0; int n_ev = 0;
+        for (int i = 0; i < n_done; i++) {
+            if (!r.sampled[i]) continue;
+            n_ev++;
+            const IterEvents& e = r.ev[i];
+            float a = 0, b = 0, d = 0;
+            HIPCK(c, hipEventElapsedTime(&a, e.start, e.matched));
+            if (e.posted) HIPCK(c, hipEventElapsedTime(&b, e.matched, e.posted));
+            if (e.end) HIPCK(c, hipEventElapsedTime(&d, e.posted ? e.posted : e.matched, e.end));
+            ev_match += a; ev_post += b; ev_solve += d;
+            c->it_match_ms[(size_t)i] = a; c->it_post_ms[(size_t)i] = b; c->it_solve_ms[(size_t)i] = d;
+            if (c->trace) fprintf(stderr, "[icp_hip] it %2d  n %d  match %.4f  post %.4f  solve %.4f ms\n", i, pl.ns[i], a, b, d);
+        }
+        if (n_ev > 0) {
+            const double f = (double)n_done / n_ev;
+            t.match_ms += ev_match * f; t.weight_reject_build_ms += ev_post * f; t.solve_ms += ev_solve * f;
+        }
+        t.sampled_iterations = n_ev;
+        float tot = 0; HIPCK(c, hipEventElapsedTime(&tot, c->events[0], c->events[1])); t.total_ms = tot;
+    }
     if (status != ICP_OK) c->err = "no valid correspondences in at least one iteration (reference would hang in ASSERT)";
     guard.ok = true;
     return status;
@@ -609,7 +657,7 @@
         }
         HIPCK(c, hipMemcpyAsync(rg.slots, slot_image.data(), rg.slot_bytes, hipMemcpyHostToDevice, c->stream));
         const int n_init = n_rows * NSUM + 16;
-        hipLaunchKernelGGL(k_run_init, dim3((n_init + 255) / 256), dim3(256), 0, c->stream, nullptr, rg.slots, 0, rg.trows, n_rows * NSUM, rg.run_fault, 16);
+        hipLaunchKernelGGL(k_run_init, dim3((n_init + 255) / 256), dim3(256), 0, c->stream, PoseState{}, nullptr, rg.slots, 0, rg.trows, n_rows * NSUM, rg.run_fault, 16, nullptr, 0);
         HIPCK(c, hipGetLastError());
     }
     for (int j = 0; j < n_poses; j++) {
```

New measurement: 35820 (median of 6 runs). 2.4% higher.
